# allenai/satlas-super-resolution

Measured on AMD Instinct MI355X. Metric: G+D train-step images/sec, higher is better.
Workload: dtype fp32h

## Files before the change

include/ssr_hip.h:

```cpp
#ifndef SSR_HIP_H
#define SSR_HIP_H

#include <stdint.h>

#ifdef __cplusplus
extern "C" {
#endif

#define SSR_F32 0
#define SSR_BF16 1
#define SSR_F32X3 2
#define SSR_F32H 3
#define SSR_F32H_WSHIFT 10

#define SSR_OK 0
#define SSR_EINVAL (-1)
#define SSR_EUNSUP (-2)

#define SSR_ACT_NONE 0
#define SSR_ACT_LRELU 1
#define SSR_ACT_RELU 2

typedef struct ssr_view {
    void* p;
    int32_t cs;
    int32_t coff;
} ssr_view;

typedef struct ssr_conv_desc {
    int32_t dtype;
    ssr_view x;
    int32_t N, Hi, Wi;
    int32_t up;
    int32_t Cin;
    ssr_view x2;
    int32_t Cin2;
    const void* w;
    int32_t CoutPad;
    const float* bias;
    int32_t KH, KW, stride, pad_y, pad_x;
    int32_t Gh, Gw;
    int32_t Ho, Wo, oys, oyo, oxs, oxo;
    int32_t Cout;
    ssr_view y, y0, y1;
    float alpha;
    int32_t act;
    ssr_view r1; int32_t r1_nc; float beta1;
    ssr_view r2; int32_t r2_nc; float beta2;
    int32_t accumulate;
    ssr_view m; int32_t m_c0, m_c1;
    int32_t s2d;
    int32_t m_relu;
    int32_t* fix_list;
    int32_t fix_cap;
    float fix_thr;
    const float* w_ref;
    const float* w_ref_sigma;
    int32_t w_ref_cin;
} ssr_conv_desc;

int ssr_conv2d(const ssr_conv_desc* d, void* stream);
int ssr_conv2d_fixup(const ssr_conv_desc* d, void* stream);
int ssr_conv2d_batch(const ssr_conv_desc* ds, int32_t n, void* stream);
int ssr_conv2d_impl(const ssr_conv_desc* d, void* stream, int32_t impl);
int ssr_conv2d_variant(const ssr_conv_desc* d);
int ssr_conv2d_chain(const ssr_conv_desc* ds, int32_t n, void* state, void* stream);
int ssr_conv2d_chain_ok(const ssr_conv_desc* ds, int32_t n);
int64_t ssr_conv2d_chain_state_bytes(int32_t N, int32_t Gh, int32_t Gw);
int ssr_conv2d_symbol(const ssr_conv_desc* d, char* buf, int32_t buflen);
int ssr_conv2d_ck(int32_t dtype, int32_t KH);
int ssr_conv2d_s2d_ok(int32_t dtype, int32_t Cin, int32_t Cout, int32_t CoutPad);

typedef struct ssr_rdb_desc {
    int32_t dtype, N, H, W;
    ssr_view in, slices, out, mask;
    const void* w[5];
    const float* bias[5];
    float alpha5, beta1;
    ssr_view r2;
    float beta2;
    const void* w_next[5];
    int32_t w_next_bytes[5];
    int32_t tile;
} ssr_rdb_desc;
int ssr_rdb_forward(const ssr_rdb_desc* d, void* stream);
int ssr_rdb_backward(const ssr_rdb_desc* d, void* stream);
int ssr_rdb_tile_of(const ssr_rdb_desc* d);

typedef struct ssr_wgrad_layer {
    ssr_view x;
    ssr_view dy;
    int32_t N, Hi, Wi, up, Cin, Cout;
    int32_t pad_y, pad_x, Gh, Gw;
    float alpha;
    float* dw;
    int32_t Cin_w;
    float* db;
} ssr_wgrad_layer;

typedef struct ssr_wgrad_item {
    int32_t layer, co0, ci0, tile_begin, tile_end, atomic;
    int32_t nco, layer_b, co0_b;
} ssr_wgrad_item;

int ssr_conv2d_wgrad(const ssr_wgrad_layer* layers_dev, const ssr_wgrad_item* items_dev, int32_t n_items,
                     int32_t dtype, int32_t KH, int32_t KW, int32_t stride, void* stream);
int32_t ssr_wgrad_tiles(int32_t N, int32_t Gh, int32_t Gw, int32_t dtype, int32_t KH);
int32_t ssr_wgrad_ci_tile(int32_t dtype, int32_t KH);
int32_t ssr_wgrad_co_tile(int32_t dtype, int32_t KH);

typedef struct ssr_pack_item {
    const float* src;
    const float* inv_scale;
    void* dst_fwd;
    void* dst_dgrad;
    int32_t Cout, Cin, KH, KW, stride;
    int32_t CoutPad, CinPad;
    int32_t CinPadO, CoutPadI;
    int32_t ck_fwd, ck_dgrad;
    int32_t fwd_s2d;
} ssr_pack_item;

int ssr_pack_weights(const ssr_pack_item* items_dev, int32_t n_items, int32_t dtype, void* stream);

typedef struct ssr_pack_seg {
    const float* src;
    void* dst;
    float scale;
    int32_t Cout, Cin;
    int32_t ci0, nci;
    int32_t kbase;
    int32_t rows_pad, ck;
} ssr_pack_seg;
int ssr_pack_dgrad_gather(const ssr_pack_seg* items_dev, int32_t n_items, int32_t dtype, void* stream);

int ssr_add_views(ssr_view dst, ssr_view src, int32_t dtype, int64_t npix, int32_t C, void* stream);

int ssr_nchw_to_nhwc(const float* src, int32_t N, int32_t C, int32_t H, int32_t W, ssr_view dst, int32_t dtype,
                     int32_t unshuffle, int32_t up, float scale, void* stream);
int ssr_nhwc_to_nchw(ssr_view src, int32_t dtype, float* dst, int32_t N, int32_t C, int32_t H, int32_t W,
                     void* stream);
int ssr_fill(void* p, int64_t n_elems, int32_t dtype, float value, void* stream);

int ssr_bilinear2x_fwd(ssr_view a, ssr_view b, ssr_view y, int32_t dtype, int32_t N, int32_t H, int32_t W, int32_t C,
                       void* stream);
int ssr_bilinear2x_bwd(ssr_view dy, ssr_view r, ssr_view y1, ssr_view y, ssr_view m, int32_t dtype, int32_t N,
                       int32_t H, int32_t W, int32_t C, void* stream);
#define SSR_BILINEAR_FLAT 0x100
int ssr_nearest2x_bwd(ssr_view dy, ssr_view r, ssr_view y1, ssr_view y, ssr_view m, int32_t dtype, int32_t N,
                      int32_t H, int32_t W, int32_t C, void* stream);

typedef struct ssr_sn_item {
    const float* w;
    float* u;
    float* v;
    float* sigma;
    float* tmp;
    int32_t rows, cols;
} ssr_sn_item;
int ssr_spectral_norm(const ssr_sn_item* items_dev, int32_t n_items, int32_t max_rows, int32_t max_cols,
                      int32_t power_iter, void* stream);
#define SSR_SN_BWD_SLOTS 64
typedef struct ssr_sn_bwd_item {
    const float* dw_sn; const float* w; const float* u; const float* v; const float* sigma;
    float* dw; float* tmp; int32_t rows, cols;
} ssr_sn_bwd_item;
int ssr_spectral_norm_bwd(const ssr_sn_bwd_item* items_dev, int32_t n_items, int32_t max_elems, void* stream);

int ssr_usm_sharp(const float* src, float* dst, int32_t planes, int32_t H, int32_t W, float in_scale, float weight,
                  float threshold, void* stream);

#define SSR_DETERMINISTIC 0x200
#define SSR_LOSS_SLOTS 256
int ssr_l1_loss(ssr_view a, ssr_view b, ssr_view grad, int32_t dtype, int64_t npix, int32_t C, float weight,
                float* loss_out, void* stream);
int ssr_bce_logits_loss(ssr_view x, ssr_view grad, int32_t dtype, int64_t npix, float target, float weight,
                        float* loss_out, float* mean_out, void* stream);

typedef struct ssr_reduce_item { float* dst; const float* src; int64_t n, stride; int32_t parts, pad_; } ssr_reduce_item;
int ssr_wgrad_reduce(const ssr_reduce_item* items_dev, int32_t n_items, int64_t max_elems, void* stream);

typedef struct ssr_adam_args {
    float* param; const float* grad; float* exp_avg; float* exp_avg_sq;
    float* ema;
    int64_t n;
    const float* lr;
    int32_t* step;
    float beta1, beta2, eps, ema_decay, grad_scale;
} ssr_adam_args;
int ssr_adam_step(const ssr_adam_args* a, void* stream);

int ssr_axpby_f32(float a, const float* x, float b, float* y, int64_t n, void* stream);

#define SSR_SCAN_MAX_RANGES 8
int ssr_nonfinite_scan(const float* const* srcs, const int64_t* ns, int32_t n_ranges, int32_t* flag, void* stream);
int ssr_adam_step_guarded(const ssr_adam_args* a, int32_t* flag, int32_t* skipped, void* stream);

int ssr_quantize_u8(const float* src_nchw, uint8_t* dst_nhwc, int32_t N, int32_t C, int32_t H, int32_t W, int32_t mode, void* stream);
int ssr_quantize_u8_checked(const float* src_nchw, uint8_t* dst_nhwc, int32_t N, int32_t C, int32_t H, int32_t W, int32_t mode,
                            int32_t* nonfinite, void* stream);
int ssr_metric_shift_sums(const uint8_t* a, const uint8_t* b, int32_t H, int32_t W, int32_t C, int32_t crop, int32_t max_offset,
                          int64_t* out, void* stream);
int ssr_metric_ssim_sums(const uint8_t* a, const uint8_t* b, int32_t H, int32_t W, int32_t C, int32_t crop, double* out, void* stream);

int ssr_scene_zero_scan(const uint8_t* scene, int32_t T, int32_t H, int32_t W, uint8_t* has_zero, void* stream);
int ssr_scene_gather(const uint8_t* scene, int32_t T, int32_t H, int32_t W, const int32_t* chunk_ids, const int32_t* frame_ids,
                     int32_t B, int32_t n, ssr_view dst, int32_t dtype, void* stream);
int ssr_scene_scatter_u8(ssr_view src, int32_t dtype, const int32_t* chunk_ids, int32_t B, int32_t C, uint8_t* mosaic, int32_t Ho,
                         int32_t Wo, int32_t* nonfinite, void* stream);

int ssr_scene_zero_scan_at(const uint8_t* scene, int32_t T, int32_t H, int32_t W, const int32_t* origins, int32_t n_chunks,
                           uint8_t* has_zero, void* stream);
int ssr_scene_gather_at(const uint8_t* scene, int32_t T, int32_t H, int32_t W, const int32_t* origins, const int32_t* frame_ids,
                        int32_t B, int32_t n, ssr_view dst, int32_t dtype, void* stream);
// ... 39 lines not shown
```

satlas_super_resolution_amd/csrc/common.h:

```cpp
#pragma once
#include <hip/hip_runtime.h>
#include <stdint.h>
#include "ssr_hip.h"
#include <type_traits>

template <int I, int N, typename F> __device__ __forceinline__ void static_for(F&& f) {
    if constexpr (I < N) {
        f(std::integral_constant<int, I>{});
        static_for<I + 1, N>(f);
    }
}

typedef float f32x4 __attribute__((ext_vector_type(4)));
typedef float f32x16 __attribute__((ext_vector_type(16)));
typedef __bf16 bf16x8 __attribute__((ext_vector_type(8)));
typedef __bf16 bf16x4 __attribute__((ext_vector_type(4)));
typedef uint32_t u32x4 __attribute__((ext_vector_type(4)));
typedef _Float16 f16x8 __attribute__((ext_vector_type(8)));
typedef _Float16 f16x4 __attribute__((ext_vector_type(4)));

template <bool H> __device__ __forceinline__ f32x16 split_mfma(const bf16x8& a, const bf16x8& b, const f32x16& c) {
    if constexpr (H) return __builtin_amdgcn_mfma_f32_32x32x16_f16(__builtin_bit_cast(f16x8, a), __builtin_bit_cast(f16x8, b), c, 0, 0, 0);
    else return __builtin_amdgcn_mfma_f32_32x32x16_bf16(a, b, c, 0, 0, 0);
}
template <bool H> __device__ __forceinline__ void split_f32x4(const u32x4& v, uint2& hi, uint2& lo) {
    const f32x4 f = __builtin_bit_cast(f32x4, v);
    if constexpr (H) {
        f16x4 h, l;
#pragma unroll
        for (int k = 0; k < 4; ++k) {
            h[k] = (_Float16)f[k];
            l[k] = (_Float16)(f[k] - (float)h[k]);
        }
        hi = __builtin_bit_cast(uint2, h);
        lo = __builtin_bit_cast(uint2, l);
    } else {
        bf16x4 h, l;
#pragma unroll
        for (int k = 0; k < 4; ++k) {
            h[k] = (__bf16)f[k];
            l[k] = (__bf16)(f[k] - (float)h[k]);
        }
        hi = __builtin_bit_cast(uint2, h);
        lo = __builtin_bit_cast(uint2, l);
    }
}
constexpr float SSR_F32H_WSCALE = (float)(1 << SSR_F32H_WSHIFT), SSR_F32H_UNSCALE = 1.0f / (float)(1 << SSR_F32H_WSHIFT);

#define LRELU_SLOPE 0.2f

template <typename T> struct DT;
template <> struct DT<float> { static constexpr int VEC = 4; };
template <> struct DT<__bf16> { static constexpr int VEC = 8; };

__device__ __forceinline__ float to_f32(float v) { return v; }
__device__ __forceinline__ float to_f32(__bf16 v) { return (float)v; }
template <typename T> __device__ __forceinline__ T from_f32(float v);
template <> __device__ __forceinline__ float from_f32<float>(float v) { return v; }
template <> __device__ __forceinline__ __bf16 from_f32<__bf16>(float v) { return (__bf16)v; }

__device__ __forceinline__ float lrelu(float v) { return v > 0.f ? v : LRELU_SLOPE * v; }
__device__ __forceinline__ float lrelu_grad_from_out(float out) { return out > 0.f ? 1.f : LRELU_SLOPE; }
__device__ __forceinline__ float lrelu_max(float v) {
    float r;
    const float s = LRELU_SLOPE * v;
    asm("v_max_f32 %0, %1, %2" : "=v"(r) : "v"(v), "v"(s));
    return r;
}
__device__ __forceinline__ float lrelu_mask_lo(float v, unsigned m2) { return (int)(m2 << 16) > 0 ? v : LRELU_SLOPE * v; }
__device__ __forceinline__ float lrelu_mask_hi(float v, unsigned m2) { return (int)m2 > 0xFFFF ? v : LRELU_SLOPE * v; }

template <typename T> __device__ __forceinline__ void mma16(f32x16& acc, const u32x4& a, const u32x4& b);
template <> __device__ __forceinline__ void mma16<float>(f32x16& acc, const u32x4& a, const u32x4& b) {
    const f32x4 af = __builtin_bit_cast(f32x4, a), bf = __builtin_bit_cast(f32x4, b);
#pragma unroll
    for (int s = 0; s < 4; ++s) acc = __builtin_amdgcn_mfma_f32_32x32x2f32(af[s], bf[s], acc, 0, 0, 0);
}
template <> __device__ __forceinline__ void mma16<__bf16>(f32x16& acc, const u32x4& a, const u32x4& b) {
    acc = __builtin_amdgcn_mfma_f32_32x32x16_bf16(__builtin_bit_cast(bf16x8, a), __builtin_bit_cast(bf16x8, b), acc,
                                                  0, 0, 0);
}

__device__ __forceinline__ int mfma32_row(int r, int g) { return (r & 3) + 8 * (r >> 2) + 4 * g; }

constexpr int SSR_MAX_DEVICES = 32;
inline int ssr_device_ordinal() {
    int dev = 0;
    if (hipGetDevice(&dev) != hipSuccess || dev < 0 || dev >= SSR_MAX_DEVICES) dev = 0;
    return dev;
}

#define SSR_LAUNCH_CHECK()                       \
    do {                                         \
        hipError_t e__ = hipGetLastError();      \
        if (e__ != hipSuccess) return (int)e__;  \
    } while (0)
```

satlas_super_resolution_amd/csrc/conv.hip:

```cpp
#include "conv_epilogue.h"
#include <cstdlib>
#include <cstdio>

namespace {

template <typename T, int KH, int KW, int S, int NT, int MW, int KS>
__device__ __forceinline__ void conv_body(const ssr_conv_desc& d) {
    constexpr int VEC = DT<T>::VEC;
    constexpr int KSTEPS = (KH == 4) ? 1 : 2;
    constexpr int CK = KSTEPS * 2 * VEC, VPR = 2 * KSTEPS, CKP = CK + VEC, BN = 32 * NT;
    constexpr int TH = 2 * MW, TW = 16;
    constexpr int PH = (TH - 1) * S + KH, PW = (TW - 1) * S + KW;
    constexpr int NTHR = 64 * MW * KS;
    constexpr int PVEC = PH * PW * VPR, WVEC = KH * KW * BN * VPR;
    constexpr int NPV = (PVEC + NTHR - 1) / NTHR, NWV = (WVEC + NTHR - 1) / NTHR;
    constexpr int STAGE = (PH * PW + KH * KW * BN) * CKP;
    extern __shared__ __attribute__((aligned(16))) char smem[];
    T* lds = reinterpret_cast<T*>(smem);

    const int tid = threadIdx.x, lane = tid & 63, wave = tid >> 6;
    const int wm = wave % MW, kh = wave / MW;
    const int tiles_x = (d.Gw + TW - 1) / TW, tiles_y = (d.Gh + TH - 1) / TH;
    int b = blockIdx.x;
    const int tx_i = b % tiles_x; b /= tiles_x;
// ... 635 lines not shown
            if (KS == 2 && kh_s == 1) contract_h(buf, std::integral_constant<int, 1>{}, units);
            else contract_h(buf, std::integral_constant<int, 0>{}, units);
        } else {
            if (KS == 2 && kh_s == 1) contract_h(buf, std::integral_constant<int, 1>{}, none);
            else contract_h(buf, std::integral_constant<int, 0>{}, none);
        }
    };

    XPROBE(1);
    static_for<0, PD>([&](auto jc) { load_stage(decltype(jc)::value, jc); });
    store_stage(0, std::integral_constant<int, 0>{});
    __syncthreads();
    XPROBE(2);
    for (int c = 0; c < nst; c += PD) {
        static_for<0, PD>([&](auto jc) {
            constexpr int j = decltype(jc)::value;
            const int cur = c + j;
            if (cur < nst) {
                load_stage(cur + PD, jc);
                contract(cur & 1, std::integral_constant<int, (j + 1) % PD>{}, cur + 1 < nst);
#ifdef SSR_PROBE
                const unsigned long long tm_ = __builtin_amdgcn_s_memtime();
#endif
#ifdef SSR_PROBE
                if (threadIdx.x == 0 && cur == 0) { g_probe[(blockIdx.y * gridDim.x + blockIdx.x) * 24 + 20] = tm_; g_probe[(blockIdx.y * gridDim.x + blockIdx.x) * 24 + 21] = __builtin_amdgcn_s_memtime(); }
#endif
                __syncthreads();
#ifdef SSR_PROBE
                if (cur < 12) XPROBE(3 + cur);
#endif
            }
        });
    }
    XPROBE(15);

    char* slab = smem + (size_t)MW * 16 * 64 * sizeof(float) + (size_t)wave * EPI_STAGE_BYTES;
    auto epilogue = [&](const f32x16& a, int t) {
        conv_epilogue<float>(d, a, co0 + t * 32, n, gy0 + 2 * wm, gx0, lane, slab);
    };
    if (KS == 1) {
#pragma unroll
        for (int t = 0; t < NT; ++t) epilogue(acc[t], t);
    } else {
        float* red = reinterpret_cast<float*>(smem);
        float* mine = red + (wm * 16) * 64 + lane;
        if (NT == 2) {
            if (kh == 0) {
#pragma unroll
                for (int r = 0; r < 16; ++r) mine[r * 64] = acc[1][r];
            }
            __syncthreads();
            if (kh == 1) {
#pragma unroll
                for (int r = 0; r < 16; ++r) acc[1][r] += mine[r * 64];
            }
            __syncthreads();
            if (kh == 1) {
#pragma unroll
                for (int r = 0; r < 16; ++r) mine[r * 64] = acc[0][r];
            }
            __syncthreads();
            if (kh == 0) {
#pragma unroll
                for (int r = 0; r < 16; ++r) acc[0][r] += mine[r * 64];
                epilogue(acc[0], 0);
            } else {
                epilogue(acc[1], 1);
            }
        } else {
            if (kh == 1) {
#pragma unroll
                for (int r = 0; r < 16; ++r) mine[r * 64] = acc[0][r];
            }
            __syncthreads();
            if (kh == 0) {
#pragma unroll
                for (int r = 0; r < 16; ++r) acc[0][r] += mine[r * 64];
                epilogue(acc[0], 0);
            }
        }
    }
    XPROBE(17);
}

template <int KH, int KW, int NT, int MW, int KS, int CPS, int PD>
__global__ __launch_bounds__(64 * MW * KS) void conv_x3p_kernel(const ssr_conv_desc d) {
    conv_body_x3p<KH, KW, NT, MW, KS, CPS, PD>(d);
}

template <int KH, int KW, int NT, int MW, int KS, int CPS, int PD>
int launch_conv_x3p(const ssr_conv_desc& d, hipStream_t st) {
    constexpr int BN = 32 * NT, TH = 2 * MW, TW = 16, PH = TH - 1 + KH, PW = TW - 1 + KW;
    constexpr size_t stage = (size_t)CPS * (PH * PW + KH * KW * BN) * 80;
    constexpr size_t red = (size_t)MW * 16 * 64 * sizeof(float) + (size_t)MW * KS * EPI_STAGE_BYTES;
    constexpr size_t lds = 2 * stage > red ? 2 * stage : red;
    static_assert(lds <= 160 * 1024, "LDS budget");
    auto kern = conv_x3p_kernel<KH, KW, NT, MW, KS, CPS, PD>;
    static bool attr_done[SSR_MAX_DEVICES] = {};
    const int attr_dev = ssr_device_ordinal();
    if (!attr_done[attr_dev]) {
        hipError_t e = hipFuncSetAttribute(reinterpret_cast<const void*>(kern), hipFuncAttributeMaxDynamicSharedMemorySize, (int)lds);
        if (e != hipSuccess) return (int)e;
        attr_done[attr_dev] = true;
    }
    const int tiles = ((d.Gw + TW - 1) / TW) * ((d.Gh + TH - 1) / TH) * d.N;
    hipLaunchKernelGGL(kern, dim3(tiles, d.CoutPad / BN, 1), dim3(64 * MW * KS), lds, st, d);
    SSR_LAUNCH_CHECK();
    return SSR_OK;
}

bool x3p_ok(const ssr_conv_desc& d, int cps) {
    static const bool on = [] { const char* e = getenv("SSR_X3_PIPE"); return e && e[0] == '1'; }();
    if (!on) return false;
    const long lim = 0x7fffff00L, npx = (long)d.N * d.Hi * d.Wi * 4;
    if (npx * d.x.cs > lim || (d.x2.p && npx * d.x2.cs > lim)) return false;
    if (d.x2.p && (d.Cin % (16 * cps)) != 0) return false;
    return true;
}

template <int KH, int KW, bool H = false>
int dispatch_tile_x3(const ssr_conv_desc& d, hipStream_t st) {
    bool nt2, small;
    pick_tile(d, nt2, small);
    static const long thr = [] { const char* e = getenv("SSR_X3_SMALL"); return e ? atol(e) : 0L; }();
    small = (long)((d.Gw + 15) / 16) * ((d.Gh + 7) / 8) * d.N * (d.CoutPad / (nt2 ? 64 : 32)) < thr;
    if (!small && !H) {
        static const bool p2 = [] { const char* e = getenv("SSR_X3_PIPE2"); return e && e[0] == '1'; }();
        if (nt2 && p2 && x3p_ok(d, 1)) return launch_conv_x3p<KH, KW, 2, 4, 2, 1, 3>(d, st);
        if (!nt2 && x3p_ok(d, 2)) return launch_conv_x3p<KH, KW, 1, 4, 2, 2, 2>(d, st);
    }
    if (nt2) return small ? launch_conv_x3<KH, KW, 2, 2, 2, H>(d, st) : launch_conv_x3<KH, KW, 2, 4, 2, H>(d, st);
    return small ? launch_conv_x3<KH, KW, 1, 2, 2, H>(d, st) : launch_conv_x3<KH, KW, 1, 4, 2, H>(d, st);
}

bool view_ok(const ssr_view& v, bool required) {
    if (!v.p) return !required;
    return (v.cs % 8) == 0 && (v.coff % 8) == 0 && ((uintptr_t)v.p % 16) == 0;
}

}

bool ssr_conv_res_try(const ssr_conv_desc& d, hipStream_t st, int* rc);
bool ssr_conv_res_qualifies(const ssr_conv_desc& d);
bool ssr_conv_ws_try(const ssr_conv_desc& d, hipStream_t st, int* rc, bool force);
bool ssr_conv_ws_qualifies(const ssr_conv_desc& d);
bool ssr_conv_thin_try(const ssr_conv_desc& d, hipStream_t st, int* rc, bool force);
bool ssr_conv_thin_qualifies(const ssr_conv_desc& d);
bool ssr_conv_big_try(const ssr_conv_desc& d, hipStream_t st, int* rc, bool force);
bool ssr_conv_big_qualifies(const ssr_conv_desc& d);
bool ssr_conv_big_batch_try(const ssr_conv_desc* ds, int n, hipStream_t st, int* rc);
bool ssr_conv_bigx3_try(const ssr_conv_desc& d, hipStream_t st, int* rc, bool force);
bool ssr_conv_bigx3_qualifies(const ssr_conv_desc& d);
bool ssr_conv_bigx3_batch_try(const ssr_conv_desc* ds, int n, hipStream_t st, int* rc);
bool ssr_conv_x3q_try(const ssr_conv_desc& d, hipStream_t st, int* rc, bool force);
bool ssr_conv_x3q_qualifies(const ssr_conv_desc& d);
bool ssr_conv_x3r_try(const ssr_conv_desc& d, hipStream_t st, int* rc, bool force);
bool ssr_conv_x3r_qualifies(const ssr_conv_desc& d);

extern "C" int ssr_conv2d_s2d_ok(int32_t dtype, int32_t Cin, int32_t Cout, int32_t CoutPad) {
    static const bool off = [] { const char* e = getenv("SSR_CONV_S2D"); return e && e[0] == '0'; }();
    if (dtype == SSR_F32X3 || dtype == SSR_F32H) {
        static const bool offx = [] { const char* e = getenv("SSR_X3_BIGTILE"); return e && e[0] == '0'; }();
        const int cpx = Cin / 16;
        return !off && !offx && Cin >= 16 && (Cin % 16) == 0 && (cpx & (cpx - 1)) == 0 && (CoutPad % 64) == 0 && (Cout % 8) == 0;
    }
    const int cpc = Cin / 32;
    return !off && dtype == SSR_BF16 && Cin >= 32 && (Cin % 32) == 0 && (cpc & (cpc - 1)) == 0 && (CoutPad % 64) == 0 && (Cout % 8) == 0;
}

extern "C" int ssr_conv2d_variant(const ssr_conv_desc* dp) {
    if (!dp) return SSR_EINVAL;
    if (dp->s2d) return dp->KH * 1000 + dp->stride * 100 + 2 * 10 + 9;
    const bool split = dp->dtype == SSR_F32X3 || dp->dtype == SSR_F32H;
    const bool pipelined_only = !split && (dp->act == SSR_ACT_RELU || dp->m_relu);
    if (!pipelined_only) {
        if (dp->dtype != SSR_BF16 && ssr_conv_thin_qualifies(*dp)) return dp->KH * 1000 + dp->stride * 100 + 1 * 10 + 7;
        if (split && ssr_conv_bigx3_qualifies(*dp)) return dp->KH * 1000 + dp->stride * 100 + 2 * 10 + 9;
        if (split && ssr_conv_x3r_qualifies(*dp))
            return dp->KH * 1000 + dp->stride * 100 + ((dp->CoutPad % 64) == 0 ? 2 : 1) * 10 + 5;
        if (dp->dtype == SSR_F32X3 && ssr_conv_x3q_qualifies(*dp))
            return dp->KH * 1000 + dp->stride * 100 + ((dp->CoutPad % 64) == 0 ? 2 : 1) * 10 + 6;
        if (!split) {
            if (ssr_conv_thin_qualifies(*dp)) return dp->KH * 1000 + dp->stride * 100 + 1 * 10 + 7;
            if (ssr_conv_ws_qualifies(*dp)) return dp->KH * 1000 + dp->stride * 100 + 1 * 10 + 8;
            if (ssr_conv_big_qualifies(*dp)) return dp->KH * 1000 + dp->stride * 100 + 2 * 10 + 9;
            if (dp->dtype == SSR_F32 && ssr_conv_x3r_qualifies(*dp))
                return dp->KH * 1000 + dp->stride * 100 + ((dp->CoutPad % 64) == 0 ? 2 : 1) * 10 + 5;
            if (ssr_conv_res_qualifies(*dp)) return dp->KH * 1000 + dp->stride * 100 + 1 * 10 + 1;
        }
    }
    bool nt2, small;
    pick_tile(*dp, nt2, small);
    return dp->KH * 1000 + dp->stride * 100 + (nt2 ? 2 : 1) * 10 + (small ? 2 : 4);
}

void ssr_conv_x3r_instance(const ssr_conv_desc& d, int* ntw, int* nu, int* ep);
int ssr_conv_x3r_tile_height(const ssr_conv_desc& d);

extern "C" int ssr_conv2d_symbol(const ssr_conv_desc* dp, char* buf, int32_t buflen) {
    if (!dp || !buf || buflen < 48) return SSR_EINVAL;
    const ssr_conv_desc& d = *dp;
    const int v = ssr_conv2d_variant(dp);
    if (v < 0) return v;
    const int w = v % 10, nt = (v / 10) % 10;
    const bool f32m = d.dtype != SSR_BF16;
    if (d.dtype != SSR_BF16 && w == 5) {
        int ntw = 1, nu = 1, ep = 3;
        ssr_conv_x3r_instance(d, &ntw, &nu, &ep);
        snprintf(buf, buflen, "conv_x3r_kernel<%d, %d, %d, %d, %d>", ntw, nu, ep, ssr_conv_x3r_tile_height(d), d.dtype == SSR_F32 ? 1 : d.dtype == SSR_F32H ? 2 : 0);
    } else if (d.dtype == SSR_F32X3 && w == 6) snprintf(buf, buflen, "conv_x3q_kernel<%d>", nt);
    else if (d.dtype == SSR_F32X3 && w == 9) snprintf(buf, buflen, "conv_bigx3_kernel4<%d>", (d.s2d || d.KH == 2) ? 2 : 3);
    else if (d.dtype == SSR_F32H && w == 9) snprintf(buf, buflen, "conv_bigh3_kernel4<%d>", (d.s2d || d.KH == 2) ? 2 : 3);
    else if (f32m && w == 7) snprintf(buf, buflen, "conv_thin_f32_kernel<%d, %d>", d.Cout == 1 ? 1 : d.Cout <= 3 ? 3 : d.Cout == 4 ? 4 : 8, d.dtype == SSR_F32X3 ? 1 : d.dtype == SSR_F32H ? 2 : 0);
    else snprintf(buf, buflen, "%s<%s,K%d,S%d,NT%d,W%d>", w == 7 ? "conv_thin_kernel" : w == 8 ? "conv_ws_kernel" : w == 9 ? "conv_big_kernel" : w == 1 ? "conv_res_kernel" : d.dtype == SSR_F32X3 ? "conv_x3_kernel" : d.dtype == SSR_F32H ? "conv_h3_kernel" : "conv_kernel",
                  d.dtype == SSR_BF16 ? "bf16" : d.dtype == SSR_F32 ? "fp32" : d.dtype == SSR_F32H ? "fp32h" : "fp32x3", v / 1000, (v / 100) % 10, nt, w);
    return SSR_OK;
}

extern "C" int ssr_conv2d_ck(int32_t dtype, int32_t KH) {
    const int vec = dtype == SSR_BF16 ? 8 : 4;
    return (KH == 4 ? 1 : 2) * 2 * vec;
}

static int conv2d_impl(const ssr_conv_desc* dp, void* stream, int impl) {
    if (!dp) return SSR_EINVAL;
    const ssr_conv_desc& d = *dp;
    if (d.act < SSR_ACT_NONE || d.act > SSR_ACT_RELU) return SSR_EINVAL;
    if (!view_ok(d.x, true) || !d.w || ((uintptr_t)d.w % 16) != 0) return SSR_EINVAL;
    if (!d.y.p || d.y.cs <= 0) return SSR_EINVAL;
    if (d.Cin <= 0 || (d.Cin % 8) != 0 || d.CoutPad <= 0 || (d.CoutPad % 32) != 0 || d.Cout > d.CoutPad)
        return SSR_EINVAL;
    if (!(d.up == 1 || d.up == 2) || d.N <= 0 || d.Gh <= 0 || d.Gw <= 0) return SSR_EINVAL;
    if (d.x2.p && (d.Cin2 <= 0 || (d.Cin2 % 8) != 0 || !view_ok(d.x2, true))) return SSR_EINVAL;
    if (!d.x2.p && d.Cin2 != 0) return SSR_EINVAL;
    hipStream_t st = reinterpret_cast<hipStream_t>(stream);
    int rc = 0;
    if (d.s2d) {
        if (!(d.KH == 4 && d.KW == 4 && d.stride == 2 && d.pad_y == 1 && d.pad_x == 1 && d.up == 1 && !d.x2.p)) return SSR_EINVAL;
        if (!ssr_conv2d_s2d_ok(d.dtype, d.Cin, d.Cout, d.CoutPad) || (d.Hi % 2) || (d.Wi % 2) || d.Gh != d.Hi / 2 || d.Gw != d.Wi / 2)
            return SSR_EINVAL;
        ssr_conv_desc e = d;
        e.KH = e.KW = 2; e.stride = 1; e.pad_y = e.pad_x = 0; e.Cin = 4 * d.Cin;
        if (d.dtype == SSR_F32X3 || d.dtype == SSR_F32H) return ssr_conv_bigx3_try(e, st, &rc, true) ? rc : SSR_EUNSUP;
        return ssr_conv_big_try(e, st, &rc, true) ? rc : SSR_EUNSUP;
    }
    if (d.dtype == SSR_F32H) {
        if (d.fix_list) return SSR_EUNSUP;
        if (impl == 4) return ssr_conv_bigx3_try(d, st, &rc, true) ? rc : SSR_EUNSUP;
        if (impl == 5) return ssr_conv_thin_try(d, st, &rc, true) ? rc : SSR_EUNSUP;
        if (impl == 7) return ssr_conv_x3r_try(d, st, &rc, true) ? rc : SSR_EUNSUP;
        if (impl == 0 && ssr_conv_thin_try(d, st, &rc, false)) return rc;
        if (impl == 0 && ssr_conv_bigx3_try(d, st, &rc, false)) return rc;
        if (impl == 0 && ssr_conv_x3r_try(d, st, &rc, false)) return rc;
        if (d.KH == 3 && d.KW == 3 && d.stride == 1) return dispatch_tile_x3<3, 3, true>(d, st);
        if (d.KH == 2 && d.KW == 2 && d.stride == 1) return dispatch_tile_x3<2, 2, true>(d, st);
        ssr_conv_desc e = d;
        e.dtype = SSR_F32;
        return dispatch_geom<float>(e, st);
    }
    if (d.dtype == SSR_F32X3) {
        if (impl == 4) return ssr_conv_bigx3_try(d, st, &rc, true) ? rc : SSR_EUNSUP;
        if (impl == 5) return ssr_conv_thin_try(d, st, &rc, true) ? rc : SSR_EUNSUP;
        if (impl == 6) return ssr_conv_x3q_try(d, st, &rc, true) ? rc : SSR_EUNSUP;
        if (impl == 7) return ssr_conv_x3r_try(d, st, &rc, true) ? rc : SSR_EUNSUP;
        if (impl == 0 && ssr_conv_thin_try(d, st, &rc, false)) return rc;
        if (impl == 0 && ssr_conv_bigx3_try(d, st, &rc, false)) return rc;
        if (impl == 0 && ssr_conv_x3r_try(d, st, &rc, false)) return rc;
        if (impl == 0 && ssr_conv_x3q_try(d, st, &rc, false)) return rc;
        if (d.KH == 3 && d.KW == 3 && d.stride == 1) return dispatch_tile_x3<3, 3>(d, st);
        if (d.KH == 2 && d.KW == 2 && d.stride == 1) return dispatch_tile_x3<2, 2>(d, st);
        ssr_conv_desc e = d;
        e.dtype = SSR_F32;
        return dispatch_geom<float>(e, st);
    }
    if (d.act == SSR_ACT_RELU || d.m_relu) impl = 3;
    if (impl == 1) return ssr_conv_ws_try(d, st, &rc, true) ? rc : SSR_EUNSUP;
    if (impl == 4) return ssr_conv_big_try(d, st, &rc, true) ? rc : SSR_EUNSUP;
    if (impl == 5) return ssr_conv_thin_try(d, st, &rc, true) ? rc : SSR_EUNSUP;
    if (impl == 0 && ssr_conv_thin_try(d, st, &rc, false)) return rc;
    if (impl == 0 && ssr_conv_ws_try(d, st, &rc, false)) return rc;
    if (impl == 0 && ssr_conv_big_try(d, st, &rc, false)) return rc;
    if (d.dtype == SSR_F32 && impl == 7) return ssr_conv_x3r_try(d, st, &rc, true) ? rc : SSR_EUNSUP;
    if (d.dtype == SSR_F32 && impl == 0 && ssr_conv_x3r_try(d, st, &rc, false)) return rc;
    if (impl != 3 && ssr_conv_res_try(d, st, &rc)) return rc;
    if (d.dtype == SSR_F32) return dispatch_geom<float>(d, st);
    if (d.dtype == SSR_BF16) return dispatch_geom<__bf16>(d, st);
    return SSR_EUNSUP;
}

extern "C" int ssr_conv2d(const ssr_conv_desc* dp, void* stream) { return conv2d_impl(dp, stream, 0); }

namespace {
__global__ __launch_bounds__(256) void conv_fixup_kernel(const ssr_conv_desc d) {
    int* hdr = d.fix_list;
    const int count = min(hdr[0], d.fix_cap);
    const int lane = threadIdx.x & 63, wave = threadIdx.x >> 6;
    const int nw = gridDim.x * 4;
    const int KK = d.KH * d.KW, K = d.w_ref_cin * KK;
    const float* __restrict__ xp = reinterpret_cast<const float*>(d.x.p);
    float* __restrict__ yp = reinterpret_cast<float*>(d.y.p);
    const double inv_sigma = d.w_ref_sigma ? 1.0 / (double)d.w_ref_sigma[0] : 1.0;
    const int sh = d.up == 2 ? 1 : 0, LH = d.Hi << sh, LW = d.Wi << sh;
    for (int e = blockIdx.x * 4 + wave; e < count; e += nw) {
        const int p = hdr[4 + 2 * e], co = hdr[5 + 2 * e];
        const int ox = p % d.Wo, t = p / d.Wo, oy = t % d.Ho, n = t / d.Ho;
        const float* __restrict__ wrow = d.w_ref + (size_t)co * K;
        double s = 0.0;
        for (int k = lane; k < K; k += 64) {
            const int ci = k / KK, tap = k - ci * KK, ky = tap / d.KW, kx = tap - ky * d.KW;
            const int iy = oy * d.stride + ky - d.pad_y, ix = ox * d.stride + kx - d.pad_x;
            if (iy >= 0 && iy < LH && ix >= 0 && ix < LW) {
                const size_t px = (size_t)(n * d.Hi + (iy >> sh)) * d.Wi + (ix >> sh);
                s += (double)wrow[k] * (double)xp[px * d.x.cs + d.x.coff + ci];
            }
        }
#pragma unroll
        for (int m = 32; m >= 1; m >>= 1) s += __shfl_xor(s, m);
        if (lane == 0) {
            const float v = (float)(s * inv_sigma + (d.bias ? (double)d.bias[co] : 0.0));
            yp[(size_t)p * d.y.cs + d.y.coff + co] = lrelu(v);
        }
    }
    __syncthreads();
    if (threadIdx.x == 0) {
        __threadfence();
        if (atomicAdd(hdr + 1, 1) == (int)gridDim.x - 1) {
            atomicMax(hdr + 2, hdr[0]);
            hdr[0] = 0;
            hdr[1] = 0;
        }
    }
}
}

extern "C" int ssr_conv2d_fixup(const ssr_conv_desc* dp, void* stream) {
    if (!dp) return SSR_EINVAL;
    const ssr_conv_desc& d = *dp;
    if (!d.fix_list || d.fix_cap <= 0 || !d.w_ref || d.w_ref_cin <= 0 || !d.x.p || !d.y.p) return SSR_EINVAL;
    if ((d.dtype != SSR_F32X3 && d.dtype != SSR_F32) || d.act != SSR_ACT_LRELU || d.x2.p || d.y0.p || d.y1.p || d.r1.p || d.r2.p || d.m.p ||
        d.accumulate || d.alpha != 1.f || d.stride != 1 || d.s2d || d.oys != 1 || d.oxs != 1 || d.oyo != 0 || d.oxo != 0 ||
        d.w_ref_cin > d.Cin)
        return SSR_EUNSUP;
    hipLaunchKernelGGL(conv_fixup_kernel, dim3(32), dim3(256), 0, reinterpret_cast<hipStream_t>(stream), d);
    SSR_LAUNCH_CHECK();
    return SSR_OK;
}

extern "C" int ssr_conv2d_batch(const ssr_conv_desc* ds, int32_t n, void* stream) {
    if (!ds || n <= 0 || n > 4) return SSR_EINVAL;
    bool same = ds[0].dtype == SSR_BF16 && ds[0].KH == 2 && ds[0].KW == 2 && ds[0].stride == 1;
    for (int k = 1; k < n && same; ++k)
        same = ds[k].dtype == ds[0].dtype && ds[k].KH == 2 && ds[k].KW == 2 && ds[k].stride == 1 && ds[k].N == ds[0].N &&
               ds[k].Gh == ds[0].Gh && ds[k].Gw == ds[0].Gw && ds[k].CoutPad == ds[0].CoutPad && ds[k].Cin == ds[0].Cin &&
               ds[k].Cin2 == ds[0].Cin2 && ds[k].Hi == ds[0].Hi && ds[k].Wi == ds[0].Wi && ds[k].up == ds[0].up;
    static const bool off = [] { const char* e = getenv("SSR_CONV_BATCH"); return e && e[0] == '0'; }();
    if (!off && ds[0].dtype == SSR_F32X3 && ds[0].KH == 2 && ds[0].KW == 2 && ds[0].stride == 1) {
        int rcx = 0;
        if (ssr_conv_bigx3_batch_try(ds, n, reinterpret_cast<hipStream_t>(stream), &rcx)) return rcx;
    }
    if (same && !off) {
        for (int k = 0; k < n; ++k) {
            const ssr_conv_desc& d = ds[k];
            if (!view_ok(d.x, true) || !d.w || ((uintptr_t)d.w % 16) != 0 || !d.y.p || d.y.cs <= 0 || d.Cin <= 0 || (d.Cin % 8) != 0 ||
                d.CoutPad <= 0 || (d.CoutPad % 32) != 0 || d.Cout > d.CoutPad || !(d.up == 1 || d.up == 2) || d.N <= 0 || d.Gh <= 0 ||
                d.Gw <= 0 || (d.x2.p && (d.Cin2 <= 0 || (d.Cin2 % 8) != 0 || !view_ok(d.x2, true))) || (!d.x2.p && d.Cin2 != 0))
                return SSR_EINVAL;
        }
        hipStream_t st = reinterpret_cast<hipStream_t>(stream);
        int rcb = 0;
        if (ssr_conv_big_batch_try(ds, n, st, &rcb)) return rcb;
        bool nt2, small;
        pick_tile(ds[0], nt2, small);
        const long tiles4 = (long)((ds[0].Gw + 15) / 16) * ((ds[0].Gh + 7) / 8) * ds[0].N * (ds[0].CoutPad / (nt2 ? 64 : 32)) * n;
        small = tiles4 < 384;
        if (nt2) return small ? launch_conv4<__bf16, 2, 2, 1, 2, 2, 2>(ds, n, st) : launch_conv4<__bf16, 2, 2, 1, 2, 4, 2>(ds, n, st);
        return small ? launch_conv4<__bf16, 2, 2, 1, 1, 2, 2>(ds, n, st) : launch_conv4<__bf16, 2, 2, 1, 1, 4, 2>(ds, n, st);
    }
    for (int k = 0; k < n; ++k) {
        const int rc = conv2d_impl(ds + k, stream, 0);
// ... 8 lines not shown
```

satlas_super_resolution_amd/csrc/conv_big_x3.hip:

```cpp
#include "common.h"
#include <cstdlib>

namespace {

constexpr int XB_TH = 32, XB_TW = 16;
template <int KT> struct XbT {
    static constexpr int AROW = 80;
    static constexpr int VPP = 4;
    static constexpr int PH = XB_TH + KT - 1, PW = XB_TW + KT - 1, NPIX = PH * PW;
    static constexpr int PATCH = NPIX * AROW;
    static constexpr int WROWS = KT * KT * 64;
    static constexpr int WBYTES = WROWS * AROW;
    static constexpr int BUF = PATCH + WBYTES;
    static constexpr int BIAS = BUF;
    static constexpr int SLABS = BIAS + 256;
    static constexpr int LDS = SLABS + 4 * 32 * 272;
    static constexpr int NPV = (NPIX * VPP + 255) / 256;
    static constexpr int NWV = (WROWS * VPP + 255) / 256;
    static constexpr int NSTEP = KT * KT;
    static constexpr int TAIL = KT == 3 ? 2 : 1;
    static constexpr int LPS = (NPV + NWV + NSTEP - TAIL - 1) / (NSTEP - TAIL);
    static_assert(LDS <= 160 * 1024 && LPS <= 6, "LDS budget / load slots of a step");
};

#define XB_BAR() asm volatile("s_waitcnt lgkmcnt(0)\n\ts_barrier" ::: "memory")
#ifdef SSR_PROBE
#define XB_T() (__builtin_amdgcn_s_memtime())
#define XB_ACC(k, t0) do { const unsigned long long t1_ = XB_T(); xb_t[k] += t1_ - (t0); (t0) = t1_; } while (0)
#else
#define XB_T() 0ull
#define XB_ACC(k, t0) do { } while (0)
#endif
constexpr int XB_OOB = 0x7ffffff0;
constexpr int XB_SLAB_PITCH = 272, XB_SLAB = 32 * XB_SLAB_PITCH;
__device__ __forceinline__ __amdgpu_buffer_rsrc_t xb_rsrc(const void* p, long bytes) {
    return __builtin_amdgcn_make_buffer_rsrc(const_cast<void*>(p), 0, (int)(bytes > 0x7fffff00L ? 0x7fffff00L : (bytes < 0 ? 0 : bytes)), 0x00020000);
}
template <int KT>
__device__ __forceinline__ void xb_pixel(int w, int m, int s, int& row, int& col) {
    row = 8 * w + 2 * m + (s >> 4);
    col = s < 16 ? s : ((s + 32 - (XB_TW + KT - 1)) & 15);
}
__device__ __forceinline__ void xb_split4(const u32x4& v, uint2& hi, uint2& lo) {
    const f32x4 f = __builtin_bit_cast(f32x4, v);
    bf16x4 h, l;
#pragma unroll
    for (int k = 0; k < 4; ++k) {
        h[k] = (__bf16)f[k];
        l[k] = (__bf16)(f[k] - (float)h[k]);
    }
    hi = __builtin_bit_cast(uint2, h);
    lo = __builtin_bit_cast(uint2, l);
}

template <int KT, bool H = false>
__device__ __forceinline__ void conv_bigx3_body(const ssr_conv_desc& d) {
    using T = XbT<KT>;
    constexpr int AROW = T::AROW, VPP = T::VPP, PW = T::PW, NPIX = T::NPIX, PATCH = T::PATCH, NPV = T::NPV, NWV = T::NWV, NSTEP = T::NSTEP;
    extern __shared__ __attribute__((aligned(16))) char smem[];
    const int tid = threadIdx.x, lane = tid & 63, wave = tid >> 6;
    const int i = lane & 31, g = lane >> 5;
    const int tiles_x = (d.Gw + XB_TW - 1) / XB_TW, tiles_y = (d.Gh + XB_TH - 1) / XB_TH;
    const int tpi = tiles_x * tiles_y, G = gridDim.x / tpi;
    const int tp = blockIdx.x % tpi, n0 = blockIdx.x / tpi;
    const int tx_i = tp % tiles_x, ty_i = tp / tiles_x;
    const int nimg = (d.N - n0 + G - 1) / G;
    const int gy0 = ty_i * XB_TH, gx0 = tx_i * XB_TW;
    const int co0 = blockIdx.y * 64;
    const int upshift = d.up == 2 ? 1 : 0;
    const int LH = d.Hi << upshift, LW = d.Wi << upshift;
    const int nchunks = (d.Cin + 15) / 16;
    const int wchunk = KT * KT * d.CoutPad * 64;
    const int T_ = nimg * nchunks;
    const int ximg = d.Hi * d.Wi * d.x.cs * 4, oimg = d.Ho * d.Wo;

    unsigned long long xb_t[8] = {0, 0, 0, 0, 0, 0, 0, 0}, xb_t0 = XB_T();
    const unsigned long long xb_start = xb_t0;
    (void)xb_t; (void)xb_start;
    float* bias_lds = reinterpret_cast<float*>(smem + T::BIAS);
    if (tid < 64) bias_lds[tid] = (d.bias && co0 + tid < d.Cout) ? d.bias[co0 + tid] * (H ? SSR_F32H_WSCALE : 1.f) : 0.f;

    const bool s2d = KT == 2 && d.s2d != 0;
    const int cpc_shift = s2d ? 31 - __builtin_clz((unsigned)(d.Cin >> 6)) : 0;
    const int x_cs = d.x.cs, x_Wi = d.Wi, x_Cin = d.Cin;
    static_assert((T::WROWS * VPP) % 256 == 0, "no partial weight vector");
    const int p4 = tid >> 2, part4 = tid & 3;
    const int plo0 = p4 * AROW + part4 * 8;
    const int wlo0 = PATCH + p4 * AROW + part4 * 16;
    const int wgo0 = (co0 + p4) * 64 + part4 * 16, wstep = d.CoutPad * 64;
    constexpr int PTAIL = NPIX * VPP - (NPV - 1) * 256;
    int pgo[NPV];
    unsigned pmk[KT == 2 ? NPV : 1];
    const int climit = s2d ? 0x7fffffff : x_Cin - (tid % VPP) * 4;
#pragma unroll
    for (int q = 0; q < NPV; ++q) {
        const int v = tid + q * 256;
        const int pix = v / VPP, part = v % VPP;
        const int py = pix / PW, px = pix - py * PW;
        const int ly = gy0 + py - d.pad_y, lx = gx0 + px - d.pad_x;
        if constexpr (KT == 2) {
            if (s2d) {
                const int sy = 2 * ly - 1, sx = 2 * lx - 1;
                const bool y0 = sy >= 0 && sy < d.Hi, y1 = sy + 1 >= 0 && sy + 1 < d.Hi;
                const bool x0 = sx >= 0 && sx < d.Wi, x1 = sx + 1 >= 0 && sx + 1 < d.Wi;
                pmk[q] = v < NPIX * VPP ? (unsigned)(y0 && x0) | (unsigned)(y0 && x1) << 1 | (unsigned)(y1 && x0) << 2 | (unsigned)(y1 && x1) << 3 : 0u;
                pgo[q] = ((sy * d.Wi + sx) * d.x.cs + d.x.coff + part * 4) * 4 + (d.Wi + 1) * d.x.cs * 4;
            } else {
                const bool ok = v < NPIX * VPP && ly >= 0 && ly < LH && lx >= 0 && lx < LW;
                pmk[q] = ok ? 1u : 0u;
                pgo[q] = ok ? (((ly >> upshift) * d.Wi + (lx >> upshift)) * d.x.cs + d.x.coff + part * 4) * 4 : XB_OOB;
            }
        } else {
            const bool ok = v < NPIX * VPP && ly >= 0 && ly < LH && lx >= 0 && lx < LW;
            pgo[q] = ok ? (((ly >> upshift) * d.Wi + (lx >> upshift)) * d.x.cs + d.x.coff + part * 4) * 4 : XB_OOB;
        }
    }
    const long xbias = s2d ? (long)(d.Wi + 1) * d.x.cs * 4 : 0;
    const __amdgpu_buffer_rsrc_t rsx = xb_rsrc(reinterpret_cast<const char*>(d.x.p) - xbias, (long)d.N * ximg + xbias),
                                 rsw = xb_rsrc(d.w, (long)nchunks * wchunk);
    u32x4 rp[NPV], rw[NWV];
    struct LoadPos { int q, c0, xs, ws; };
    auto load_pos = [&](int nn, int c) {
        LoadPos p;
        p.c0 = c * 16;
        if constexpr (KT == 2) {
            p.q = s2d ? c >> cpc_shift : 0;
            p.xs = nn * ximg + (s2d ? (((p.q >> 1) * x_Wi + (p.q & 1)) * x_cs + ((c - (p.q << cpc_shift)) << 4)) * 4 : p.c0 * 4);
        } else {
            p.q = 0;
            p.xs = nn * ximg + p.c0 * 4;
        }
        p.ws = c * wchunk;
        return p;
    };
    auto load_one = [&](const LoadPos& lp, auto jc) {
        constexpr int j = decltype(jc)::value;
        if constexpr (j < NPV) {
            bool ok = lp.c0 < climit;
            if constexpr (KT == 2) ok = ok && ((pmk[j] >> lp.q) & 1u);
            rp[j] = __builtin_amdgcn_raw_buffer_load_b128(rsx, ok ? pgo[j] : XB_OOB, lp.xs, 0);
        } else {
            rw[j - NPV] = __builtin_amdgcn_raw_buffer_load_b128(rsw, wgo0, lp.ws + (j - NPV) * wstep, 0);
        }
    };
    auto load_chunk = [&](int nn, int c) { const LoadPos lp = load_pos(nn, c); static_for<0, NPV + NWV>([&](auto jc) { load_one(lp, jc); }); };
    auto store_chunk = [&]() {
        static_for<0, NPV>([&](auto jc) {
            constexpr int j = decltype(jc)::value;
            uint2 hi, lo;
            split_f32x4<H>(rp[j], hi, lo);
            if (j + 1 < NPV || tid < PTAIL) {
                *reinterpret_cast<uint2*>(smem + plo0 + j * 64 * AROW) = hi;
                *reinterpret_cast<uint2*>(smem + plo0 + j * 64 * AROW + 32) = lo;
            }
        });
        static_for<0, NWV>([&](auto jc) {
            constexpr int j = decltype(jc)::value;
            *reinterpret_cast<u32x4*>(smem + wlo0 + j * 64 * AROW) = rw[j];
        });
    };

    int a_off[4];
#pragma unroll
    for (int m = 0; m < 4; ++m) {
        int row, col;
        xb_pixel<KT>(wave, m, i, row, col);
        a_off[m] = (row * PW + col) * AROW + g * 16;
    }
    const int b_off = PATCH + i * AROW + g * 16;
    const int co_l = 4 * g;

    load_chunk(n0, 0);
    __syncthreads();
    XB_ACC(1, xb_t0);
    f32x16 acc[4][2];
    auto acc_init = [&]() {
#pragma unroll
        for (int t = 0; t < 2; ++t)
#pragma unroll
            for (int q4 = 0; q4 < 4; ++q4) {
                const f32x4 bq = *reinterpret_cast<const f32x4*>(bias_lds + t * 32 + 8 * q4 + co_l);
#pragma unroll
                for (int e = 0; e < 4; ++e)
#pragma unroll
                    for (int m = 0; m < 4; ++m) acc[m][t][4 * q4 + e] = bq[e];
            }
    };

    char* slab = smem + T::SLABS + wave * XB_SLAB;
    auto epilogue_impl = [&](int nn, auto opsc, auto y01c) __attribute__((always_inline)) {
        constexpr bool OPS = decltype(opsc)::value, Y01 = decltype(y01c)::value;
        const long obytes = (long)d.N * oimg * 4;
        const __amdgpu_buffer_rsrc_t rs_r1 = xb_rsrc(d.r1.p, d.r1.p ? obytes * d.r1.cs : 0), rs_r2 = xb_rsrc(d.r2.p, d.r2.p ? obytes * d.r2.cs : 0),
                                     rs_m = xb_rsrc(d.m.p, d.m.p ? obytes * d.m.cs : 0), rs_y = xb_rsrc(d.y.p, obytes * d.y.cs),
                                     rs_y0 = xb_rsrc(d.y0.p, d.y0.p ? obytes * d.y0.cs : 0), rs_y1 = xb_rsrc(d.y1.p, d.y1.p ? obytes * d.y1.cs : 0);
        const bool has_r1 = d.r1.p != nullptr, has_r2 = d.r2.p != nullptr, has_m = d.m.p != nullptr, has_acc = d.accumulate != 0,
                   has_y0 = d.y0.p != nullptr, has_y1 = d.y1.p != nullptr, m_relu = d.m_relu != 0;
        const float slope = d.act == SSR_ACT_LRELU ? 0.2f : d.act == SSR_ACT_RELU ? 0.f : 1.f;
        const float alpha = d.alpha, beta1 = has_r1 ? d.beta1 : 0.f, beta2 = has_r2 ? d.beta2 : 0.f, gacc = has_acc ? 1.f : 0.f;
        const int y_cs = d.y.cs, y_co = d.y.coff, y0_cs = d.y0.cs, y0_co = d.y0.coff, y1_cs = d.y1.cs, y1_co = d.y1.coff;
        const int r1_cs = d.r1.cs, r1_co = d.r1.coff, r2_cs = d.r2.cs, r2_co = d.r2.coff, m_cs = d.m.cs, m_co = d.m.coff;
        const int Gh = d.Gh, Gw = d.Gw, oys = d.oys, oyo = d.oyo, oxs = d.oxs, oxo = d.oxo, Wo = d.Wo;
        const int pimg = nn * oimg;
        const int hp = lane >> 4, c = co0 + (lane & 15) * 4;
        const bool cok = c < d.Cout;
#pragma unroll
        for (int m = 0; m < 4; ++m) {
            int po[8];
#pragma unroll
            for (int h = 0; h < 8; ++h) {
                int row, col;
                xb_pixel<KT>(wave, m, 4 * h + hp, row, col);
                const int gy = gy0 + row, gx = gx0 + col;
                const bool ok = gy < Gh && gx < Gw;
                const int cy = gy < Gh ? gy : Gh - 1, cx = gx < Gw ? gx : Gw - 1;
                po[h] = (pimg + (cy * oys + oyo) * Wo + cx * oxs + oxo) | (ok && cok ? 0 : (int)0x80000000);
            }
#pragma unroll
            for (int t = 0; t < 2; ++t)
#pragma unroll
                for (int q4 = 0; q4 < 4; ++q4) {
                    const f32x4 v = {acc[m][t][4 * q4], acc[m][t][4 * q4 + 1], acc[m][t][4 * q4 + 2], acc[m][t][4 * q4 + 3]};
                    *reinterpret_cast<f32x4*>(slab + i * XB_SLAB_PITCH + (t * 32 + 8 * q4 + co_l) * 4) = v;
                }
#pragma unroll
            for (int hh = 0; hh < 2; ++hh) {
                u32x4 q1[OPS ? 4 : 1], q2[OPS ? 4 : 1], qa[OPS ? 4 : 1], qm[OPS ? 4 : 1];
                if constexpr (OPS) {
#pragma unroll
                    for (int h4 = 0; h4 < 4; ++h4) {
                        const int pp = po[4 * hh + h4] & 0x7fffffff;
                        q1[h4] = __builtin_amdgcn_raw_buffer_load_b128(rs_r1, cok && has_r1 ? (pp * r1_cs + r1_co + c) * 4 : XB_OOB, 0, 0);
                        q2[h4] = __builtin_amdgcn_raw_buffer_load_b128(rs_r2, cok && has_r2 ? (pp * r2_cs + r2_co + c) * 4 : XB_OOB, 0, 0);
                        qa[h4] = __builtin_amdgcn_raw_buffer_load_b128(rs_y, cok && has_acc ? (pp * y_cs + y_co + c) * 4 : XB_OOB, 0, 0);
                        qm[h4] = __builtin_amdgcn_raw_buffer_load_b128(rs_m, cok && has_m ? (pp * m_cs + m_co + c) * 4 : XB_OOB, 0, 0);
                    }
                }
#pragma unroll
                for (int h4 = 0; h4 < 4; ++h4) {
                    const int h = 4 * hh + h4;
                    f32x4 a = *reinterpret_cast<const f32x4*>(slab + (4 * h + hp) * XB_SLAB_PITCH + (lane & 15) * 16);
                    if constexpr (H) a *= SSR_F32H_UNSCALE;
                    const bool ok = po[h] >= 0;
                    const int pp = po[h] & 0x7fffffff;
                    f32x4 v, s0, s1;
#pragma unroll
                    for (int e = 0; e < 4; ++e) {
                        float x = fmaxf(a[e], slope * a[e]) * alpha;
                        s0[e] = x;
                        if constexpr (OPS) {
                            x += beta1 * __builtin_bit_cast(f32x4, q1[h4])[e] + beta2 * __builtin_bit_cast(f32x4, q2[h4])[e] + gacc * __builtin_bit_cast(f32x4, qa[h4])[e];
                            s1[e] = x;
                            const float mv = __builtin_bit_cast(f32x4, qm[h4])[e];
                            const float f = m_relu ? (mv > 0.f ? 1.f : 0.f) : lrelu_grad_from_out(mv);
                            x *= has_m ? f : 1.f;
                        } else {
                            s1[e] = x;
                        }
                        v[e] = x;
                    }
                    if constexpr (Y01) {
                        __builtin_amdgcn_raw_buffer_store_b128(__builtin_bit_cast(u32x4, s0), rs_y0, ok && has_y0 ? (pp * y0_cs + y0_co + c) * 4 : XB_OOB, 0, 0);
                        __builtin_amdgcn_raw_buffer_store_b128(__builtin_bit_cast(u32x4, s1), rs_y1, ok && has_y1 ? (pp * y1_cs + y1_co + c) * 4 : XB_OOB, 0, 0);
                    }
                    __builtin_amdgcn_raw_buffer_store_b128(__builtin_bit_cast(u32x4, v), rs_y, ok ? (pp * y_cs + y_co + c) * 4 : XB_OOB, 0, 0);
                }
            }
        }
    };
    auto epilogue = [&](int nn) __attribute__((always_inline)) {
        const bool ops = d.r1.p != nullptr || d.r2.p != nullptr || d.m.p != nullptr || d.accumulate != 0;
        const bool y01 = d.y0.p != nullptr || d.y1.p != nullptr;
        if (ops) {
            if (y01) epilogue_impl(nn, std::true_type{}, std::true_type{});
            else epilogue_impl(nn, std::true_type{}, std::false_type{});
        } else {
            if (y01) epilogue_impl(nn, std::false_type{}, std::true_type{});
            else epilogue_impl(nn, std::false_type{}, std::false_type{});
        }
    };

    auto chunk = [&](int c, bool stored, int nn1, int c1, auto hnc) __attribute__((always_inline)) {
        constexpr bool has_next = decltype(hnc)::value;
        xb_t0 = XB_T();
        if (!stored) {
            if (c > 0) XB_BAR();
            XB_ACC(2, xb_t0);
            store_chunk();
            XB_ACC(3, xb_t0);
        }
        XB_BAR();
        XB_ACC(4, xb_t0);
        const LoadPos lp1 = load_pos(nn1, c1);
        bf16x8 wq[2][2][2], pq[2][4][2];
        auto issue1 = [&](auto sc, auto kc) {
            constexpr int s_ = decltype(sc)::value, k = decltype(kc)::value;
            if constexpr (k < 4)
                wq[s_ & 1][k >> 1][k & 1] = *reinterpret_cast<const bf16x8*>(smem + b_off + (s_ * 64 + (k >> 1) * 32) * AROW + (k & 1) * 32);
            else
                pq[s_ & 1][(k - 4) >> 1][k & 1] =
                    *reinterpret_cast<const bf16x8*>(smem + a_off[(k - 4) >> 1] + ((s_ / KT) * PW + s_ % KT) * AROW + (k & 1) * 32);
        };
        static_for<0, 12>([&](auto kc) { issue1(std::integral_constant<int, 0>{}, kc); });
        static_for<0, NSTEP>([&](auto sc) {
            constexpr int s_ = decltype(sc)::value;
            static_for<0, 24>([&](auto kc) {
                constexpr int k = decltype(kc)::value, m = k / 6, t = (k % 6) / 3, p = k % 3;
                acc[m][t] = split_mfma<H>(wq[s_ & 1][t][p == 0 ? 1 : 0], pq[s_ & 1][m][p == 1 ? 1 : 0], acc[m][t]);
                __builtin_amdgcn_sched_barrier(0);
                if constexpr (k < 12) {
                    if constexpr (s_ + 1 < NSTEP) issue1(std::integral_constant<int, s_ + 1>{}, kc);
                } else if constexpr (has_next && (k & 1) == 0 && (k - 12) / 2 < T::LPS) {
                    constexpr int j = s_ * T::LPS + (k - 12) / 2;
                    if constexpr (j < NPV + NWV) load_one(lp1, std::integral_constant<int, j>{});
                }
                __builtin_amdgcn_sched_barrier(0);
            });
        });
        __builtin_amdgcn_sched_barrier(0);
        XB_ACC(5, xb_t0);
        xb_t[7] += 1;
    };
    int gc = 0;
    for (int k = 0; k < nimg; ++k) {
        const int nn = n0 + k * G;
        const bool last_img = k + 1 == nimg;
        acc_init();
        for (int c = 0; c < (last_img ? nchunks - 1 : nchunks); ++c, ++gc) {
            const bool last_c = c + 1 == nchunks;
            chunk(gc, k > 0 && c == 0, last_c ? nn + G : nn, last_c ? 0 : c + 1, std::true_type{});
        }
        if (!last_img) {
            xb_t0 = XB_T();
            XB_BAR();
            XB_ACC(2, xb_t0);
            store_chunk();
            XB_ACC(3, xb_t0);
            epilogue(nn);
            XB_ACC(6, xb_t0);
        }
    }
    const int nl = n0 + (nimg - 1) * G;
    chunk(gc, nimg > 1 && nchunks == 1, nl, 0, std::false_type{});
    xb_t0 = XB_T();
    epilogue(nl);
    XB_ACC(6, xb_t0);
#ifdef SSR_PROBE
    if (tid == 0) {
        xb_t[0] = XB_T() - xb_start;
        const int b = (blockIdx.z * gridDim.y + blockIdx.y) * gridDim.x + blockIdx.x;
        for (int k = 0; k < 8; ++k) g_probe[b * 8 + k] = xb_t[k];
    }
#endif
    (void)T_;
}

struct ssr_conv_desc4x { ssr_conv_desc d[4]; };
template <int KT>
__global__ __launch_bounds__(256, 1) void conv_bigx3_kernel4(const ssr_conv_desc4x p) {
    conv_bigx3_body<KT>(p.d[blockIdx.z]);
}
template <int KT>
__global__ __launch_bounds__(256, 1) void conv_bigh3_kernel4(const ssr_conv_desc4x p) {
    conv_bigx3_body<KT, true>(p.d[blockIdx.z]);
}

template <int KT, bool H = false>
int launch_bigx3(const ssr_conv_desc* ds, int n, hipStream_t st) {
    constexpr int lds = XbT<KT>::LDS;
    const ssr_conv_desc& d = ds[0];
    const int tpi = ((d.Gh + XB_TH - 1) / XB_TH) * ((d.Gw + XB_TW - 1) / XB_TW);
    static const int ncu = [] { int dev = 0, v = 256; if (hipGetDevice(&dev) == hipSuccess && hipDeviceGetAttribute(&v, hipDeviceAttributeMultiprocessorCount, dev) != hipSuccess) v = 256; return v > 0 ? v : 256; }();
    int G = d.N;
    {
        const long per_img = (long)tpi * (d.CoutPad / 64) * n;
        long best = -1;
        for (int g = 1; g <= d.N; ++g) {
            const long rounds = (per_img * g + ncu - 1) / ncu, cost = rounds * ((d.N + g - 1) / g);
            const long key = (cost << 24) | (rounds << 12) | (4095 - (g > 4095 ? 4095 : g));
            if (best < 0 || key < best) { best = key; G = g; }
        }
    }
    if (const char* e = getenv("SSR_CONV_BIG_G")) {
        const int g = atoi(e);
        if (g >= 1) G = g < d.N ? g : d.N;
    }
    const int tiles = tpi * G;
    auto kern = H ? conv_bigh3_kernel4<KT> : conv_bigx3_kernel4<KT>;
    static bool attr_done[SSR_MAX_DEVICES] = {};
    const int attr_dev = ssr_device_ordinal();
    if (!attr_done[attr_dev]) {
        hipError_t e = hipFuncSetAttribute(reinterpret_cast<const void*>(kern), hipFuncAttributeMaxDynamicSharedMemorySize, lds);
        if (e != hipSuccess) return (int)e;
        attr_done[attr_dev] = true;
    }
    ssr_conv_desc4x p;
    for (int k = 0; k < 4; ++k) p.d[k] = ds[k < n ? k : 0];
    hipLaunchKernelGGL(kern, dim3(tiles, d.CoutPad / 64, n), dim3(256), lds, st, p);
    SSR_LAUNCH_CHECK();
    return SSR_OK;
}

}

bool ssr_conv_bigx3_shape_ok(const ssr_conv_desc& d) {
    if ((d.dtype != SSR_F32X3 && d.dtype != SSR_F32H) || d.fix_list) return false;
    const bool k3 = d.KH == 3 && d.KW == 3 && d.pad_y == 1 && d.pad_x == 1;
    const bool k2 = d.KH == 2 && d.KW == 2 && (d.pad_y == 0 || d.pad_y == 1) && (d.pad_x == 0 || d.pad_x == 1);
    if (!(k3 || k2) || d.stride != 1 || d.x2.p) return false;
    if (d.Cin < 8 || (d.CoutPad % 64) != 0 || (d.Cout % 4) != 0) return false;
    if (d.s2d) {
        const int cpc = d.Cin / 64;
        if (!k2 || d.pad_y != 0 || d.pad_x != 0 || d.up != 1 || (d.Cin % 64) != 0 || cpc < 1 || (cpc & (cpc - 1)) != 0) return false;
        if ((d.Hi % 2) != 0 || (d.Wi % 2) != 0 || d.Gh != d.Hi / 2 || d.Gw != d.Wi / 2) return false;
    } else if (d.Gh != (d.Hi << (d.up == 2)) || d.Gw != (d.Wi << (d.up == 2))) return false;
    if (d.r1.p && d.r1_nc < d.Cout) return false;
    if (d.r2.p && d.r2_nc < d.Cout) return false;
    if (d.m.p && !(d.m_c0 == 0 && d.m_c1 >= d.Cout)) return false;
    const long lim = 0x7fffff00L;
    const long xin = ((long)d.N * d.Hi * d.Wi + d.Wi + 1) * d.x.cs * 4, npo = (long)d.N * d.Ho * d.Wo * 4;
    if (xin > lim || npo * d.y.cs > lim || (d.y0.p && npo * d.y0.cs > lim) || (d.y1.p && npo * d.y1.cs > lim) || (d.r1.p && npo * d.r1.cs > lim) ||
        (d.r2.p && npo * d.r2.cs > lim) || (d.m.p && npo * d.m.cs > lim))
        return false;
    if ((long)((d.Cin + 15) / 16) * d.KH * d.KW * d.CoutPad * 64 > lim) return false;
    auto al16 = [](const ssr_view& v) { return !v.p || ((v.cs % 4) == 0 && (v.coff % 4) == 0 && ((uintptr_t)v.p % 16) == 0); };
    return d.x.p && d.y.p && al16(d.x) && al16(d.y) && al16(d.y0) && al16(d.y1) && al16(d.r1) && al16(d.r2) && al16(d.m);
}

bool ssr_conv_bigx3_qualifies(const ssr_conv_desc& d) {
    static const bool off = [] { const char* e = getenv("SSR_X3_BIGTILE"); return e && e[0] == '0'; }();
    if (off || !ssr_conv_bigx3_shape_ok(d) || d.KH != 3) return false;
    const long per_img = (long)((d.Gh + XB_TH - 1) / XB_TH) * ((d.Gw + XB_TW - 1) / XB_TW) * (d.CoutPad / 64);
    return per_img >= 4 && d.Gh >= 24;
}

bool ssr_conv_bigx3_try(const ssr_conv_desc& d, hipStream_t st, int* rc, bool force) {
    if (force ? !ssr_conv_bigx3_shape_ok(d) : !ssr_conv_bigx3_qualifies(d)) return false;
    if (d.dtype == SSR_F32H) *rc = d.KH == 3 ? launch_bigx3<3, true>(&d, 1, st) : launch_bigx3<2, true>(&d, 1, st);
    else *rc = d.KH == 3 ? launch_bigx3<3>(&d, 1, st) : launch_bigx3<2>(&d, 1, st);
    return true;
}

bool ssr_conv_bigx3_batch_try(const ssr_conv_desc* ds, int n, hipStream_t st, int* rc) {
    const char* e = getenv("SSR_X3_BIGTILE2");
    const bool off = e && e[0] == '0', always = e && e[0] == '2';
    if (off || n < 1 || n > 4) return false;
    for (int k = 0; k < n; ++k)
        if (!ssr_conv_bigx3_shape_ok(ds[k]) || ds[k].dtype != SSR_F32X3 || ds[k].KH != 2 || ds[k].s2d) return false;
    const ssr_conv_desc& d = ds[0];
    for (int k = 1; k < n; ++k)
        if (ds[k].N != d.N || ds[k].Gh != d.Gh || ds[k].Gw != d.Gw || ds[k].CoutPad != d.CoutPad || ds[k].Cin != d.Cin || ds[k].Hi != d.Hi || ds[k].Wi != d.Wi ||
            ds[k].up != d.up)
            return false;
    const long per_img = (long)((d.Gh + XB_TH - 1) / XB_TH) * ((d.Gw + XB_TW - 1) / XB_TW) * (d.CoutPad / 64) * n;
    if (!always && (per_img < 8 || d.Gh < 24)) return false;
    *rc = launch_bigx3<2>(ds, n, st);
    return true;
}
```

satlas_super_resolution_amd/csrc/conv_x3c.hip:

```cpp
#include "conv_x3r_core.h"
#include <cstdio>

#ifdef SSR_PROBE
#define CPROBE(cond, k) do { if (cond) g_probe[blockIdx.x * 32 + (k)] = __builtin_amdgcn_s_memtime(); } while (0)
#else
#define CPROBE(cond, k)
#endif

namespace {

constexpr int XC_MAXN = 4;
constexpr int XC_MAXCH = 16;
constexpr int XC_NS = 6;
constexpr int XC_RING = XC_NS * XR_SUB;
constexpr int XC_RED = 16 * XR_SLOT;
constexpr int XC_CTL = XC_RING + XC_RED;
constexpr int XC_LDS = XC_CTL + 256;
static_assert(XC_LDS <= 160 * 1024, "LDS budget");
constexpr int XC_STATE_HDR = 64;
constexpr int XC_POLL_MAX = 1 << 20;

struct ssr_chain_args {
    ssr_conv_desc d[XC_MAXN];
    int32_t n;
// ... 217 lines not shown
                });
                int gn = g + 4 < glast ? g + 4 : glast;
                int c_next = gn / 3, base_next = base_of(gn);
                int gnn = gn, c_nn = c_next, base_nn = base_next;
                auto body = [&](int j, auto jpc) {
                    constexpr int JP = decltype(jpc)::value;
                    static_for<0, NSUB>([&](auto qc) {
                        constexpr int q = decltype(qc)::value, kx = q / SPT, part = q % SPT, qn = q + PD;
                        constexpr int ws = (JP * 3 + kx) % WR, as = (JP * NSUB + q) % NSETS, asn = (JP * NSUB + qn) % NSETS;
                        auto group = [&](auto pc) {
                            constexpr int P = decltype(pc)::value;
#pragma unroll
                            for (int t2 = 0; t2 < TPS; ++t2)
                                acc[part * TPS + t2] = __builtin_amdgcn_mfma_f32_32x32x16_bf16(af[as][t2][P == 0 ? 1 : 0], wf[ws][P == 1 ? 1 : 0], acc[part * TPS + t2], 0, 0, 0);
                        };
                        auto reads = [&](auto hc) {
                            if constexpr (qn < NSUB) issue_a(base_cur, std::integral_constant<int, qn>{}, std::integral_constant<int, asn>{}, hc);
                            else issue_a(base_next, std::integral_constant<int, qn - NSUB>{}, std::integral_constant<int, asn>{}, hc);
                        };
                        __builtin_amdgcn_sched_barrier(0);
                        if constexpr (qn == NSUB) {
                            if (c_next > c_cur) {
                                asm volatile("" ::: "memory");
                                if (lane == 0) *(xr_lds_int)(uintptr_t)(ctl_addr + 16 + 4 * w) = Gbase + c_next;
                                asm volatile("" ::: "memory");
                            }
                            ensure(Gbase + c_next);
                            __builtin_amdgcn_sched_barrier(0);
                        }
                        group(std::integral_constant<int, 0>{});
                        __builtin_amdgcn_sched_barrier(0);
                        reads(I1{});
                        if constexpr (part == 0) {
                            constexpr int wsp = (JP * 3 + kx + WR - 1) % WR, ioff = (kx + WR - 1) / 3, tap = (kx + WR - 1) % 3;
                            load_w(g + 4 * ioff, std::integral_constant<int, tap>{}, std::integral_constant<int, wsp>{});
                        }
                        __builtin_amdgcn_sched_barrier(0);
                        group(std::integral_constant<int, 1>{});
                        __builtin_amdgcn_sched_barrier(0);
                        reads(I0{});
                        if constexpr (q == 0) {
                            gnn = g + 8 < glast ? g + 8 : glast;
                            c_nn = gnn / 3;
                            base_nn = base_of(gnn);
                        }
                        __builtin_amdgcn_sched_barrier(0);
                        group(std::integral_constant<int, 2>{});
                        __builtin_amdgcn_sched_barrier(0);
                    });
                    g += 4;
                    c_cur = c_next; base_cur = base_next;
                    gn = gnn; c_next = c_nn; base_next = base_nn;
                };
                for (int j = 0; j < nj; j += 2) {
                    body(j, std::integral_constant<int, 0>{});
                    if (j + 1 < nj) body(j + 1, std::integral_constant<int, 1>{});
                }
            }
            asm volatile("" ::: "memory");
            if (lane == 0) *(xr_lds_int)(uintptr_t)(ctl_addr + 16 + 4 * w) = Gbase + nch;
            asm volatile("" ::: "memory");
            Gbase += nch;
            CPROBE(tid == 0, 2 + 4 * ci);
            if (ci > 0) lds_wait(8 * ci);
            char* red = smem + XC_RING;
#pragma unroll
            for (int t = 0; t < 4; ++t)
                if (t != w) {
                    char* sp = red + (w * 4 + t) * XR_SLOT + lane * 16;
#pragma unroll
                    for (int q = 0; q < 4; ++q) {
                        f32x4 v = {acc[t][4 * q], acc[t][4 * q + 1], acc[t][4 * q + 2], acc[t][4 * q + 3]};
                        *reinterpret_cast<f32x4*>(sp + q * 1024) = v;
                    }
                }
            lds_arrive();
            lds_wait(8 * ci + 4);
            CPROBE(tid == 0, 3 + 4 * ci);
            f32x16 own;
#pragma unroll
            for (int t = 0; t < 4; ++t)
                if (t == w) own = acc[t];
            f32x16 sum;
#pragma unroll
            for (int s = 0; s < 4; ++s) {
                f32x16 part;
                const char* sp = red + (s * 4 + w) * XR_SLOT + lane * 16;
#pragma unroll
                for (int q = 0; q < 4; ++q) {
                    const f32x4 v = *reinterpret_cast<const f32x4*>(sp + q * 1024);
                    part[4 * q] = v[0]; part[4 * q + 1] = v[1]; part[4 * q + 2] = v[2]; part[4 * q + 3] = v[3];
                }
                const bool mine = s == w;
#pragma unroll
                for (int r = 0; r < 16; ++r) {
                    const float p = mine ? own[r] : part[r];
                    sum[r] = s == 0 ? p : sum[r] + p;
                }
            }
            lds_arrive();
            xr_epilogue<EP, 16>(d, sum, 0, n, gy0 + 2 * w, gx0, lane, red + (w * 4 + w) * XR_SLOT);
            asm volatile("s_waitcnt vmcnt(0)" ::: "memory");
            if (lane == 0) __hip_atomic_store((gu8*)((char*)a.state + flag_off + ci * 4 + w), (unsigned char)eb, __ATOMIC_RELAXED, __HIP_MEMORY_SCOPE_AGENT);
            CPROBE(tid == 0, 4 + 4 * ci);
        }
    }
    __syncthreads();
    if (tid == 0) {
        const unsigned done = atomicAdd(a.state + 1, 1u);
        if (done == gridDim.x - 1) {
            __hip_atomic_store(a.state + 0, 0u, __ATOMIC_RELAXED, __HIP_MEMORY_SCOPE_AGENT);
            __hip_atomic_store(a.state + 1, 0u, __ATOMIC_RELAXED, __HIP_MEMORY_SCOPE_AGENT);
            __hip_atomic_fetch_add(a.state + 2, 1u, __ATOMIC_RELAXED, __HIP_MEMORY_SCOPE_AGENT);
        }
    }
    CPROBE(tid == 0, 31);
}

template <int EP>
int launch_x3c(const ssr_chain_args& a, int blocks, hipStream_t st) {
    auto kern = conv_x3c_kernel<EP>;
    static bool attr_done[SSR_MAX_DEVICES] = {};
    const int dev = ssr_device_ordinal();
    if (!attr_done[dev]) {
        hipError_t e = hipFuncSetAttribute(reinterpret_cast<const void*>(kern), hipFuncAttributeMaxDynamicSharedMemorySize, XC_LDS);
        if (e != hipSuccess) return (int)e;
        attr_done[dev] = true;
    }
    hipLaunchKernelGGL(kern, dim3(blocks), dim3(XR_NTHR), XC_LDS, st, a);
    SSR_LAUNCH_CHECK();
    return SSR_OK;
}

bool overlap(const ssr_view& a, int na, const ssr_view& b, int nb) {
    return a.p && b.p && a.p == b.p && a.coff < b.coff + nb && b.coff < a.coff + na;
}

}

bool ssr_conv_x3r_shape_ok(const ssr_conv_desc& d);
void ssr_conv_x3r_instance(const ssr_conv_desc& d, int* ntw, int* nu, int* ep);

extern "C" int64_t ssr_conv2d_chain_state_bytes(int32_t N, int32_t Gh, int32_t Gw) {
    return XC_STATE_HDR + (int64_t)N * ((Gw + 15) / 16) * ((Gh + 7) / 8) * 16;
}

extern "C" int ssr_conv2d_chain_ok(const ssr_conv_desc* ds, int32_t n) {
    static const bool off = [] { const char* e = getenv("SSR_X3_CHAIN"); return e && e[0] == '0'; }();
    if (off || !ds || n < 2 || n > XC_MAXN) return 0;
    int ep0 = -1;
    for (int k = 0; k < n; ++k) {
        const ssr_conv_desc& d = ds[k];
        if (d.dtype != SSR_F32X3 || !ssr_conv_x3r_shape_ok(d) || d.CoutPad != 32 || d.Cout > 32) return 0;
        if (d.N != ds[0].N || d.Hi != ds[0].Hi || d.Wi != ds[0].Wi || d.Gh != ds[0].Gh || d.Gw != ds[0].Gw) return 0;
        if ((d.Cin % 16) != 0 || (d.x2.p && (d.Cin2 % 16) != 0) || (d.Cin + d.Cin2) / 16 > XC_MAXCH || d.Cin + d.Cin2 < 16) return 0;
        int nt = 0, nu = 0, ep = 3;
        ssr_conv_x3r_instance(d, &nt, &nu, &ep);
        if (ep == XR_EP_GENERIC || (ep0 >= 0 && ep != ep0)) return 0;
        ep0 = ep;
        for (int j = 0; j < k; ++j) {
            if (overlap(d.y, d.Cout, ds[j].y, ds[j].Cout)) return 0;
            if (overlap(d.y, d.Cout, ds[j].x, ds[j].Cin) || (ds[j].x2.p && overlap(d.y, d.Cout, ds[j].x2, ds[j].Cin2))) return 0;
        }
        if (overlap(d.y, d.Cout, d.x, d.Cin) || (d.x2.p && overlap(d.y, d.Cout, d.x2, d.Cin2))) return 0;
        if (d.r1.p || d.r2.p) return 0;
        if (d.m.p) for (int j = 0; j < n; ++j) if (overlap(ds[j].y, ds[j].Cout, d.m, d.Cout)) return 0;
    }
    const int tiles = ((ds[0].Gw + 15) / 16) * ((ds[0].Gh + 7) / 8);
    if (tiles > 64) return 0;
    for (int k = 0; k < n; ++k) {
        const ssr_conv_desc& d = ds[k];
        const int nch = (d.Cin + d.Cin2) / 16;
        int first_dep = -1, last_free = -1, prev = -2;
        bool asc = true, desc = true;
        for (int c = 0; c < nch; ++c) {
            const bool in_x = c * 16 < d.Cin;
            ssr_view v = in_x ? d.x : d.x2;
            v.coff += in_x ? c * 16 : c * 16 - d.Cin;
            int dep = -1;
            for (int j = 0; j < k; ++j)
                if (overlap(v, 16, ds[j].y, ds[j].Cout)) {
                    if (dep >= 0) return 0;
                    if (v.coff < ds[j].y.coff || v.coff + 16 > ds[j].y.coff + ds[j].Cout) return 0;
                    dep = j;
                }
            if (c > 0) {
                if (dep < prev) asc = false;
                if (dep > prev) desc = false;
            }
            prev = dep;
            (void)first_dep; (void)last_free;
        }
        if (!asc && !desc) return 0;
    }
    return 1;
}

extern "C" int ssr_conv2d_chain(const ssr_conv_desc* ds, int32_t n, void* state, void* stream) {
    if (!ds || n <= 0) return SSR_EINVAL;
    hipStream_t st = reinterpret_cast<hipStream_t>(stream);
    if (!state || !ssr_conv2d_chain_ok(ds, n)) {
        for (int k = 0; k < n; ++k) {
            const int rc = ssr_conv2d(ds + k, stream);
            if (rc != SSR_OK) return rc;
        }
        return SSR_OK;
    }
    ssr_chain_args a{};
    a.n = n;
    a.tiles_x = (ds[0].Gw + 15) / 16;
    a.tiles_y = (ds[0].Gh + 7) / 8;
    a.state = reinterpret_cast<uint32_t*>(state);
    int ep = 3, nt = 0, nu = 0;
    for (int k = 0; k < n; ++k) {
        a.d[k] = ds[k];
        const ssr_conv_desc& d = ds[k];
        const int nch = (d.Cin + d.Cin2) / 16;
        a.nch[k] = nch;
        int firstd = -1;
        for (int c = 0; c < nch; ++c) {
            const bool in_x = c * 16 < d.Cin;
            ssr_view v = in_x ? d.x : d.x2;
            v.coff += in_x ? c * 16 : c * 16 - d.Cin;
            int dep = -1;
            for (int j = 0; j < k; ++j)
                if (overlap(v, 16, ds[j].y, ds[j].Cout)) dep = j;
            a.dep[k][c] = (int8_t)dep;
            if (c == 0) firstd = dep;
        }
        a.rev[k] = (int8_t)((nch > 1 && firstd > a.dep[k][nch - 1]) ? 1 : 0);
        ssr_conv_x3r_instance(d, &nt, &nu, &ep);
    }
    const int blocks = a.tiles_x * a.tiles_y * ds[0].N;
    switch (ep) {
        case XR_EP_LRELU: return launch_x3c<XR_EP_LRELU>(a, blocks, st);
        case XR_EP_LIN: return launch_x3c<XR_EP_LIN>(a, blocks, st);
        case XR_EP_MASK: return launch_x3c<XR_EP_MASK>(a, blocks, st);
        default: return SSR_EUNSUP;
    }
}
```

satlas_super_resolution_amd/engine.py:

```python
from __future__ import annotations

import ctypes as C
import math
import os
from collections import OrderedDict
from dataclasses import dataclass
from typing import Dict, List, Optional, Tuple

import torch

from . import hip
from .hip import ConvDesc, View, WgradItem, WgradLayer, PackItem, SNItem, SNBwdItem, ReduceItem, view


def rup(a: int, b: int) -> int:
    return (a + b - 1) // b * b


def ck_of(dt: int) -> int:
    return 32 if dt == hip.BF16 else 16


@dataclass
class ConvSpec:
# ... 128 lines not shown
        with torch.no_grad():
            for key in self.offsets:
                if key in sd:
                    self.tensor(key).copy_(sd[key].to(self.device, torch.float32))
                elif strict:
                    raise KeyError(key)
            for n in self.sn_names:
                if n + ".weight_u" in sd:
                    self.u[n].copy_(sd[n + ".weight_u"].to(self.device, torch.float32))
                    self.v[n].copy_(sd[n + ".weight_v"].to(self.device, torch.float32))
                elif strict:
                    raise KeyError(n + ".weight_u")

    def state_dict(self) -> "OrderedDict[str, torch.Tensor]":
        out = OrderedDict()
        for s in self.specs.values():
            if s.sn:
                out[s.name + ".weight_orig"] = self.tensor(s.name + ".weight_orig").clone()
                out[s.name + ".weight_u"] = self.u[s.name].clone()
                out[s.name + ".weight_v"] = self.v[s.name].clone()
            else:
                out[s.name + ".weight"] = self.tensor(s.name + ".weight").clone()
            if s.bias:
                out[s.name + ".bias"] = self.tensor(s.name + ".bias").clone()
        return out

    def pack(self):
        hip.check(hip.lib().ssr_pack_weights(self.pack_table.data_ptr(), len(self._pack_items), self.fwd_dtype,
                                             hip.stream_ptr()), "ssr_pack_weights")
        if self._pack_items_bwd is not None:
            hip.check(hip.lib().ssr_pack_weights(self.pack_table_bwd.data_ptr(), len(self._pack_items_bwd), self.dtype,
                                                 hip.stream_ptr()), "ssr_pack_weights (backward layouts)")
        if self._seg_items:
            if self.seg_table is None:
                self.seg_table = hip.device_table(self._seg_items)
            hip.check(hip.lib().ssr_pack_dgrad_gather(self.seg_table.data_ptr(), len(self._seg_items), self.dtype,
                                                      hip.stream_ptr()), "ssr_pack_dgrad_gather")

    def add_repack(self, name: str, ck: int) -> torch.Tensor:
        key = (name, ck)
        if key in self.repacked:
            return self.repacked[key]
        s = self.specs[name]
        cout_pad, cin_pad = rup(s.cout, 32), rup(rup(s.cin, 8), ck)
        buf = torch.zeros(s.k * s.k * cout_pad * cin_pad, dtype=hip.torch_dtype(self.dtype), device=self.device)
        woff, _ = self.offsets[name + (".weight_orig" if s.sn else ".weight")]
        inv = (self.sigma.data_ptr() + 4 * self.sn_names.index(name)) if s.sn else None
        self._pack_items.append(PackItem(self.data.data_ptr() + 4 * woff, inv, buf.data_ptr(), None, s.cout, s.cin, s.k, s.k,
                                         s.stride, cout_pad, cin_pad, rup(s.cin, 32), rup(rup(s.cout, 8), ck), ck, ck))
        self.pack_table = hip.device_table(self._pack_items)
        self.repacked[key] = buf
        return buf

    def add_rdb_gather(self, prefix: str, nf: int, gc: int, a5: float, ck0: int = 0):
        tdt = hip.torch_dtype(self.dtype)
        if ck0 and (prefix, "k0", ck0) not in self.gather:
            K = 4 * gc + nf
            rows_pad, kpad = rup(nf, 32), rup(K, ck0)
            buf = torch.zeros(kpad * 9 * rows_pad, dtype=tdt, device=self.device)
            self.gather[(prefix, "k0", ck0)] = buf
            for jj in range(1, 6):
                cout_j = nf if jj == 5 else gc
                self._seg_items.append(hip.PackSeg(self.ptr(f"{prefix}.conv{jj}.weight"), buf.data_ptr(),
                                                   a5 if jj == 5 else 1.0, cout_j, nf + (jj - 1) * gc, 0, nf,
                                                   (jj - 1) * gc, rows_pad, ck0))
            self.seg_table = None
        if (prefix, 0) in self.gather:
            return
        ck = hip.lib().ssr_conv2d_ck(self.dtype, 3)
        for k in range(5):
            nout = nf if k == 0 else gc
            ci0 = 0 if k == 0 else nf + (k - 1) * gc
            K = (4 - k) * gc + nf
            rows_pad, kpad = rup(nout, 32), rup(K, ck)
            buf = torch.zeros(kpad * 9 * rows_pad, dtype=tdt, device=self.device)
            self.gather[(prefix, k)], self.gather_rows[(prefix, k)] = buf, rows_pad
            for jj in range(k + 1, 6):
                cout_j = nf if jj == 5 else gc
                cin_j = nf + (jj - 1) * gc
                self._seg_items.append(hip.PackSeg(self.ptr(f"{prefix}.conv{jj}.weight"), buf.data_ptr(),
                                                   a5 if jj == 5 else 1.0, cout_j, cin_j, ci0, nout,
                                                   (jj - k - 1) * gc, rows_pad, ck))
        self.seg_table = None

    def spectral_norm(self, power_iter: bool):
        if self.sn_names:
            hip.check(hip.lib().ssr_spectral_norm(self.sn_table.data_ptr(), len(self.sn_names), self.sn_max_rows,
                                                  self.sn_max_cols, 1 if power_iter else 0, hip.stream_ptr()),
                      "ssr_spectral_norm")

    def spectral_norm_backward(self):
        if self.sn_names:
            hip.check(hip.lib().ssr_spectral_norm_bwd(self.sn_bwd_table.data_ptr(), len(self.sn_names),
                                                      self.sn_max_elems, hip.stream_ptr()), "ssr_spectral_norm_bwd")
            hip.check(hip.lib().ssr_fill(self.grad_sn.data_ptr(), self.grad_sn.numel(), hip.F32, 0.0, hip.stream_ptr()), "ssr_fill")


class Launcher:

    FORK, JOIN = object(), object()

    def __init__(self):
        self.calls = []
        self._sides = {}

    def add(self, fn, *args, what=""):
        self.calls.append((fn, args, what))

    def fork(self, sub: "Launcher", what=""):
        self.calls.append((Launcher.FORK, (sub,), what))

    def join(self):
        self.calls.append((Launcher.JOIN, (), "join"))

    def flat_calls(self):
        for fn, args, what in self.calls:
            if fn is Launcher.FORK:
                yield from args[0].flat_calls()
            elif fn is not Launcher.JOIN:
                yield fn, args, what

    def run(self):
        st = hip.stream_ptr()
        for fn, args, what in self.calls:
            if fn is Launcher.FORK:
                side = self._sides.get(id(args[0]))
                if side is None:
                    side = self._sides[id(args[0])] = torch.cuda.Stream()
                side.wait_stream(torch.cuda.current_stream())
                with torch.cuda.stream(side):
                    args[0].run()
                continue
            if fn is Launcher.JOIN:
                for side in self._sides.values():
                    torch.cuda.current_stream().wait_stream(side)
                continue
            rc = fn(*args, st)
            if rc != 0:
                hip.check(rc, what or getattr(fn, "__name__", "call"))

    def __len__(self):
        return len(self.calls)


class _ConvBuilder:

    def __init__(self, store: ParamStore, N: int):
        self.store, self.N, self.dt = store, N, store.dtype
        self.keep = []
        self.packed_fwd, self.packed_dgrad = store.packed_fwd, store.packed_dgrad

    def conv(self, L: Launcher, name: str, x: View, hi: int, wi: int, y: View, *, up=1, act=hip.ACT_NONE, alpha=1.0,
             y0: View = hip.NULL_VIEW, r1: View = hip.NULL_VIEW, r1_nc=0, beta1=0.0, r2: View = hip.NULL_VIEW,
             r2_nc=0, beta2=0.0, cin: Optional[int] = None):
        s = self.store.specs[name]
        cout_pad, _, _, _ = self.store.pad[name]
        d = ConvDesc()
        d.dtype = self.store.fwd_dtype
        d.x, d.N, d.Hi, d.Wi, d.up = x, self.N, hi, wi, up
        d.Cin = rup(s.cin, 8) if cin is None else cin
        d.w = self.packed_fwd[name].data_ptr()
        d.CoutPad = cout_pad
        d.bias = self.store.ptr(name + ".bias") if s.bias else None
        d.KH = d.KW = s.k
        d.stride = s.stride
        d.pad_y = d.pad_x = 1
        lh, lw = hi * up, wi * up
        d.Gh, d.Gw = (lh // s.stride, lw // s.stride)
        d.Ho, d.Wo, d.oys, d.oyo, d.oxs, d.oxo = d.Gh, d.Gw, 1, 0, 1, 0
        d.Cout = s.cout
        d.y, d.y0, d.y1 = y, y0, hip.NULL_VIEW
        d.alpha, d.act = alpha, act
        d.r1, d.r1_nc, d.beta1 = r1, r1_nc, beta1
        d.r2, d.r2_nc, d.beta2 = r2, r2_nc, beta2
        d.accumulate = 0
        d.m, d.m_c0, d.m_c1 = hip.NULL_VIEW, 0, 0
        d.s2d = 1 if self.store.s2d.get(name) else 0
        self.keep.append(d)
        fix = (self.store.fwd_dtype == hip.F32X3 and act == hip.ACT_LRELU and s.stride == 1 and s.k == 3 and alpha == 1.0 and not y0.p
               and not r1.p and not r2.p and X3_FIXUP[0])
        if fix:
            d.fix_list = self._fix_list()
            d.fix_cap, d.fix_thr = X3_FIX_CAP, X3_FIX_THR[0]
            d.w_ref, d.w_ref_cin = self.store.ptr(name + (".weight_orig" if s.sn else ".weight")), s.cin
            d.w_ref_sigma = (self.store.sigma.data_ptr() + 4 * self.store.sn_names.index(name)) if s.sn else None
        L.add(hip.lib().ssr_conv2d, C.byref(d), what=f"conv fwd {name}")
        if fix:
            L.add(hip.lib().ssr_conv2d_fixup, C.byref(d), what=f"lrelu decision fix-up {name}")
        return d

    def _fix_list(self) -> int:
        words = 4 + 2 * X3_FIX_CAP
        if not getattr(self, "_fix_pool", None) or self._fix_used == self._fix_pool[-1].shape[0]:
            self._fix_pool = getattr(self, "_fix_pool", []) + [torch.zeros(64, words, dtype=torch.int32, device=self.store.device)]
            self._fix_used = 0
        self._fix_used += 1
        return self._fix_pool[-1][self._fix_used - 1].data_ptr()

    def fix_high_water(self) -> int:
        return max([int(p[:, 2].max()) for p in getattr(self, "_fix_pool", [])] or [0])

    def dgrad(self, L: Launcher, name: str, dy: View, gh: int, gw: int, y: View, *, cout: Optional[int] = None,
              alpha=1.0, y1: View = hip.NULL_VIEW, r1: View = hip.NULL_VIEW, r1_nc=0, beta1=0.0,
              r2: View = hip.NULL_VIEW, r2_nc=0, beta2=0.0, accumulate=0, m: View = hip.NULL_VIEW, m_c0=0, m_c1=0,
              cin_dy: Optional[int] = None, m_relu=0):
        s = self.store.specs[name]
        _, _, cin_pad_o, cout_pad_i = self.store.pad[name]
        wbase = self.packed_dgrad[name].data_ptr()
        esz = 2 if self.dt == hip.BF16 else 4
        classes = [(0, 0)] if s.stride == 1 else [(0, 0), (0, 1), (1, 0), (1, 1)]
        arr = (ConvDesc * len(classes))()
        for ic, (py, px) in enumerate(classes):
            d = arr[ic]
            d.dtype = self.dt
            d.x, d.N, d.Hi, d.Wi, d.up = dy, self.N, gh, gw, 1
            d.Cin = rup(s.cout, 8) if cin_dy is None else cin_dy
            d.CoutPad = cin_pad_o
            d.bias = None
            d.Cout = s.cin if cout is None else cout
            if s.stride == 1:
                d.w = wbase
                d.KH = d.KW = s.k
                d.stride, d.pad_y, d.pad_x = 1, 1, 1
                d.Gh, d.Gw = gh, gw
                d.Ho, d.Wo, d.oys, d.oyo, d.oxs, d.oxo = gh, gw, 1, 0, 1, 0
            else:
                cls = py * 2 + px
                d.w = wbase + cls * 4 * cin_pad_o * cout_pad_i * esz
                d.KH = d.KW = 2
                d.stride, d.pad_y, d.pad_x = 1, 1 - py, 1 - px
                d.Gh, d.Gw = gh, gw
                d.Ho, d.Wo, d.oys, d.oyo, d.oxs, d.oxo = 2 * gh, 2 * gw, 2, py, 2, px
            d.y, d.y0, d.y1 = y, hip.NULL_VIEW, y1
            d.alpha, d.act = alpha, hip.ACT_NONE
            d.r1, d.r1_nc, d.beta1 = r1, r1_nc, beta1
            d.r2, d.r2_nc, d.beta2 = r2, r2_nc, beta2
            d.accumulate = accumulate
            d.m, d.m_c0, d.m_c1 = m, m_c0, m_c1
            d.m_relu = m_relu
        self.keep.append(arr)
        if len(classes) == 1:
            L.add(hip.lib().ssr_conv2d, C.byref(arr[0]), what=f"conv dgrad {name}")
        else:
            L.add(hip.lib().ssr_conv2d_batch, arr, len(classes), what=f"conv dgrad {name}")


def gather_dgrad(cb: "_ConvBuilder", L: Launcher, prefix: str, k: int, x1: View, c1: int, x2: View, c2: int, gh: int,
                 gw: int, y: View, cout: int, **epi):
    st = cb.store
    d = ConvDesc()
    d.dtype = cb.dt
    d.N, d.Hi, d.Wi, d.up = cb.N, gh, gw, 1
    if c1 > 0:
        d.x, d.Cin, d.x2, d.Cin2 = x1, c1, x2, c2
    else:
        d.x, d.Cin, d.x2, d.Cin2 = x2, c2, hip.NULL_VIEW, 0
    d.w = st.gather[(prefix, k)].data_ptr()
    d.CoutPad = st.gather_rows[(prefix, k)]
    d.bias = None
    d.KH = d.KW = 3
    d.stride, d.pad_y, d.pad_x = 1, 1, 1
    d.Gh, d.Gw = gh, gw
    d.Ho, d.Wo, d.oys, d.oyo, d.oxs, d.oxo = gh, gw, 1, 0, 1, 0
    d.Cout = cout
    d.y, d.y0, d.y1 = y, hip.NULL_VIEW, hip.NULL_VIEW
    d.alpha, d.act = 1.0, hip.ACT_NONE
    d.r1, d.r1_nc, d.beta1 = epi.get("r1", hip.NULL_VIEW), epi.get("r1_nc", 0), epi.get("beta1", 0.0)
    d.r2, d.r2_nc, d.beta2 = epi.get("r2", hip.NULL_VIEW), epi.get("r2_nc", 0), epi.get("beta2", 0.0)
    d.accumulate = 0
    d.m, d.m_c0, d.m_c1 = epi.get("m", hip.NULL_VIEW), epi.get("m_c0", 0), epi.get("m_c1", 0)
    cb.keep.append(d)
    L.add(hip.lib().ssr_conv2d, C.byref(d), what=f"conv dgrad-gather {prefix}.slice{k}")
    return d


X3_FIXUP = [os.environ.get("SSR_X3_FIXUP", "0") == "1"]
X3_FIX_THR = [float(os.environ.get("SSR_X3_FIX_THR", "1e-4"))]
X3_FIX_CAP = 8192

_DET = [os.environ.get("SSR_DETERMINISTIC", "0") == "1"]


def deterministic() -> bool:
    return _DET[0]


class deterministic_mode:
    def __init__(self, on: bool):
        self.on = bool(on)

    def __enter__(self):
        self.prev, _DET[0] = _DET[0], (self.on or _DET[0])

    def __exit__(self, *a):
        _DET[0] = self.prev


_CUS = None


def _device_cus():
    global _CUS
    if _CUS is None:
        n = torch.cuda.get_device_properties(torch.cuda.current_device()).multi_processor_count if torch.cuda.is_available() else 256
        _CUS = (int(n), 8 if n % 32 == 0 and n >= 64 else 1)
    return _CUS


class WgradBatch:

    MAX_TILES_PER_ITEM = {3: int(os.environ.get("SSR_WGRAD_T3", "128")), 4: int(os.environ.get("SSR_WGRAD_T4", "64"))}

    def __init__(self, dtype: int, k: int, stride: int, force_atomic: bool = False, det: Optional[bool] = None):
        self.dtype, self.k, self.stride = dtype, k, stride
        self.force_atomic = force_atomic
        fused = dtype == hip.F32X3 and ((k == 3 and stride == 1 and os.environ.get("SSR_X3_WGRAD_FUSED", "1") == "1")
                                        or (k == 4 and stride == 2 and os.environ.get("SSR_X3_WGRAD_FUSED4", "1") == "1"))
        self.kdt = hip.F32X3 if fused else hip.BF16 if dtype == hip.F32X3 else dtype
        self.layers: List[WgradLayer] = []
        self.items: List[WgradItem] = []
        self.layer_tab = self.item_tab = None
        self.split_tabs: List[torch.Tensor] = []
        self.split_tab = None
        self.splits: List[Tuple[torch.Tensor, torch.Tensor, torch.Tensor]] = []
        self.det = deterministic() if det is None else bool(det)
        assert not (self.det and force_atomic), "deterministic mode: no second launch may accumulate into the same gradients concurrently"
        self.virtual = set()
        self._partials = []
        self.partial = self.reduce_tab = None
        self.n_reduce = self.max_reduce = 0

    def add(self, x: View, dy: View, N, hi, wi, up, cin, cout, gh, gw, alpha, dw_ptr, cin_w, db_ptr):
        li = len(self.layers)
        self.layers.append(WgradLayer(x, dy, N, hi, wi, up, cin, cout, 1, 1, gh, gw, alpha, dw_ptr, cin_w, db_ptr))
        tiles = hip.lib().ssr_wgrad_tiles(N, gh, gw, self.kdt, self.k)
        splits = max(1, -(-tiles // (self.MAX_TILES_PER_ITEM.get(self.k, 128) * (2 if self.kdt == hip.F32X3 else 1))))
        per = -(-tiles // splits)
        lsp = [li] * splits
        if self.det and splits > 1:
            lsp = []
            for sp in range(splits):
                lsp.append(len(self.layers))
                self.virtual.add(len(self.layers))
                self.layers.append(WgradLayer(x, dy, N, hi, wi, up, cin, cout, 1, 1, gh, gw, alpha, None, cin_w, None))
            self._partials.append((dw_ptr, db_ptr, cout * cin_w * self.k * self.k, cout if db_ptr else 0, lsp))
        for co0 in range(0, cout, 32):
            for ci0 in range(0, cin_w, hip.lib().ssr_wgrad_ci_tile(self.kdt, self.k)):
                for sp in range(splits):
                    b, e = sp * per, min(tiles, (sp + 1) * per)
                    if b < e:
                        atomic = 1 if ((splits > 1 and not self.det) or self.force_atomic) else 0
                        self.items.append(WgradItem(lsp[sp], co0, ci0, b, e, atomic, 1, lsp[sp], co0))

    def _weight(self, it):
        L = self.layers[it.layer]
        return (it.tile_end - it.tile_begin) * (2 if L.Cin_w - it.ci0 > 32 else 1) * max(1, it.nco)

    COST_TILE = {2: 5900, 1: 4300}
    COST_WRITEOUT = 25000

    @property
    def N_CU(self):
        return _device_cus()[0]

    @property
    def N_XCD(self):
        return _device_cus()[1]

    def _cost(self, it):
        nco = max(1, it.nco)
        return (it.tile_end - it.tile_begin) * self.COST_TILE[nco] + nco * self.COST_WRITEOUT

    def _makespan(self, items):
        import heapq
        free = [0] * self.N_CU
        for c in sorted((self._cost(it) for it in items), reverse=True):
            heapq.heapreplace(free, free[0] + c)
        return max(free)

    def _balance(self, items):
        def cut(its, t_pair, t_single):
            out = []
            for it in its:
                n, t = it.tile_end - it.tile_begin, (t_pair if it.nco == 2 else t_single)
                parts = max(1, -(-n // t))
                per = -(-n // parts)
                for b in range(it.tile_begin, it.tile_end, per):
                    out.append(WgradItem(it.layer, it.co0, it.ci0, b, min(it.tile_end, b + per), 1 if parts > 1 else it.atomic,
                                         it.nco, it.layer_b, it.co0_b))
            return out
        best = None
        for t_pair in (128, 64, 32):
            for t_single in (128, 64, 32, 16):
                cand = cut(items, t_pair, t_single)
                m = self._makespan(cand)
                if best is None or m < best[0] * 0.98:
                    best = (m, cand, t_pair, t_single)
# ... 106 lines not shown
            self.layer_tab = hip.device_table(self.layers)
            return
        for xi, dyi, with_bias in ((0, 0, True), (0, 1, True), (1, 0, False)):
            tab = []
            for L in self.layers:
                tab.append(WgradLayer(self._twin(L.x, xi), self._twin(L.dy, dyi), L.N, L.Hi, L.Wi, L.up, L.Cin, L.Cout, L.pad_y,
                                      L.pad_x, L.Gh, L.Gw, L.alpha, L.dw, L.Cin_w, L.db if with_bias else None))
            self.split_tabs.append(hip.device_table(tab))
        self.layer_tab = self.split_tabs[0]

    def launch(self, L: Launcher):
        if not self.layers:
            return
        lib = hip.lib()
        if self.partial is not None:
            L.add(lib.ssr_fill, self.partial.data_ptr(), self.partial.numel(), hip.F32, 0.0, what="zero wgrad partials")
        self._launch_wgrad(L, lib)
        if self.partial is not None:
            L.add(lib.ssr_wgrad_reduce, self.reduce_tab.data_ptr(), self.n_reduce, self.max_reduce, what="wgrad partials -> grad (fixed order)")

    def _launch_wgrad(self, L: Launcher, lib):
        if self.dtype == hip.F32X3 and self.kdt == hip.BF16:
            if all(p.numel() % 8 == 0 for p, _, _ in self.splits):
                if self.split_tab is None:
                    self.split_tab = hip.device_table([hip.SplitItem(p.data_ptr(), h.data_ptr(), l.data_ptr(), p.numel()) for p, h, l in self.splits])
                L.add(lib.ssr_split_bf16_multi, self.split_tab.data_ptr(), len(self.splits), max(p.numel() for p, _, _ in self.splits),
                      what="split bf16")
            else:
                for parent, hi_t, lo_t in self.splits:
                    L.add(lib.ssr_split_bf16, parent.data_ptr(), hi_t.data_ptr(), lo_t.data_ptr(), parent.numel(), what="split bf16")
            for tab in self.split_tabs:
                L.add(lib.ssr_conv2d_wgrad, tab.data_ptr(), self.item_tab.data_ptr(), len(self.items), hip.BF16, self.k, self.k,
                      self.stride, what="wgrad batch (split pass)")
            return
        L.add(lib.ssr_conv2d_wgrad, self.layer_tab.data_ptr(), self.item_tab.data_ptr(), len(self.items),
              self.kdt, self.k, self.k, self.stride, what="wgrad batch")


def generator_specs(num_in_ch, num_out_ch=3, scale=4, num_feat=64, num_block=23, num_grow_ch=32) -> List[ConvSpec]:
    if scale == 2:
        num_in_ch *= 4
    elif scale == 1:
        num_in_ch *= 16
    nf, gc = num_feat, num_grow_ch
    specs = [ConvSpec("conv_first", nf, num_in_ch)]
    for i in range(num_block):
        for j in (1, 2, 3):
            for k in range(1, 5):
                specs.append(ConvSpec(f"body.{i}.rdb{j}.conv{k}", gc, nf + (k - 1) * gc, dgrad_packed=False))
            specs.append(ConvSpec(f"body.{i}.rdb{j}.conv5", nf, nf + 4 * gc, dgrad_packed=False))
    specs.append(ConvSpec("conv_body", nf, nf))
    specs.append(ConvSpec("conv_up1", nf, nf))
    specs.append(ConvSpec("conv_up2", nf, nf))
    if scale in (8, 16):
        specs.append(ConvSpec("conv_up3", nf, nf))
        if scale == 16:
            specs.append(ConvSpec("conv_up4", nf, nf))
    specs.append(ConvSpec("conv_hr", nf, nf))
    specs.append(ConvSpec("conv_last", num_out_ch, nf))
    return specs


class GeneratorPlan:

    def _link_rdb_prefetch(self, descs):
        esz = 2
        if os.environ.get("SSR_RDB_PREFETCH", "0") != "1":
            return
        for cur, nxt in zip(descs[:-1], descs[1:]):
            for k in range(5):
                cur.w_next[k] = nxt.w[k]
                cin = self.nf + k * self.gc
                cur.w_next_bytes[k] = 9 * cin * (self.nf if k == 4 else self.gc) * esz

    def __init__(self, store: ParamStore, B: int, H: int, W: int, *, num_in_ch, num_out_ch=3, scale=4, num_feat=64,
                 num_block=23, num_grow_ch=32, training=True, out_buf: Optional[torch.Tensor] = None,
                 d_out_buf: Optional[torch.Tensor] = None, need_input_grad=False, wgrad_atomic: bool = False,
                 bwd_segments: int = 1):
        self.store, self.B, self.dt = store, B, store.dtype
        self.det = deterministic()
        self.scale, self.nf, self.nb, self.gc = scale, num_feat, num_block, num_grow_ch
        self.num_in_ch, self.num_out_ch = num_in_ch, num_out_ch
        self.unshuffle = 2 if scale == 2 else 4 if scale == 1 else 1
        assert H % self.unshuffle == 0 and W % self.unshuffle == 0
        self.Hin, self.Win = H, W
        H, W = H // self.unshuffle, W // self.unshuffle
        self.H, self.W = H, W
        self.cin_eff = num_in_ch * self.unshuffle ** 2
        assert num_feat % 8 == 0 and num_grow_ch % 8 == 0, "num_feat/num_grow_ch must be multiples of 8"
        self.training = training
        tdt, dev = hip.torch_dtype(self.dt), store.device
        nf, gc, nb = self.nf, self.gc, self.nb
        cd = nf + 4 * gc
        z = lambda *s: torch.zeros(*s, dtype=tdt, device=dev)
        self.n_up = {1: 2, 2: 2, 4: 2, 8: 3, 16: 4}[scale] if scale in (1, 2, 4, 8, 16) else 2
        self.up_names = [f"conv_up{i + 1}" for i in range(self.n_up)]
        self.Ho, self.Wo = H * (1 << self.n_up), W * (1 << self.n_up)
        self.xin = z(B, H, W, rup(self.cin_eff, 8))
        n_rdb = 3 * nb
        n_bufs = n_rdb if training else min(n_rdb, 4)
        self.bufs = [z(B, H, W, cd) for _ in range(n_bufs)]
        self.body_out = z(B, H, W, nf)
        self.trunk = z(B, H, W, nf)
        self.ups = [z(B, H << (i + 1), W << (i + 1), nf) for i in range(self.n_up)]
        self.hr = z(B, self.Ho, self.Wo, nf)
        self.out = out_buf if out_buf is not None else z(B, self.Ho, self.Wo, rup(num_out_ch, 8))
        assert self.out.shape[:3] == (B, self.Ho, self.Wo)
        cb = self._cb = _ConvBuilder(store, B)
        self._cb = cb
        self._chain_state = None
        if (self.dt == hip.F32X3 and nf == 64 and gc == 32 and not X3_FIXUP[0] and os.environ.get("SSR_X3_CHAIN", "0") == "1"):
            nbytes = int(hip.lib().ssr_conv2d_chain_state_bytes(B, H, W))
            self._chain_state = torch.zeros((nbytes + 3) // 4, dtype=torch.int32, device=dev)
        F = Launcher()
        buf = lambda r: self.bufs[r % n_bufs]
        self.feat = self.bufs[0] if n_bufs == n_rdb else z(B, H, W, nf)
        cb.conv(F, "conv_first", view(self.xin), H, W, view(buf(0), 0),
                y0=hip.NULL_VIEW if n_bufs == n_rdb else view(self.feat))
        self.fused_rdb = (self.dt == hip.BF16 and nf == 64 and gc == 32 and os.environ.get("SSR_FUSED_RDB", "1") != "0")
        self._rdb_descs = []
        for r in range(n_rdb):
            i, j = divmod(r, 3)
            p = f"body.{i}.rdb{j + 1}"
            cur = buf(r)
            dst = view(self.body_out) if r == n_rdb - 1 else view(buf(r + 1), 0)
            if self.fused_rdb:
                rd = hip.RdbDesc()
                rd.dtype, rd.N, rd.H, rd.W = self.dt, B, H, W
                rd.inp, rd.slices, rd.out, rd.mask = view(cur, 0), view(cur, 0), dst, hip.NULL_VIEW
                for k in range(5):
                    rd.w[k] = store.packed_fwd[f"{p}.conv{k + 1}"].data_ptr()
                    rd.bias[k] = store.ptr(f"{p}.conv{k + 1}.bias")
                rd.w[4] = store.add_repack(f"{p}.conv5", 16).data_ptr()
                if j < 2:
                    rd.alpha5, rd.beta1, rd.r2, rd.beta2 = 0.2, 1.0, hip.NULL_VIEW, 0.0
                else:
                    rd.alpha5, rd.beta1, rd.r2, rd.beta2 = 0.04, 0.2, view(buf(r - 2), 0), 1.0
                self._rdb_descs.append(rd)
                F.add(hip.lib().ssr_rdb_forward, C.byref(rd), what=f"rdb fwd {p}")
                continue
            tmp = Launcher() if self._chain_state is not None else F
            ds = [cb.conv(tmp, f"{p}.conv{k}", view(cur, 0), H, W, view(cur, nf + (k - 1) * gc), act=hip.ACT_LRELU,
                          cin=nf + (k - 1) * gc) for k in range(1, 5)]
            if tmp is not F:
                self._add_chain(F, ds, f"conv chain fwd {p}.conv1-4")
            if j < 2:
                cb.conv(F, f"{p}.conv5", view(cur, 0), H, W, dst, alpha=0.2, r1=view(cur, 0), r1_nc=nf, beta1=1.0,
                        cin=cd)
            else:
                cb.conv(F, f"{p}.conv5", view(cur, 0), H, W, dst, alpha=0.04, r1=view(cur, 0), r1_nc=nf, beta1=0.2,
                        r2=view(buf(r - 2), 0), r2_nc=nf, beta2=1.0, cin=cd)
        self._link_rdb_prefetch(self._rdb_descs)
        cb.conv(F, "conv_body", view(self.body_out), H, W, view(self.trunk), r1=view(self.feat, 0), r1_nc=nf, beta1=1.0)
        src, sh, sw = self.trunk, H, W
        for i, nm in enumerate(self.up_names):
            cb.conv(F, nm, view(src), sh, sw, view(self.ups[i]), up=2, act=hip.ACT_LRELU)
            src, sh, sw = self.ups[i], sh * 2, sw * 2
        cb.conv(F, "conv_hr", view(src), sh, sw, view(self.hr), act=hip.ACT_LRELU)
        cb.conv(F, "conv_last", view(self.hr), sh, sw, view(self.out))
        self.fwd = F
        if not training:
            return
        assert n_bufs == n_rdb
        self.d_out = d_out_buf if d_out_buf is not None else z(B, self.Ho, self.Wo, self.out.shape[-1])
        assert self.d_out.shape == self.out.shape
        self.g_hr = z(B, self.Ho, self.Wo, nf)
        self.g_ups = [z(B, H << (i + 1), W << (i + 1), nf) for i in range(self.n_up)]
        self.g_tmp = [z(B, H << (i + 1), W << (i + 1), nf) for i in range(self.n_up)]
        self.g_trunk = z(B, H, W, nf)
        self.g_body_out = z(B, H, W, nf)
        self.dbufs = [z(B, H, W, cd) for _ in range(n_rdb)]
        self.g_xin = z(B, H, W, self.xin.shape[-1]) if need_input_grad else None
        Bk = Launcher()
        st = store
        n_chunks = max(1, int(os.environ.get("SSR_WGRAD_CHUNKS", "1")))
        n_seg = max(1, int(bwd_segments))
        if n_seg > 1:
            n_chunks = n_seg
        cuts = {round(n_rdb * q / n_chunks) for q in range(1, n_chunks)}
        batches = [WgradBatch(self.dt, 3, 1, wgrad_atomic, det=self.det)]
        self.bwd_segments = []
        seg_state = {"launcher": Bk, "hi": st.numel}

        def add_wg(name, x: View, dy: View, hi, wi, up, gh, gw, alpha=1.0, cin=None):
            s = st.specs[name]
            batches[-1].add(x, dy, B, hi, wi, up, rup(s.cin, 8) if cin is None else cin, s.cout, gh, gw, alpha,
                            st.ptr(name + ".weight", st.grad), s.cin, st.ptr(name + ".bias", st.grad) if s.bias else None)

        def close_batch(next_first_key=None):
            nonlocal Bk
            wgb = batches[-1]
            wgb.finalize()
            if n_seg > 1:
                wgb.launch(Bk)
                lo = st.offsets[next_first_key][0] if next_first_key else 0
                hi = seg_state["hi"]
                assert 0 <= lo < hi <= st.numel, (next_first_key, lo, hi)
                g0, esz = st.grad.data_ptr(), st.grad.element_size()
                for iw, Lw in enumerate(wgb.layers):
                    if iw in wgb.virtual:
                        continue
                    for ptr in (Lw.dw, Lw.db):
                        if ptr:
                            off = (int(ptr) - g0) // esz
                            assert lo <= off < hi, f"weight gradient at arena offset {off} outside its segment [{lo}, {hi})"
                self.bwd_segments.append((Bk, lo, hi - lo))
                seg_state["hi"] = lo
                Bk = Launcher()
            else:
                sub = Launcher()
                wgb.launch(sub)
                Bk.fork(sub, what="wgrad chunk")
            batches.append(WgradBatch(self.dt, 3, 1, wgrad_atomic, det=self.det))

        Ho, Wo = self.Ho, self.Wo
        last_up = self.ups[-1]
        add_wg("conv_last", view(self.hr), view(self.d_out), Ho, Wo, 1, Ho, Wo)
        cb.dgrad(Bk, "conv_last", view(self.d_out), Ho, Wo, view(self.g_hr), m=view(self.hr), m_c0=0, m_c1=nf)
        add_wg("conv_hr", view(last_up), view(self.g_hr), Ho, Wo, 1, Ho, Wo)
        cb.dgrad(Bk, "conv_hr", view(self.g_hr), Ho, Wo, view(self.g_ups[-1]), m=view(last_up), m_c0=0, m_c1=nf)
        for i in reversed(range(self.n_up)):
            nm = self.up_names[i]
            hh, ww = H << (i + 1), W << (i + 1)
            src = self.ups[i - 1] if i > 0 else self.trunk
            add_wg(nm, view(src), view(self.g_ups[i]), hh // 2, ww // 2, 2, hh, ww)
            cb.dgrad(Bk, nm, view(self.g_ups[i]), hh, ww, view(self.g_tmp[i]))
            if i > 0:
                Bk.add(hip.lib().ssr_nearest2x_bwd, view(self.g_tmp[i]), hip.NULL_VIEW, hip.NULL_VIEW,
                       view(self.g_ups[i - 1]), view(self.ups[i - 1]), self.dt, B, hh // 2, ww // 2, nf,
                       what="nearest2x_bwd")
            else:
                Bk.add(hip.lib().ssr_nearest2x_bwd, view(self.g_tmp[i]), hip.NULL_VIEW, hip.NULL_VIEW,
                       view(self.g_trunk), hip.NULL_VIEW, self.dt, B, H, W, nf, what="nearest2x_bwd")
        add_wg("conv_body", view(self.body_out), view(self.g_trunk), H, W, 1, H, W)
        cb.dgrad(Bk, "conv_body", view(self.g_trunk), H, W, view(self.g_body_out))
        bwd_descs = []
        for r in reversed(range(n_rdb)):
            i, j = divmod(r, 3)
            p = f"body.{i}.rdb{j + 1}"
            cur, dcur = self.bufs[r], self.dbufs[r]
            d_out_r = view(self.g_body_out) if r == n_rdb - 1 else view(self.dbufs[r + 1], 0)
            if j == 2:
                d_rrdb = d_out_r
                a5, b5 = 0.04, 0.2
            else:
                rr = 3 * i + 2
                d_rrdb = view(self.g_body_out) if rr == n_rdb - 1 else view(self.dbufs[rr + 1], 0)
                a5, b5 = 0.2, 1.0
            fused_bwd = self.fused_rdb and os.environ.get("SSR_FUSED_RDB_BWD", "1") != "0"
            if n_chunks > 1 and (r + 1) in cuts:
                ir, jr = divmod(r + 1, 3)
                close_batch(f"body.{ir}.rdb{jr + 1}.conv1.weight")
            store.add_rdb_gather(p, nf, gc, a5, ck0=16 if fused_bwd else 0)
            add_wg(f"{p}.conv5", view(cur, 0), d_out_r, H, W, 1, H, W, alpha=a5, cin=cd)
            for k in (4, 3, 2, 1):
                add_wg(f"{p}.conv{k}", view(cur, 0), view(dcur, nf + (k - 1) * gc), H, W, 1, H, W,
                       cin=nf + (k - 1) * gc)
            if fused_bwd:
                rd = hip.RdbDesc()
                rd.dtype, rd.N, rd.H, rd.W = self.dt, B, H, W
                rd.inp, rd.slices, rd.out, rd.mask = d_out_r, view(dcur, 0), view(dcur, 0), view(cur, 0)
                for jj in range(5):
                    rd.w[jj] = store.gather[(p, 4 - jj)].data_ptr()
                    rd.bias[jj] = None
                rd.w[4] = store.gather[(p, "k0", 16)].data_ptr()
                rd.alpha5, rd.beta1 = 1.0, b5
                rd.r2, rd.beta2 = (d_rrdb, 1.0) if j == 0 else (hip.NULL_VIEW, 0.0)
                self._rdb_descs.append(rd)
                bwd_descs.append(rd)
                Bk.add(hip.lib().ssr_rdb_backward, C.byref(rd), what=f"rdb bwd {p}")
                continue
            tmp = Launcher() if self._chain_state is not None else Bk
            ds = [gather_dgrad(cb, tmp, p, k, view(dcur, nf + k * gc), (4 - k) * gc, d_out_r, nf, H, W,
                               view(dcur, nf + (k - 1) * gc), gc, m=view(cur, nf + (k - 1) * gc), m_c0=0, m_c1=gc) for k in (4, 3, 2, 1)]
            if tmp is not Bk:
                self._add_chain(Bk, ds, f"conv chain dgrad-gather {p}.slice4-1")
            kw = dict(r1=d_out_r, r1_nc=nf, beta1=b5)
            if j == 0:
                kw.update(r2=d_rrdb, r2_nc=nf, beta2=1.0)
            gather_dgrad(cb, Bk, p, 0, view(dcur, nf), 4 * gc, d_out_r, nf, H, W, view(dcur, 0), nf, **kw)
        self._link_rdb_prefetch(bwd_descs)
        Bk.add(hip.lib().ssr_add_views, view(self.dbufs[0], 0), view(self.g_trunk), self.dt, B * H * W, nf,
               what="add d_trunk")
        add_wg("conv_first", view(self.xin), view(self.dbufs[0], 0), H, W, 1, H, W, cin=self.xin.shape[-1])
        if need_input_grad:
            cb.dgrad(Bk, "conv_first", view(self.dbufs[0], 0), H, W, view(self.g_xin), cout=self.xin.shape[-1],
                     cin_dy=nf)
        if n_chunks > 1:
            close_batch()
            if n_seg == 1:
                Bk.join()
            batches.pop()
        else:
            batches[0].finalize()
            batches[0].launch(Bk)
        self._wg_batches = batches
        if n_seg > 1:
            whole = Launcher()
            for L, _, _ in self.bwd_segments:
                whole.calls.extend(L.calls)
            self.bwd = whole
            assert sum(n for _, _, n in self.bwd_segments) == st.numel and self.bwd_segments[-1][1] == 0
        else:
            self.bwd = Bk

    def _add_chain(self, L: Launcher, descs, what: str):
        arr = (ConvDesc * len(descs))()
        for i, d in enumerate(descs):
            C.memmove(C.byref(arr[i]), C.byref(d), C.sizeof(ConvDesc))
        self._cb.keep.append(arr)
        L.add(hip.lib().ssr_conv2d_chain, arr, len(descs), self._chain_state.data_ptr(), what=what)

    def load_input(self, x_nchw: torch.Tensor, scale: float = 1.0):
        assert x_nchw.dtype == torch.float32 and x_nchw.is_contiguous() and x_nchw.is_cuda
        assert tuple(x_nchw.shape) == (self.B, self.num_in_ch, self.Hin, self.Win), x_nchw.shape
        hip.check(hip.lib().ssr_nchw_to_nhwc(x_nchw.data_ptr(), self.B, self.num_in_ch, self.Hin, self.Win,
                                             view(self.xin), self.dt, self.unshuffle, 1, scale, hip.stream_ptr()),
                  "ssr_nchw_to_nhwc")

    def read_output(self, out_nchw: Optional[torch.Tensor] = None) -> torch.Tensor:
        if out_nchw is None:
            out_nchw = torch.empty(self.B, self.num_out_ch, self.Ho, self.Wo, device=self.store.device)
        hip.check(hip.lib().ssr_nhwc_to_nchw(view(self.out), self.dt, out_nchw.data_ptr(), self.B, self.num_out_ch,
                                             self.Ho, self.Wo, hip.stream_ptr()), "ssr_nhwc_to_nchw")
        return out_nchw

    def load_output_grad(self, g_nchw: torch.Tensor):
        hip.check(hip.lib().ssr_nchw_to_nhwc(g_nchw.data_ptr(), self.B, self.num_out_ch, self.Ho, self.Wo,
                                             view(self.d_out), self.dt, 1, 1, 1.0, hip.stream_ptr()),
                  "ssr_nchw_to_nhwc")

    def read_input_grad(self) -> torch.Tensor:
        g = torch.empty(self.B, self.cin_eff, self.H, self.W, device=self.store.device)
        hip.check(hip.lib().ssr_nhwc_to_nchw(view(self.g_xin), self.dt, g.data_ptr(), self.B, self.cin_eff, self.H,
                                             self.W, hip.stream_ptr()), "ssr_nhwc_to_nchw")
        return g


class SplitGeneratorPlan:

    def __init__(self, store: ParamStore, B: int, H: int, W: int, *, out_buf: torch.Tensor, d_out_buf: torch.Tensor, parts: int = 2,
                 **kw):
        assert B % parts == 0 and kw.get("training", True)
        h = B // parts
        self.B, self.half, self.store = B, h, store
        self.parts = [GeneratorPlan(store, h, H, W, out_buf=out_buf[i * h:(i + 1) * h], d_out_buf=d_out_buf[i * h:(i + 1) * h],
                                    wgrad_atomic=True, **kw) for i in range(parts)]
        a = self.parts[0]
        self.fused_rdb, self.unshuffle = a.fused_rdb, a.unshuffle
        self.num_in_ch, self.num_out_ch, self.Hin, self.Win, self.Ho, self.Wo = a.num_in_ch, a.num_out_ch, a.Hin, a.Win, a.Ho, a.Wo
        self.out, self.dt = out_buf, a.dt
        self.fwd, self.bwd = Launcher(), Launcher()
        for L, which in ((self.fwd, "fwd"), (self.bwd, "bwd")):
            for p in self.parts[1:]:
                L.fork(getattr(p, which), what="another part of the batch")
            L.calls.extend(getattr(a, which).calls)
            L.join()

    def load_input(self, x_nchw: torch.Tensor, scale: float = 1.0):
        for i, p in enumerate(self.parts):
            p.load_input(x_nchw[i * self.half:(i + 1) * self.half], scale)

    def read_output(self, out_nchw: Optional[torch.Tensor] = None) -> torch.Tensor:
        if out_nchw is None:
            out_nchw = torch.empty(self.B, self.num_out_ch, self.Ho, self.Wo, device=self.store.device)
        for i, p in enumerate(self.parts):
            p.read_output(out_nchw[i * self.half:(i + 1) * self.half])
        return out_nchw


def discriminator_specs(num_in_ch, num_feat=64, in_hw: Optional[Tuple[int, int]] = None, dtype: Optional[int] = None) -> List[ConvSpec]:
    nf = num_feat
    min_rows = 16 if dtype in (hip.F32X3, hip.F32H3, hip.F32H) else 24
    grid = lambda k: None if in_hw is None or min(in_hw[0] >> k, in_hw[1] >> k) >= min_rows else False
    return _disc_specs(num_in_ch, nf, grid)


def _disc_specs(num_in_ch, nf, grid) -> List[ConvSpec]:
    return [
        ConvSpec("conv0", nf, num_in_ch, 3, 1, True, False),
        ConvSpec("conv1", nf * 2, nf, 4, 2, False, True, s2d=grid(1)),
        ConvSpec("conv2", nf * 4, nf * 2, 4, 2, False, True, s2d=grid(2)),
        ConvSpec("conv3", nf * 8, nf * 4, 4, 2, False, True, s2d=grid(3)),
        ConvSpec("conv4", nf * 4, nf * 8, 3, 1, False, True),
        ConvSpec("conv5", nf * 2, nf * 4, 3, 1, False, True),
        ConvSpec("conv6", nf, nf * 2, 3, 1, False, True),
        ConvSpec("conv7", nf, nf, 3, 1, False, True),
        ConvSpec("conv8", nf, nf, 3, 1, False, True),
        ConvSpec("conv9", 1, nf, 3, 1, True, False),
    ]


class DiscriminatorPlan:

    def __init__(self, store: ParamStore, B: int, H: int, W: int, *, num_in_ch, num_feat=64, skip_connection=True,
                 training=True):
        assert H % 8 == 0 and W % 8 == 0, "U-Net discriminator needs H, W divisible by 8"
        assert num_feat % 8 == 0
        self.store, self.B, self.H, self.W, self.dt = store, B, H, W, store.dtype
        self.det = deterministic()
        self.nf, self.skip, self.cd = num_feat, skip_connection, num_in_ch
        self.cdp = rup(num_in_ch, 8)
        tdt, dev = hip.torch_dtype(self.dt), store.device
        nf = num_feat
        z = lambda *s: torch.zeros(*s, dtype=tdt, device=dev)
        H2, W2, H4, W4, H8, W8 = H // 2, W // 2, H // 4, W // 4, H // 8, W // 8
        self.x0, self.x1, self.x2, self.x3 = z(B, H, W, nf), z(B, H2, W2, 2 * nf), z(B, H4, W4, 4 * nf), z(B, H8, W8, 8 * nf)
        self.u3, self.a4 = z(B, H4, W4, 8 * nf), z(B, H4, W4, 4 * nf)
        self.u4, self.a5 = z(B, H2, W2, 4 * nf), z(B, H2, W2, 2 * nf)
        self.u5, self.a6 = z(B, H, W, 2 * nf), z(B, H, W, nf)
        self.x6 = z(B, H, W, nf) if skip_connection else self.a6
        self.o7, self.o8 = z(B, H, W, nf), z(B, H, W, nf)
        self.logits = z(B, H, W, 8)
        self._cb = _ConvBuilder(store, B)
        self._fwd_cache: Dict[Tuple[int, int], Launcher] = {}
        self._bwd_cache: Dict[Tuple, Launcher] = {}
        self.training = training
        if training:
            self.d_logits = z(B, H, W, 8)
            self.g_o8, self.g_o7 = z(B, H, W, nf), z(B, H, W, nf)
            self.g_a6, self.g_x6 = z(B, H, W, nf), (z(B, H, W, nf) if skip_connection else None)
            self.g_u5 = z(B, H, W, 2 * nf)
            self.g_a5, self.g_x5 = z(B, H2, W2, 2 * nf), (z(B, H2, W2, 2 * nf) if skip_connection else None)
            self.g_u4 = z(B, H2, W2, 4 * nf)
            self.g_a4, self.g_x4 = z(B, H4, W4, 4 * nf), (z(B, H4, W4, 4 * nf) if skip_connection else None)
            self.g_u3 = z(B, H4, W4, 8 * nf)
            self.g3, self.g2, self.g1, self.g0 = z(B, H8, W8, 8 * nf), z(B, H4, W4, 4 * nf), z(B, H2, W2, 2 * nf), z(B, H, W, nf)
            self.g_in = z(B, H, W, self.cdp)

    def forward_plan(self, x_buf: torch.Tensor) -> Launcher:
        key = x_buf.data_ptr()
        if key in self._fwd_cache:
            return self._fwd_cache[key]
        assert tuple(x_buf.shape) == (self.B, self.H, self.W, self.cdp), (x_buf.shape, self.cdp)
        cb, nf, B, H, W, dt = self._cb, self.nf, self.B, self.H, self.W, self.dt
        H2, W2, H4, W4, H8, W8 = H // 2, W // 2, H // 4, W // 4, H // 8, W // 8
        L = Launcher()
        lib = hip.lib()
        LR = hip.ACT_LRELU
        cb.conv(L, "conv0", view(x_buf), H, W, view(self.x0), act=LR, cin=self.cdp)
        cb.conv(L, "conv1", view(self.x0), H, W, view(self.x1), act=LR)
        cb.conv(L, "conv2", view(self.x1), H2, W2, view(self.x2), act=LR)
        cb.conv(L, "conv3", view(self.x2), H4, W4, view(self.x3), act=LR)
        L.add(lib.ssr_bilinear2x_fwd, view(self.x3), hip.NULL_VIEW, view(self.u3), dt, B, H8, W8, 8 * nf,
              what="bilinear u3")
        cb.conv(L, "conv4", view(self.u3), H4, W4, view(self.a4), act=LR)
        L.add(lib.ssr_bilinear2x_fwd, view(self.a4), view(self.x2) if self.skip else hip.NULL_VIEW, view(self.u4), dt,
              B, H4, W4, 4 * nf, what="bilinear u4")
        cb.conv(L, "conv5", view(self.u4), H2, W2, view(self.a5), act=LR)
        L.add(lib.ssr_bilinear2x_fwd, view(self.a5), view(self.x1) if self.skip else hip.NULL_VIEW, view(self.u5), dt,
              B, H2, W2, 2 * nf, what="bilinear u5")
        if self.skip:
            cb.conv(L, "conv6", view(self.u5), H, W, view(self.x6), act=LR, y0=view(self.a6), r1=view(self.x0),
                    r1_nc=nf, beta1=1.0)
        else:
            cb.conv(L, "conv6", view(self.u5), H, W, view(self.a6), act=LR)
        cb.conv(L, "conv7", view(self.x6), H, W, view(self.o7), act=LR)
        cb.conv(L, "conv8", view(self.o7), H, W, view(self.o8), act=LR)
        cb.conv(L, "conv9", view(self.o8), H, W, view(self.logits))
        self._fwd_cache[key] = L
        return L

    def backward_plan(self, x_buf: torch.Tensor, param_grads: bool, input_grad: bool,
                      in_residual: Optional[torch.Tensor] = None) -> Launcher:
        key = (x_buf.data_ptr(), param_grads, 1 if input_grad else 0, 0 if in_residual is None else in_residual.data_ptr())
        if key in self._bwd_cache:
            return self._bwd_cache[key]
        cb, st, nf, B, H, W, dt = self._cb, self.store, self.nf, self.B, self.H, self.W, self.dt
        H2, W2, H4, W4, H8, W8 = H // 2, W // 2, H // 4, W // 4, H // 8, W // 8
        lib = hip.lib()
        L = Launcher()
        wg3, wg4 = WgradBatch(dt, 3, 1, det=self.det), WgradBatch(dt, 4, 2, det=self.det)

        def add_wg(name, x, dy, hi, wi, gh, gw, cin=None):
            if not param_grads:
                return
            s = st.specs[name]
            arena = st.grad_sn if s.sn else st.grad
            (wg3 if s.k == 3 else wg4).add(x, dy, B, hi, wi, 1, rup(s.cin, 8) if cin is None else cin, s.cout, gh, gw,
                                           1.0, st.ptr(st.wkey(name), arena), s.cin,
                                           st.ptr(name + ".bias", st.grad) if s.bias else None)

        NV = hip.NULL_VIEW
        add_wg("conv9", view(self.o8), view(self.d_logits), H, W, H, W)
        cb.dgrad(L, "conv9", view(self.d_logits), H, W, view(self.g_o8), m=view(self.o8), m_c0=0, m_c1=nf)
        add_wg("conv8", view(self.o7), view(self.g_o8), H, W, H, W)
        cb.dgrad(L, "conv8", view(self.g_o8), H, W, view(self.g_o7), m=view(self.o7), m_c0=0, m_c1=nf)
        add_wg("conv7", view(self.x6), view(self.g_o7), H, W, H, W)
        cb.dgrad(L, "conv7", view(self.g_o7), H, W, view(self.g_a6), y1=view(self.g_x6) if self.skip else NV,
                 m=view(self.a6), m_c0=0, m_c1=nf)
        add_wg("conv6", view(self.u5), view(self.g_a6), H, W, H, W)
        cb.dgrad(L, "conv6", view(self.g_a6), H, W, view(self.g_u5))
        L.add(lib.ssr_bilinear2x_bwd, view(self.g_u5), NV, view(self.g_x5) if self.skip else NV, view(self.g_a5),
              view(self.a5), dt, B, H2, W2, 2 * nf, what="bilinear bwd 5")
        add_wg("conv5", view(self.u4), view(self.g_a5), H2, W2, H2, W2)
        cb.dgrad(L, "conv5", view(self.g_a5), H2, W2, view(self.g_u4))
        L.add(lib.ssr_bilinear2x_bwd, view(self.g_u4), NV, view(self.g_x4) if self.skip else NV, view(self.g_a4),
              view(self.a4), dt, B, H4, W4, 4 * nf, what="bilinear bwd 4")
        add_wg("conv4", view(self.u3), view(self.g_a4), H4, W4, H4, W4)
        cb.dgrad(L, "conv4", view(self.g_a4), H4, W4, view(self.g_u3))
        L.add(lib.ssr_bilinear2x_bwd, view(self.g_u3), NV, NV, view(self.g3), view(self.x3), dt, B, H8, W8, 8 * nf,
              what="bilinear bwd 3")
        sk = lambda t: (view(t) if self.skip else NV)
        add_wg("conv3", view(self.x2), view(self.g3), H4, W4, H8, W8)
        cb.dgrad(L, "conv3", view(self.g3), H8, W8, view(self.g2), r1=sk(self.g_x4), r1_nc=4 * nf, beta1=1.0,
                 m=view(self.x2), m_c0=0, m_c1=4 * nf)
        add_wg("conv2", view(self.x1), view(self.g2), H2, W2, H4, W4)
        cb.dgrad(L, "conv2", view(self.g2), H4, W4, view(self.g1), r1=sk(self.g_x5), r1_nc=2 * nf, beta1=1.0,
                 m=view(self.x1), m_c0=0, m_c1=2 * nf)
        add_wg("conv1", view(self.x0), view(self.g1), H, W, H2, W2)
        cb.dgrad(L, "conv1", view(self.g1), H2, W2, view(self.g0), r1=sk(self.g_x6), r1_nc=nf, beta1=1.0,
                 m=view(self.x0), m_c0=0, m_c1=nf)
        add_wg("conv0", view(x_buf), view(self.g0), H, W, H, W, cin=self.cdp)
        if input_grad:
            kw = {}
            if in_residual is not None:
                kw.update(r1=view(in_residual), r1_nc=self.cdp, beta1=1.0)
            cb.dgrad(L, "conv0", view(self.g0), H, W, view(self.g_in), cout=self.cdp, cin_dy=nf, **kw)
        wg3.finalize(); wg4.finalize()
        wg3.launch(L); wg4.launch(L)
        self._keep = getattr(self, "_keep", []) + [wg3, wg4]
        self._bwd_cache[key] = L
        return L
```

satlas_super_resolution_amd/hip.py:

```python
from __future__ import annotations

import ctypes as C
import os
from typing import Optional

import torch

_HERE = os.path.dirname(os.path.abspath(__file__))
LIB_PATH = os.path.join(_HERE, "libssr_hip.so")

F32, BF16, F32X3 = 0, 1, 2
F32H3 = 3
ACT_NONE, ACT_LRELU, ACT_RELU = 0, 1, 2
DETERMINISTIC = 0x200
LOSS_SLOTS = 256
SN_BWD_SLOTS = 64
BILINEAR_FLAT = 0x100


class HipLibraryError(RuntimeError):
    pass


class View(C.Structure):
    _fields_ = [("p", C.c_void_p), ("cs", C.c_int32), ("coff", C.c_int32)]


NULL_VIEW = View(None, 0, 0)


class ConvDesc(C.Structure):
    _fields_ = [
        ("dtype", C.c_int32),
        ("x", View), ("N", C.c_int32), ("Hi", C.c_int32), ("Wi", C.c_int32), ("up", C.c_int32), ("Cin", C.c_int32),
        ("x2", View), ("Cin2", C.c_int32),
        ("w", C.c_void_p), ("CoutPad", C.c_int32), ("bias", C.c_void_p),
        ("KH", C.c_int32), ("KW", C.c_int32), ("stride", C.c_int32), ("pad_y", C.c_int32), ("pad_x", C.c_int32),
        ("Gh", C.c_int32), ("Gw", C.c_int32),
        ("Ho", C.c_int32), ("Wo", C.c_int32), ("oys", C.c_int32), ("oyo", C.c_int32), ("oxs", C.c_int32),
        ("oxo", C.c_int32), ("Cout", C.c_int32),
        ("y", View), ("y0", View), ("y1", View),
        ("alpha", C.c_float), ("act", C.c_int32),
        ("r1", View), ("r1_nc", C.c_int32), ("beta1", C.c_float),
        ("r2", View), ("r2_nc", C.c_int32), ("beta2", C.c_float),
        ("accumulate", C.c_int32),
        ("m", View), ("m_c0", C.c_int32), ("m_c1", C.c_int32),
        ("s2d", C.c_int32), ("m_relu", C.c_int32),
        ("fix_list", C.c_void_p), ("fix_cap", C.c_int32), ("fix_thr", C.c_float), ("w_ref", C.c_void_p), ("w_ref_sigma", C.c_void_p),
        ("w_ref_cin", C.c_int32),
    ]


class RdbDesc(C.Structure):
    _fields_ = [("dtype", C.c_int32), ("N", C.c_int32), ("H", C.c_int32), ("W", C.c_int32),
                ("inp", View), ("slices", View), ("out", View), ("mask", View), ("w", C.c_void_p * 5), ("bias", C.c_void_p * 5),
                ("alpha5", C.c_float), ("beta1", C.c_float), ("r2", View), ("beta2", C.c_float),
                ("w_next", C.c_void_p * 5), ("w_next_bytes", C.c_int32 * 5), ("tile", C.c_int32)]


class WgradLayer(C.Structure):
    _fields_ = [
        ("x", View), ("dy", View),
        ("N", C.c_int32), ("Hi", C.c_int32), ("Wi", C.c_int32), ("up", C.c_int32), ("Cin", C.c_int32),
        ("Cout", C.c_int32), ("pad_y", C.c_int32), ("pad_x", C.c_int32), ("Gh", C.c_int32), ("Gw", C.c_int32),
        ("alpha", C.c_float), ("dw", C.c_void_p), ("Cin_w", C.c_int32), ("db", C.c_void_p),
    ]


class WgradItem(C.Structure):
    _fields_ = [("layer", C.c_int32), ("co0", C.c_int32), ("ci0", C.c_int32), ("tile_begin", C.c_int32),
                ("tile_end", C.c_int32), ("atomic", C.c_int32), ("nco", C.c_int32), ("layer_b", C.c_int32), ("co0_b", C.c_int32)]


class PackItem(C.Structure):
    _fields_ = [
        ("src", C.c_void_p), ("inv_scale", C.c_void_p), ("dst_fwd", C.c_void_p), ("dst_dgrad", C.c_void_p),
        ("Cout", C.c_int32), ("Cin", C.c_int32), ("KH", C.c_int32), ("KW", C.c_int32), ("stride", C.c_int32),
        ("CoutPad", C.c_int32), ("CinPad", C.c_int32), ("CinPadO", C.c_int32), ("CoutPadI", C.c_int32),
        ("ck_fwd", C.c_int32), ("ck_dgrad", C.c_int32), ("fwd_s2d", C.c_int32),
    ]


class PackSeg(C.Structure):
    _fields_ = [("src", C.c_void_p), ("dst", C.c_void_p), ("scale", C.c_float), ("Cout", C.c_int32), ("Cin", C.c_int32),
                ("ci0", C.c_int32), ("nci", C.c_int32), ("kbase", C.c_int32), ("rows_pad", C.c_int32), ("ck", C.c_int32)]


class SNItem(C.Structure):
    _fields_ = [("w", C.c_void_p), ("u", C.c_void_p), ("v", C.c_void_p), ("sigma", C.c_void_p), ("tmp", C.c_void_p),
                ("rows", C.c_int32), ("cols", C.c_int32)]


class SNBwdItem(C.Structure):
    _fields_ = [("dw_sn", C.c_void_p), ("w", C.c_void_p), ("u", C.c_void_p), ("v", C.c_void_p), ("sigma", C.c_void_p),
                ("dw", C.c_void_p), ("tmp", C.c_void_p), ("rows", C.c_int32), ("cols", C.c_int32)]


class ReduceItem(C.Structure):
    _fields_ = [("dst", C.c_void_p), ("src", C.c_void_p), ("n", C.c_int64), ("stride", C.c_int64), ("parts", C.c_int32),
                ("pad_", C.c_int32)]


class SplitItem(C.Structure):
    _fields_ = [("x", C.c_void_p), ("hi", C.c_void_p), ("lo", C.c_void_p), ("n", C.c_int64)]


class AdamArgs(C.Structure):
    _fields_ = [("param", C.c_void_p), ("grad", C.c_void_p), ("exp_avg", C.c_void_p), ("exp_avg_sq", C.c_void_p),
                ("ema", C.c_void_p), ("n", C.c_int64), ("lr", C.c_void_p), ("step", C.c_void_p),
                ("beta1", C.c_float), ("beta2", C.c_float), ("eps", C.c_float), ("ema_decay", C.c_float),
                ("grad_scale", C.c_float)]


ABI_SYMBOLS = [
    "ssr_conv2d", "ssr_conv2d_fixup", "ssr_conv2d_batch", "ssr_conv2d_impl", "ssr_conv2d_variant", "ssr_conv2d_symbol", "ssr_conv2d_chain", "ssr_conv2d_chain_ok", "ssr_conv2d_chain_state_bytes", "ssr_conv2d_ck", "ssr_conv2d_s2d_ok", "ssr_rdb_forward", "ssr_rdb_backward", "ssr_rdb_tile_of", "ssr_conv2d_wgrad", "ssr_wgrad_reduce", "ssr_wgrad_tiles", "ssr_wgrad_ci_tile", "ssr_wgrad_co_tile", "ssr_pack_weights", "ssr_pack_dgrad_gather", "ssr_add_views", "ssr_nchw_to_nhwc", "ssr_nhwc_to_nchw",
    "ssr_fill", "ssr_bilinear2x_fwd", "ssr_bilinear2x_bwd", "ssr_nearest2x_bwd", "ssr_spectral_norm",
    "ssr_spectral_norm_bwd", "ssr_usm_sharp", "ssr_l1_loss", "ssr_bce_logits_loss", "ssr_adam_step", "ssr_axpby_f32",
    "ssr_quantize_u8", "ssr_metric_shift_sums", "ssr_metric_ssim_sums", "ssr_split_bf16", "ssr_split_bf16_multi", "ssr_channel_affine", "ssr_relu_maxpool2_fwd", "ssr_relu_maxpool2_bwd",
    "ssr_gram_splits", "ssr_gram_fwd", "ssr_gram_l1", "ssr_gram_bwd",
    "ssr_nonfinite_scan", "ssr_adam_step_guarded", "ssr_quantize_u8_checked",
    "ssr_scene_zero_scan", "ssr_scene_gather", "ssr_scene_scatter_u8",
    "ssr_scene_zero_scan_at", "ssr_scene_gather_at", "ssr_scene_blend_add", "ssr_scene_blend_finish",
    "ssr_scene_gather_bands",
    "ssr_device_info", "ssr_abi_version",
]
SCAN_MAX_RANGES = 8

_lib: Optional[C.CDLL] = None


def lib() -> C.CDLL:
    global _lib
    if _lib is not None:
        return _lib
    if not os.path.exists(LIB_PATH):
        raise HipLibraryError(
            f"{LIB_PATH} not found: build it with `python -c 'import __graft_entry__ as g; g.build()'` "
            "(hipcc --offload-arch=gfx950).  There is no CPU fallback for the product path.")
    try:
        l = C.CDLL(LIB_PATH)
    except OSError as e:
        raise HipLibraryError(f"cannot load {LIB_PATH}: {e}") from e
    vp, i32, i64, f32 = C.c_void_p, C.c_int32, C.c_int64, C.c_float
    l.ssr_conv2d.argtypes = [C.POINTER(ConvDesc), vp]
    l.ssr_conv2d_fixup.argtypes = [C.POINTER(ConvDesc), vp]
    l.ssr_conv2d_impl.argtypes = [C.POINTER(ConvDesc), vp, i32]
    l.ssr_conv2d_batch.argtypes = [C.POINTER(ConvDesc), i32, vp]
    l.ssr_conv2d_variant.argtypes = [C.POINTER(ConvDesc)]
    l.ssr_conv2d_symbol.argtypes = [C.POINTER(ConvDesc), C.c_char_p, i32]
    l.ssr_conv2d_chain.argtypes = [C.POINTER(ConvDesc), i32, vp, vp]
    l.ssr_conv2d_chain_ok.argtypes = [C.POINTER(ConvDesc), i32]
    l.ssr_conv2d_chain_state_bytes.argtypes = [i32, i32, i32]
    l.ssr_conv2d_ck.argtypes = [i32, i32]
    l.ssr_conv2d_s2d_ok.argtypes = [i32, i32, i32, i32]
    l.ssr_rdb_forward.argtypes = [C.POINTER(RdbDesc), vp]
    l.ssr_rdb_backward.argtypes = [C.POINTER(RdbDesc), vp]
    l.ssr_rdb_tile_of.argtypes = [C.POINTER(RdbDesc)]
    l.ssr_conv2d_wgrad.argtypes = [vp, vp, i32, i32, i32, i32, i32, vp]
    l.ssr_wgrad_reduce.argtypes = [vp, i32, i64, vp]
    l.ssr_wgrad_ci_tile.argtypes = [i32, i32]
    l.ssr_wgrad_co_tile.argtypes = [i32, i32]
    l.ssr_wgrad_tiles.argtypes = [i32, i32, i32, i32, i32]
    l.ssr_pack_weights.argtypes = [vp, i32, i32, vp]
    l.ssr_pack_dgrad_gather.argtypes = [vp, i32, i32, vp]
    l.ssr_add_views.argtypes = [View, View, i32, i64, i32, vp]
    l.ssr_nchw_to_nhwc.argtypes = [vp, i32, i32, i32, i32, View, i32, i32, i32, f32, vp]
    l.ssr_nhwc_to_nchw.argtypes = [View, i32, vp, i32, i32, i32, i32, vp]
    l.ssr_fill.argtypes = [vp, i64, i32, f32, vp]
    l.ssr_bilinear2x_fwd.argtypes = [View, View, View, i32, i32, i32, i32, i32, vp]
    l.ssr_bilinear2x_bwd.argtypes = [View, View, View, View, View, i32, i32, i32, i32, i32, vp]
    l.ssr_nearest2x_bwd.argtypes = [View, View, View, View, View, i32, i32, i32, i32, i32, vp]
    l.ssr_spectral_norm.argtypes = [vp, i32, i32, i32, i32, vp]
    l.ssr_spectral_norm_bwd.argtypes = [vp, i32, i32, vp]
    l.ssr_l1_loss.argtypes = [View, View, View, i32, i64, i32, f32, vp, vp]
    l.ssr_usm_sharp.argtypes = [vp, vp, i32, i32, i32, f32, f32, f32, vp]
    l.ssr_bce_logits_loss.argtypes = [View, View, i32, i64, f32, f32, vp, vp, vp]
    l.ssr_adam_step.argtypes = [C.POINTER(AdamArgs), vp]
    l.ssr_axpby_f32.argtypes = [f32, vp, f32, vp, i64, vp]
    l.ssr_quantize_u8.argtypes = [vp, vp, i32, i32, i32, i32, i32, vp]
    l.ssr_metric_shift_sums.argtypes = [vp, vp, i32, i32, i32, i32, i32, vp, vp]
    l.ssr_metric_ssim_sums.argtypes = [vp, vp, i32, i32, i32, i32, vp, vp]
    l.ssr_split_bf16.argtypes = [vp, vp, vp, i64, vp]
    l.ssr_split_bf16_multi.argtypes = [vp, i32, i64, vp]
    l.ssr_channel_affine.argtypes = [View, View, i32, i64, i32, C.POINTER(C.c_float), C.POINTER(C.c_float), i32, vp]
    l.ssr_relu_maxpool2_fwd.argtypes = [View, View, i32, i32, i32, i32, i32, vp]
    l.ssr_relu_maxpool2_bwd.argtypes = [View, View, View, i32, i32, i32, i32, i32, i32, vp]
    l.ssr_gram_splits.argtypes = [i32, i32, i32]
    l.ssr_gram_fwd.argtypes = [View, vp, vp, i32, i32, i32, i32, f32, vp]
    l.ssr_gram_l1.argtypes = [vp, vp, vp, i32, i64, f32, vp, vp]
    l.ssr_gram_bwd.argtypes = [View, vp, View, i32, i32, i32, i32, f32, i32, vp]
    l.ssr_nonfinite_scan.argtypes = [C.POINTER(vp), C.POINTER(i64), i32, vp, vp]
    l.ssr_adam_step_guarded.argtypes = [C.POINTER(AdamArgs), vp, vp, vp]
    l.ssr_quantize_u8_checked.argtypes = [vp, vp, i32, i32, i32, i32, i32, vp, vp]
    l.ssr_scene_zero_scan.argtypes = [vp, i32, i32, i32, vp, vp]
    l.ssr_scene_gather.argtypes = [vp, i32, i32, i32, vp, vp, i32, i32, View, i32, vp]
    l.ssr_scene_scatter_u8.argtypes = [View, i32, vp, i32, i32, vp, i32, i32, vp, vp]
    l.ssr_scene_zero_scan_at.argtypes = [vp, i32, i32, i32, vp, i32, vp, vp]
    l.ssr_scene_gather_at.argtypes = [vp, i32, i32, i32, vp, vp, i32, i32, View, i32, vp]
    l.ssr_scene_blend_add.argtypes = [View, i32, vp, i32, i32, vp, vp, i32, i32, vp, vp]
    l.ssr_scene_blend_finish.argtypes = [vp, vp, vp, i32, vp, i32, i32, vp]
    l.ssr_scene_gather_bands.argtypes = [vp, vp, i32, i32, i32, i32, vp, vp, i32, i32, View, i32, vp]
    l.ssr_device_info.argtypes = [C.c_char_p, i32]
    l.ssr_abi_version.argtypes = []
    for s in ABI_SYMBOLS:
        getattr(l, s).restype = i64 if s == "ssr_conv2d_chain_state_bytes" else i32
    _lib = l
    return l


def check(rc: int, what: str):
    if rc != 0:
        raise HipLibraryError(f"{what} failed with code {rc}"
                              + (" (bad descriptor)" if rc == -1 else " (unsupported)" if rc == -2 else " (hipError)"))


def stream_ptr() -> int:
    return torch.cuda.current_stream().cuda_stream


F32F = 16 + F32X3
F32H = 32 + F32X3


def storage_code(dt: int) -> int:
    return F32X3 if dt in (F32F, F32H) else dt


def forward_code(dt: int) -> int:
    return F32 if dt == F32F else F32H3 if dt == F32H else dt


def torch_dtype(dt: int):
    return torch.bfloat16 if dt == BF16 else torch.float32


def dtype_code(dt) -> int:
    if isinstance(dt, str):
        try:
            return {"fp32": F32, "float32": F32, "bf16": BF16, "bfloat16": BF16, "fp32x3": F32X3, "bf16x3": F32X3, "fp32f": F32F, "fp32h": F32H}[dt]
        except KeyError:
            raise ValueError(f"unsupported compute dtype {dt!r}") from None
    if dt is torch.float32:
        return F32
    if dt is torch.bfloat16:
        return BF16
    if dt in (F32, BF16, F32X3, F32F, F32H):
        return int(dt)
    raise ValueError(f"unsupported compute dtype {dt!r}")


import weakref

_PARENTS = weakref.WeakValueDictionary()


def parent_of(v: "View") -> torch.Tensor:
    return _PARENTS[v.p]


def view(t: Optional[torch.Tensor], coff: int = 0) -> View:
    if t is None:
        return View(None, 0, 0)
    assert t.is_contiguous()
    old = _PARENTS.get(t.data_ptr())
    if old is None or old.numel() < t.numel():
        _PARENTS[t.data_ptr()] = t
    return View(t.data_ptr(), t.shape[-1], coff)


def device_table(items) -> torch.Tensor:
    arr_t = type(items[0]) * len(items)
    arr = arr_t(*items)
    raw = bytes(memoryview(arr).cast("B"))
    host = torch.frombuffer(bytearray(raw), dtype=torch.uint8)
    return host.cuda()


def device_info() -> str:
    buf = C.create_string_buffer(256)
    lib().ssr_device_info(buf, 256)
    return buf.value.decode()


def conv_symbol(desc) -> str:
    buf = C.create_string_buffer(96)
    check(lib().ssr_conv2d_symbol(C.byref(desc), buf, 96), "ssr_conv2d_symbol")
    return buf.value.decode()
```

Before: 1183.

## Store LeakyReLU activation signs as packed bitmasks for backward masking

```diff
diff --git a/include/ssr_hip.h b/include/ssr_hip.h
--- a/include/ssr_hip.h
+++ b/include/ssr_hip.h
@@ -57,9 +57,15 @@
     const float* w_ref;
     const float* w_ref_sigma;
     int32_t w_ref_cin;
+    uint32_t* ybits;
+    int32_t ybits_words;
+    int32_t ybits_s0;
+    const uint32_t* mbits;
+    int32_t mbits_words;
 } ssr_conv_desc;
 
 int ssr_conv2d(const ssr_conv_desc* d, void* stream);
+int ssr_conv2d_bits_ok(const ssr_conv_desc* d);
 int ssr_conv2d_fixup(const ssr_conv_desc* d, void* stream);
 int ssr_conv2d_batch(const ssr_conv_desc* ds, int32_t n, void* stream);
 int ssr_conv2d_impl(const ssr_conv_desc* d, void* stream, int32_t impl);
diff --git a/satlas_super_resolution_amd/csrc/common.h b/satlas_super_resolution_amd/csrc/common.h
--- a/satlas_super_resolution_amd/csrc/common.h
+++ b/satlas_super_resolution_amd/csrc/common.h
@@ -60,7 +60,8 @@
 template <> __device__ __forceinline__ __bf16 from_f32<__bf16>(float v) { return (__bf16)v; }
 
 __device__ __forceinline__ float lrelu(float v) { return v > 0.f ? v : LRELU_SLOPE * v; }
-__device__ __forceinline__ float lrelu_grad_from_out(float out) { return out > 0.f ? 1.f : LRELU_SLOPE; }
+__device__ __forceinline__ bool act_out_positive(float out) { return out > 0.f; }
+__device__ __forceinline__ float lrelu_grad_from_out(float out) { return act_out_positive(out) ? 1.f : LRELU_SLOPE; }
 __device__ __forceinline__ float lrelu_max(float v) {
     float r;
     const float s = LRELU_SLOPE * v;
diff --git a/satlas_super_resolution_amd/csrc/conv.hip b/satlas_super_resolution_amd/csrc/conv.hip
--- a/satlas_super_resolution_amd/csrc/conv.hip
+++ b/satlas_super_resolution_amd/csrc/conv.hip
@@ -811,6 +811,8 @@
 bool ssr_conv_bigx3_try(const ssr_conv_desc& d, hipStream_t st, int* rc, bool force);
 bool ssr_conv_bigx3_qualifies(const ssr_conv_desc& d);
 bool ssr_conv_bigx3_batch_try(const ssr_conv_desc* ds, int n, hipStream_t st, int* rc);
+bool ssr_conv_bigx3_batch_qualifies(const ssr_conv_desc* ds, int n);
+bool ssr_conv_bigx3_shape_ok(const ssr_conv_desc& d);
 bool ssr_conv_x3q_try(const ssr_conv_desc& d, hipStream_t st, int* rc, bool force);
 bool ssr_conv_x3q_qualifies(const ssr_conv_desc& d);
 bool ssr_conv_x3r_try(const ssr_conv_desc& d, hipStream_t st, int* rc, bool force);
@@ -868,8 +870,8 @@
         ssr_conv_x3r_instance(d, &ntw, &nu, &ep);
         snprintf(buf, buflen, "conv_x3r_kernel<%d, %d, %d, %d, %d>", ntw, nu, ep, ssr_conv_x3r_tile_height(d), d.dtype == SSR_F32 ? 1 : d.dtype == SSR_F32H ? 2 : 0);
     } else if (d.dtype == SSR_F32X3 && w == 6) snprintf(buf, buflen, "conv_x3q_kernel<%d>", nt);
-    else if (d.dtype == SSR_F32X3 && w == 9) snprintf(buf, buflen, "conv_bigx3_kernel4<%d>", (d.s2d || d.KH == 2) ? 2 : 3);
-    else if (d.dtype == SSR_F32H && w == 9) snprintf(buf, buflen, "conv_bigh3_kernel4<%d>", (d.s2d || d.KH == 2) ? 2 : 3);
+    else if (d.dtype == SSR_F32X3 && w == 9) snprintf(buf, buflen, "conv_bigx3%s_kernel4<%d>", (d.ybits || d.mbits) ? "b" : "", (d.s2d || d.KH == 2) ? 2 : 3);
+    else if (d.dtype == SSR_F32H && w == 9) snprintf(buf, buflen, "conv_bigh3%s_kernel4<%d>", (d.ybits || d.mbits) ? "b" : "", (d.s2d || d.KH == 2) ? 2 : 3);
     else if (f32m && w == 7) snprintf(buf, buflen, "conv_thin_f32_kernel<%d, %d>", d.Cout == 1 ? 1 : d.Cout <= 3 ? 3 : d.Cout == 4 ? 4 : 8, d.dtype == SSR_F32X3 ? 1 : d.dtype == SSR_F32H ? 2 : 0);
     else snprintf(buf, buflen, "%s<%s,K%d,S%d,NT%d,W%d>", w == 7 ? "conv_thin_kernel" : w == 8 ? "conv_ws_kernel" : w == 9 ? "conv_big_kernel" : w == 1 ? "conv_res_kernel" : d.dtype == SSR_F32X3 ? "conv_x3_kernel" : d.dtype == SSR_F32H ? "conv_h3_kernel" : "conv_kernel",
                   d.dtype == SSR_BF16 ? "bf16" : d.dtype == SSR_F32 ? "fp32" : d.dtype == SSR_F32H ? "fp32h" : "fp32x3", v / 1000, (v / 100) % 10, nt, w);
@@ -881,9 +883,34 @@
     return (KH == 4 ? 1 : 2) * 2 * vec;
 }
 
+static bool conv2d_bits_kernel(const ssr_conv_desc& d, int impl) {
+    if (d.dtype != SSR_F32X3 && d.dtype != SSR_F32H) return false;
+    if (d.s2d) {
+        ssr_conv_desc e = d;
+        e.KH = e.KW = 2; e.stride = 1; e.pad_y = e.pad_x = 0; e.Cin = 4 * d.Cin;
+        return d.KH == 4 && d.KW == 4 && d.stride == 2 && d.pad_y == 1 && d.pad_x == 1 && ssr_conv2d_s2d_ok(d.dtype, d.Cin, d.Cout, d.CoutPad) &&
+               ssr_conv_bigx3_shape_ok(e);
+    }
+    if (impl == 4) return ssr_conv_bigx3_shape_ok(d);
+    return impl == 0 && !ssr_conv_thin_qualifies(d) && ssr_conv_bigx3_qualifies(d);
+}
+
+extern "C" int ssr_conv2d_bits_ok(const ssr_conv_desc* dp) {
+    if (!dp) return 0;
+    const ssr_conv_desc& d = *dp;
+    if (!d.ybits && !d.mbits) return 1;
+    if (d.dtype == SSR_F32X3 && d.KH == 2 && d.KW == 2 && d.stride == 1 && !d.s2d && d.oys == 2 && d.oxs == 2) {
+        static const bool off = [] { const char* e = getenv("SSR_CONV_BATCH"); return e && e[0] == '0'; }();
+        const ssr_conv_desc ds[4] = {d, d, d, d};
+        return !off && ssr_conv_bigx3_batch_qualifies(ds, 4) ? 1 : 0;
+    }
+    return conv2d_bits_kernel(d, 0) ? 1 : 0;
+}
+
 static int conv2d_impl(const ssr_conv_desc* dp, void* stream, int impl) {
     if (!dp) return SSR_EINVAL;
     const ssr_conv_desc& d = *dp;
+    if ((d.ybits || d.mbits) && !conv2d_bits_kernel(d, impl)) return SSR_EUNSUP;
     if (d.act < SSR_ACT_NONE || d.act > SSR_ACT_RELU) return SSR_EINVAL;
     if (!view_ok(d.x, true) || !d.w || ((uintptr_t)d.w % 16) != 0) return SSR_EINVAL;
     if (!d.y.p || d.y.cs <= 0) return SSR_EINVAL;
diff --git a/satlas_super_resolution_amd/csrc/conv_big_x3.hip b/satlas_super_resolution_amd/csrc/conv_big_x3.hip
--- a/satlas_super_resolution_amd/csrc/conv_big_x3.hip
+++ b/satlas_super_resolution_amd/csrc/conv_big_x3.hip
@@ -41,6 +41,10 @@
     row = 8 * w + 2 * m + (s >> 4);
     col = s < 16 ? s : ((s + 32 - (XB_TW + KT - 1)) & 15);
 }
+typedef unsigned u32x2 __attribute__((ext_vector_type(2)));
+template <int CTRL> __device__ __forceinline__ unsigned xb_dpp(unsigned v) {
+    return (unsigned)__builtin_amdgcn_update_dpp(0, (int)v, CTRL, 0xf, 0xf, true);
+}
 __device__ __forceinline__ void xb_split4(const u32x4& v, uint2& hi, uint2& lo) {
     const f32x4 f = __builtin_bit_cast(f32x4, v);
     bf16x4 h, l;
@@ -53,7 +57,7 @@
     lo = __builtin_bit_cast(uint2, l);
 }
 
-template <int KT, bool H = false>
+template <int KT, bool H = false, bool BK = false>
 __device__ __forceinline__ void conv_bigx3_body(const ssr_conv_desc& d) {
     using T = XbT<KT>;
     constexpr int AROW = T::AROW, VPP = T::VPP, PW = T::PW, NPIX = T::NPIX, PATCH = T::PATCH, NPV = T::NPV, NWV = T::NWV, NSTEP = T::NSTEP;
@@ -188,14 +192,18 @@
     };
 
     char* slab = smem + T::SLABS + wave * XB_SLAB;
-    auto epilogue_impl = [&](int nn, auto opsc, auto y01c) __attribute__((always_inline)) {
-        constexpr bool OPS = decltype(opsc)::value, Y01 = decltype(y01c)::value;
+    auto epilogue_impl = [&](int nn, auto opsc, auto y01c, auto bitsc) __attribute__((always_inline)) {
+        constexpr bool OPS = decltype(opsc)::value, Y01 = decltype(y01c)::value, BITS = decltype(bitsc)::value;
         const long obytes = (long)d.N * oimg * 4;
+        const bool has_yb = BITS && d.ybits != nullptr, yb_s0 = BITS && d.ybits_s0 != 0;
+        const void* const bp = has_yb ? (const void*)d.ybits : (const void*)d.mbits;
+        const int b_w = has_yb ? d.ybits_words : d.mbits_words, wd0 = co0 >> 5;
         const __amdgpu_buffer_rsrc_t rs_r1 = xb_rsrc(d.r1.p, d.r1.p ? obytes * d.r1.cs : 0), rs_r2 = xb_rsrc(d.r2.p, d.r2.p ? obytes * d.r2.cs : 0),
-                                     rs_m = xb_rsrc(d.m.p, d.m.p ? obytes * d.m.cs : 0), rs_y = xb_rsrc(d.y.p, obytes * d.y.cs),
+                                     rs_m = BITS ? xb_rsrc(bp, bp ? obytes * b_w : 0) : xb_rsrc(d.m.p, d.m.p ? obytes * d.m.cs : 0), rs_y = xb_rsrc(d.y.p, obytes * d.y.cs),
                                      rs_y0 = xb_rsrc(d.y0.p, d.y0.p ? obytes * d.y0.cs : 0), rs_y1 = xb_rsrc(d.y1.p, d.y1.p ? obytes * d.y1.cs : 0);
-        const bool has_r1 = d.r1.p != nullptr, has_r2 = d.r2.p != nullptr, has_m = d.m.p != nullptr, has_acc = d.accumulate != 0,
-                   has_y0 = d.y0.p != nullptr, has_y1 = d.y1.p != nullptr, m_relu = d.m_relu != 0;
+        const bool has_r1 = d.r1.p != nullptr, has_r2 = d.r2.p != nullptr, has_m = BITS ? !has_yb : d.m.p != nullptr, has_acc = d.accumulate != 0,
+                   has_y0 = !BITS && d.y0.p != nullptr, has_y1 = d.y1.p != nullptr, m_relu = d.m_relu != 0;
+        const float fneg = m_relu ? 0.f : LRELU_SLOPE;
         const float slope = d.act == SSR_ACT_LRELU ? 0.2f : d.act == SSR_ACT_RELU ? 0.f : 1.f;
         const float alpha = d.alpha, beta1 = has_r1 ? d.beta1 : 0.f, beta2 = has_r2 ? d.beta2 : 0.f, gacc = has_acc ? 1.f : 0.f;
         const int y_cs = d.y.cs, y_co = d.y.coff, y0_cs = d.y0.cs, y0_co = d.y0.coff, y1_cs = d.y1.cs, y1_co = d.y1.coff;
@@ -204,6 +212,9 @@
         const int pimg = nn * oimg;
         const int hp = lane >> 4, c = co0 + (lane & 15) * 4;
         const bool cok = c < d.Cout;
+        unsigned ybit[4];
+#pragma unroll
+        for (int e = 0; e < 4; ++e) ybit[e] = BITS && cok ? 1u << (4 * (lane & 7) + e) : 0u;
 #pragma unroll
         for (int m = 0; m < 4; ++m) {
             int po[8];
@@ -225,7 +236,8 @@
                 }
 #pragma unroll
             for (int hh = 0; hh < 2; ++hh) {
-                u32x4 q1[OPS ? 4 : 1], q2[OPS ? 4 : 1], qa[OPS ? 4 : 1], qm[OPS ? 4 : 1];
+                u32x4 q1[OPS ? 4 : 1], q2[OPS ? 4 : 1], qa[OPS ? 4 : 1], qm[OPS && !BITS ? 4 : 1];
+                u32x2 qb[OPS && BITS ? 4 : 1];
                 if constexpr (OPS) {
 #pragma unroll
                     for (int h4 = 0; h4 < 4; ++h4) {
@@ -233,7 +245,8 @@
                         q1[h4] = __builtin_amdgcn_raw_buffer_load_b128(rs_r1, cok && has_r1 ? (pp * r1_cs + r1_co + c) * 4 : XB_OOB, 0, 0);
                         q2[h4] = __builtin_amdgcn_raw_buffer_load_b128(rs_r2, cok && has_r2 ? (pp * r2_cs + r2_co + c) * 4 : XB_OOB, 0, 0);
                         qa[h4] = __builtin_amdgcn_raw_buffer_load_b128(rs_y, cok && has_acc ? (pp * y_cs + y_co + c) * 4 : XB_OOB, 0, 0);
-                        qm[h4] = __builtin_amdgcn_raw_buffer_load_b128(rs_m, cok && has_m ? (pp * m_cs + m_co + c) * 4 : XB_OOB, 0, 0);
+                        if constexpr (BITS) qb[h4] = __builtin_amdgcn_raw_buffer_load_b64(rs_m, cok && has_m ? (pp * b_w + wd0) * 4 : XB_OOB, 0, 0);
+                        else qm[h4] = __builtin_amdgcn_raw_buffer_load_b128(rs_m, cok && has_m ? (pp * m_cs + m_co + c) * 4 : XB_OOB, 0, 0);
                     }
                 }
 #pragma unroll
@@ -244,6 +257,8 @@
                     const bool ok = po[h] >= 0;
                     const int pp = po[h] & 0x7fffffff;
                     f32x4 v, s0, s1;
+                    unsigned mnib = 0, wv = 0;
+                    if constexpr (OPS && BITS) mnib = ((lane & 8) ? qb[h4][1] : qb[h4][0]) >> (4 * (lane & 7));
 #pragma unroll
                     for (int e = 0; e < 4; ++e) {
                         float x = fmaxf(a[e], slope * a[e]) * alpha;
@@ -251,16 +266,29 @@
                         if constexpr (OPS) {
                             x += beta1 * __builtin_bit_cast(f32x4, q1[h4])[e] + beta2 * __builtin_bit_cast(f32x4, q2[h4])[e] + gacc * __builtin_bit_cast(f32x4, qa[h4])[e];
                             s1[e] = x;
-                            const float mv = __builtin_bit_cast(f32x4, qm[h4])[e];
-                            const float f = m_relu ? (mv > 0.f ? 1.f : 0.f) : lrelu_grad_from_out(mv);
-                            x *= has_m ? f : 1.f;
+                            if constexpr (BITS) {
+                                x *= has_m ? ((mnib >> e) & 1u ? 1.f : fneg) : 1.f;
+                            } else {
+                                const float mv = __builtin_bit_cast(f32x4, qm[h4])[e];
+                                const float f = m_relu ? (act_out_positive(mv) ? 1.f : 0.f) : lrelu_grad_from_out(mv);
+                                x *= has_m ? f : 1.f;
+                            }
                         } else {
                             s1[e] = x;
                         }
                         v[e] = x;
+                        if constexpr (BITS) wv |= act_out_positive(OPS && yb_s0 ? s0[e] : x) ? ybit[e] : 0u;
+                    }
+                    if constexpr (BITS) {
+                        wv |= xb_dpp<0xB1>(wv);
+                        wv |= xb_dpp<0x4E>(wv);
+                        wv |= xb_dpp<0x141>(wv);
+                        const u32x2 w2 = {wv, xb_dpp<0x128>(wv)};
+                        __builtin_amdgcn_raw_buffer_store_b64(w2, rs_m, ok && has_yb && (lane & 15) == 0 ? (pp * b_w + wd0) * 4 : XB_OOB, 0, 0);
                     }
                     if constexpr (Y01) {
-                        __builtin_amdgcn_raw_buffer_store_b128(__builtin_bit_cast(u32x4, s0), rs_y0, ok && has_y0 ? (pp * y0_cs + y0_co + c) * 4 : XB_OOB, 0, 0);
+                        if constexpr (!BITS)
+                            __builtin_amdgcn_raw_buffer_store_b128(__builtin_bit_cast(u32x4, s0), rs_y0, ok && has_y0 ? (pp * y0_cs + y0_co + c) * 4 : XB_OOB, 0, 0);
                         __builtin_amdgcn_raw_buffer_store_b128(__builtin_bit_cast(u32x4, s1), rs_y1, ok && has_y1 ? (pp * y1_cs + y1_co + c) * 4 : XB_OOB, 0, 0);
                     }
                     __builtin_amdgcn_raw_buffer_store_b128(__builtin_bit_cast(u32x4, v), rs_y, ok ? (pp * y_cs + y_co + c) * 4 : XB_OOB, 0, 0);
@@ -269,14 +297,18 @@
         }
     };
     auto epilogue = [&](int nn) __attribute__((always_inline)) {
-        const bool ops = d.r1.p != nullptr || d.r2.p != nullptr || d.m.p != nullptr || d.accumulate != 0;
+        const bool ops = d.r1.p != nullptr || d.r2.p != nullptr || d.m.p != nullptr || d.mbits != nullptr || d.accumulate != 0;
         const bool y01 = d.y0.p != nullptr || d.y1.p != nullptr;
-        if (ops) {
-            if (y01) epilogue_impl(nn, std::true_type{}, std::true_type{});
-            else epilogue_impl(nn, std::true_type{}, std::false_type{});
+        if constexpr (BK) {
+            if (y01) epilogue_impl(nn, std::true_type{}, std::true_type{}, std::true_type{});
+            else if (ops) epilogue_impl(nn, std::true_type{}, std::false_type{}, std::true_type{});
+            else epilogue_impl(nn, std::false_type{}, std::false_type{}, std::true_type{});
+        } else if (ops) {
+            if (y01) epilogue_impl(nn, std::true_type{}, std::true_type{}, std::false_type{});
+            else epilogue_impl(nn, std::true_type{}, std::false_type{}, std::false_type{});
         } else {
-            if (y01) epilogue_impl(nn, std::false_type{}, std::true_type{});
-            else epilogue_impl(nn, std::false_type{}, std::false_type{});
+            if (y01) epilogue_impl(nn, std::false_type{}, std::true_type{}, std::false_type{});
+            else epilogue_impl(nn, std::false_type{}, std::false_type{}, std::false_type{});
         }
     };
 
@@ -365,7 +397,16 @@
     conv_bigx3_body<KT, true>(p.d[blockIdx.z]);
 }
 
-template <int KT, bool H = false>
+template <int KT>
+__global__ __launch_bounds__(256, 1) void conv_bigx3b_kernel4(const ssr_conv_desc4x p) {
+    conv_bigx3_body<KT, false, true>(p.d[blockIdx.z]);
+}
+template <int KT>
+__global__ __launch_bounds__(256, 1) void conv_bigh3b_kernel4(const ssr_conv_desc4x p) {
+    conv_bigx3_body<KT, true, true>(p.d[blockIdx.z]);
+}
+
+template <int KT, bool H = false, bool BK = false>
 int launch_bigx3(const ssr_conv_desc* ds, int n, hipStream_t st) {
     constexpr int lds = XbT<KT>::LDS;
     const ssr_conv_desc& d = ds[0];
@@ -386,7 +427,7 @@
         if (g >= 1) G = g < d.N ? g : d.N;
     }
     const int tiles = tpi * G;
-    auto kern = H ? conv_bigh3_kernel4<KT> : conv_bigx3_kernel4<KT>;
+    auto kern = BK ? (H ? conv_bigh3b_kernel4<KT> : conv_bigx3b_kernel4<KT>) : (H ? conv_bigh3_kernel4<KT> : conv_bigx3_kernel4<KT>);
     static bool attr_done[SSR_MAX_DEVICES] = {};
     const int attr_dev = ssr_device_ordinal();
     if (!attr_done[attr_dev]) {
@@ -417,6 +458,14 @@
     if (d.r1.p && d.r1_nc < d.Cout) return false;
     if (d.r2.p && d.r2_nc < d.Cout) return false;
     if (d.m.p && !(d.m_c0 == 0 && d.m_c1 >= d.Cout)) return false;
+    if (d.ybits || d.mbits) {
+        if (d.m.p || d.y0.p || (d.ybits && d.mbits) || d.CoutPad - d.Cout >= 64) return false;
+        if (d.mbits && !(d.m_c0 == 0 && d.m_c1 >= d.Cout)) return false;
+        auto plane = [&](const void* p, int words) {
+            return !p || (words > 0 && (words % 2) == 0 && 32 * words >= d.CoutPad && ((uintptr_t)p % 8) == 0 && (long)d.N * d.Ho * d.Wo * 4 * words <= 0x7fffff00L);
+        };
+        if (!plane(d.ybits, d.ybits_words) || !plane(d.mbits, d.mbits_words)) return false;
+    }
     const long lim = 0x7fffff00L;
     const long xin = ((long)d.N * d.Hi * d.Wi + d.Wi + 1) * d.x.cs * 4, npo = (long)d.N * d.Ho * d.Wo * 4;
     if (xin > lim || npo * d.y.cs > lim || (d.y0.p && npo * d.y0.cs > lim) || (d.y1.p && npo * d.y1.cs > lim) || (d.r1.p && npo * d.r1.cs > lim) ||
@@ -436,12 +485,15 @@
 
 bool ssr_conv_bigx3_try(const ssr_conv_desc& d, hipStream_t st, int* rc, bool force) {
     if (force ? !ssr_conv_bigx3_shape_ok(d) : !ssr_conv_bigx3_qualifies(d)) return false;
-    if (d.dtype == SSR_F32H) *rc = d.KH == 3 ? launch_bigx3<3, true>(&d, 1, st) : launch_bigx3<2, true>(&d, 1, st);
+    if (d.ybits || d.mbits) {
+        if (d.dtype == SSR_F32H) *rc = d.KH == 3 ? launch_bigx3<3, true, true>(&d, 1, st) : launch_bigx3<2, true, true>(&d, 1, st);
+        else *rc = d.KH == 3 ? launch_bigx3<3, false, true>(&d, 1, st) : launch_bigx3<2, false, true>(&d, 1, st);
+    } else if (d.dtype == SSR_F32H) *rc = d.KH == 3 ? launch_bigx3<3, true>(&d, 1, st) : launch_bigx3<2, true>(&d, 1, st);
     else *rc = d.KH == 3 ? launch_bigx3<3>(&d, 1, st) : launch_bigx3<2>(&d, 1, st);
     return true;
 }
 
-bool ssr_conv_bigx3_batch_try(const ssr_conv_desc* ds, int n, hipStream_t st, int* rc) {
+bool ssr_conv_bigx3_batch_qualifies(const ssr_conv_desc* ds, int n) {
     const char* e = getenv("SSR_X3_BIGTILE2");
     const bool off = e && e[0] == '0', always = e && e[0] == '2';
     if (off || n < 1 || n > 4) return false;
@@ -450,10 +502,14 @@
     const ssr_conv_desc& d = ds[0];
     for (int k = 1; k < n; ++k)
         if (ds[k].N != d.N || ds[k].Gh != d.Gh || ds[k].Gw != d.Gw || ds[k].CoutPad != d.CoutPad || ds[k].Cin != d.Cin || ds[k].Hi != d.Hi || ds[k].Wi != d.Wi ||
-            ds[k].up != d.up)
+            ds[k].up != d.up || (ds[k].ybits != nullptr || ds[k].mbits != nullptr) != (d.ybits != nullptr || d.mbits != nullptr))
             return false;
     const long per_img = (long)((d.Gh + XB_TH - 1) / XB_TH) * ((d.Gw + XB_TW - 1) / XB_TW) * (d.CoutPad / 64) * n;
-    if (!always && (per_img < 8 || d.Gh < 24)) return false;
-    *rc = launch_bigx3<2>(ds, n, st);
+    return always || (per_img >= 8 && d.Gh >= 24);
+}
+
+bool ssr_conv_bigx3_batch_try(const ssr_conv_desc* ds, int n, hipStream_t st, int* rc) {
+    if (!ssr_conv_bigx3_batch_qualifies(ds, n)) return false;
+    *rc = (ds[0].ybits || ds[0].mbits) ? launch_bigx3<2, false, true>(ds, n, st) : launch_bigx3<2>(ds, n, st);
     return true;
 }
diff --git a/satlas_super_resolution_amd/csrc/conv_x3c.hip b/satlas_super_resolution_amd/csrc/conv_x3c.hip
--- a/satlas_super_resolution_amd/csrc/conv_x3c.hip
+++ b/satlas_super_resolution_amd/csrc/conv_x3c.hip
@@ -393,6 +393,7 @@
     for (int k = 0; k < n; ++k) {
         const ssr_conv_desc& d = ds[k];
         if (d.dtype != SSR_F32X3 || !ssr_conv_x3r_shape_ok(d) || d.CoutPad != 32 || d.Cout > 32) return 0;
+        if (d.ybits || d.mbits) return 0;
         if (d.N != ds[0].N || d.Hi != ds[0].Hi || d.Wi != ds[0].Wi || d.Gh != ds[0].Gh || d.Gw != ds[0].Gw) return 0;
         if ((d.Cin % 16) != 0 || (d.x2.p && (d.Cin2 % 16) != 0) || (d.Cin + d.Cin2) / 16 > XC_MAXCH || d.Cin + d.Cin2 < 16) return 0;
         int nt = 0, nu = 0, ep = 3;
diff --git a/satlas_super_resolution_amd/engine.py b/satlas_super_resolution_amd/engine.py
--- a/satlas_super_resolution_amd/engine.py
+++ b/satlas_super_resolution_amd/engine.py
@@ -304,7 +304,7 @@
 
     def conv(self, L: Launcher, name: str, x: View, hi: int, wi: int, y: View, *, up=1, act=hip.ACT_NONE, alpha=1.0,
              y0: View = hip.NULL_VIEW, r1: View = hip.NULL_VIEW, r1_nc=0, beta1=0.0, r2: View = hip.NULL_VIEW,
-             r2_nc=0, beta2=0.0, cin: Optional[int] = None):
+             r2_nc=0, beta2=0.0, cin: Optional[int] = None, ybits: Optional[torch.Tensor] = None, ybits_s0=False):
         s = self.store.specs[name]
         cout_pad, _, _, _ = self.store.pad[name]
         d = ConvDesc()
@@ -328,6 +328,10 @@
         d.accumulate = 0
         d.m, d.m_c0, d.m_c1 = hip.NULL_VIEW, 0, 0
         d.s2d = 1 if self.store.s2d.get(name) else 0
+        if ybits is not None:
+            d.ybits, d.ybits_words, d.ybits_s0 = ybits.data_ptr(), ybits.shape[-1], 1 if ybits_s0 else 0
+        if L is None:
+            return d
         self.keep.append(d)
         fix = (self.store.fwd_dtype == hip.F32X3 and act == hip.ACT_LRELU and s.stride == 1 and s.k == 3 and alpha == 1.0 and not y0.p
                and not r1.p and not r2.p and X3_FIXUP[0])
@@ -355,7 +359,9 @@
     def dgrad(self, L: Launcher, name: str, dy: View, gh: int, gw: int, y: View, *, cout: Optional[int] = None,
               alpha=1.0, y1: View = hip.NULL_VIEW, r1: View = hip.NULL_VIEW, r1_nc=0, beta1=0.0,
               r2: View = hip.NULL_VIEW, r2_nc=0, beta2=0.0, accumulate=0, m: View = hip.NULL_VIEW, m_c0=0, m_c1=0,
-              cin_dy: Optional[int] = None, m_relu=0):
+              cin_dy: Optional[int] = None, m_relu=0, mbits: Optional[torch.Tensor] = None):
+        if mbits is not None:
+            m = hip.NULL_VIEW
         s = self.store.specs[name]
         _, _, cin_pad_o, cout_pad_i = self.store.pad[name]
         wbase = self.packed_dgrad[name].data_ptr()
@@ -390,11 +396,29 @@
             d.accumulate = accumulate
             d.m, d.m_c0, d.m_c1 = m, m_c0, m_c1
             d.m_relu = m_relu
+            if mbits is not None:
+                d.mbits, d.mbits_words = mbits.data_ptr(), mbits.shape[-1]
+        if L is None:
+            return arr
         self.keep.append(arr)
         if len(classes) == 1:
             L.add(hip.lib().ssr_conv2d, C.byref(arr[0]), what=f"conv dgrad {name}")
         else:
             L.add(hip.lib().ssr_conv2d_batch, arr, len(classes), what=f"conv dgrad {name}")
+        return arr
+
+
+    def mask_plane(self, ho: int, wo: int, c: int, producer, consumer) -> Optional[torch.Tensor]:
+        if os.environ.get("SSR_MASK_BITS", "0") != "1":
+            return None
+        plane = torch.zeros(self.N, ho, wo, hip.mask_bits_words(c), dtype=torch.int32, device=self.store.device)
+        if not hip.conv_bits_ok(producer(plane)) or not hip.conv_bits_ok(consumer(plane)[0]):
+            return None
+        return plane
+
+    def n_bits_descs(self) -> Tuple[int, int]:
+        ds = [d for k in self.keep for d in (k if isinstance(k, C.Array) else [k]) if isinstance(d, ConvDesc)]
+        return sum(1 for d in ds if d.ybits), sum(1 for d in ds if d.mbits)
 
 
 def gather_dgrad(cb: "_ConvBuilder", L: Launcher, prefix: str, k: int, x1: View, c1: int, x2: View, c2: int, gh: int,
@@ -807,11 +831,23 @@
                         r2=view(buf(r - 2), 0), r2_nc=nf, beta2=1.0, cin=cd)
         self._link_rdb_prefetch(self._rdb_descs)
         cb.conv(F, "conv_body", view(self.body_out), H, W, view(self.trunk), r1=view(self.feat, 0), r1_nc=nf, beta1=1.0)
+        self.hr_bits = self.up_bits = None
+        if training:
+            Ho_, Wo_, nu = self.Ho, self.Wo, self.n_up
+            up_src = self.ups[nu - 2] if nu > 1 else self.trunk
+            d_out_probe = d_out_buf if d_out_buf is not None else self.out
+            g_probe = self.hr
+            self.hr_bits = cb.mask_plane(Ho_, Wo_, nf,
+                                         lambda pl: cb.conv(None, "conv_hr", view(self.ups[-1]), Ho_, Wo_, view(self.hr), act=hip.ACT_LRELU, ybits=pl),
+                                         lambda pl: cb.dgrad(None, "conv_last", view(d_out_probe), Ho_, Wo_, view(g_probe), m_c0=0, m_c1=nf, mbits=pl))
+            self.up_bits = cb.mask_plane(Ho_, Wo_, nf,
+                                         lambda pl: cb.conv(None, self.up_names[-1], view(up_src), Ho_ // 2, Wo_ // 2, view(self.ups[-1]), up=2, act=hip.ACT_LRELU, ybits=pl),
+                                         lambda pl: cb.dgrad(None, "conv_hr", view(g_probe), Ho_, Wo_, view(g_probe), m_c0=0, m_c1=nf, mbits=pl))
         src, sh, sw = self.trunk, H, W
         for i, nm in enumerate(self.up_names):
-            cb.conv(F, nm, view(src), sh, sw, view(self.ups[i]), up=2, act=hip.ACT_LRELU)
+            cb.conv(F, nm, view(src), sh, sw, view(self.ups[i]), up=2, act=hip.ACT_LRELU, ybits=self.up_bits if i == self.n_up - 1 else None)
             src, sh, sw = self.ups[i], sh * 2, sw * 2
-        cb.conv(F, "conv_hr", view(src), sh, sw, view(self.hr), act=hip.ACT_LRELU)
+        cb.conv(F, "conv_hr", view(src), sh, sw, view(self.hr), act=hip.ACT_LRELU, ybits=self.hr_bits)
         cb.conv(F, "conv_last", view(self.hr), sh, sw, view(self.out))
         self.fwd = F
         if not training:
@@ -871,9 +907,9 @@
         Ho, Wo = self.Ho, self.Wo
         last_up = self.ups[-1]
         add_wg("conv_last", view(self.hr), view(self.d_out), Ho, Wo, 1, Ho, Wo)
-        cb.dgrad(Bk, "conv_last", view(self.d_out), Ho, Wo, view(self.g_hr), m=view(self.hr), m_c0=0, m_c1=nf)
+        cb.dgrad(Bk, "conv_last", view(self.d_out), Ho, Wo, view(self.g_hr), m=view(self.hr), m_c0=0, m_c1=nf, mbits=self.hr_bits)
         add_wg("conv_hr", view(last_up), view(self.g_hr), Ho, Wo, 1, Ho, Wo)
-        cb.dgrad(Bk, "conv_hr", view(self.g_hr), Ho, Wo, view(self.g_ups[-1]), m=view(last_up), m_c0=0, m_c1=nf)
+        cb.dgrad(Bk, "conv_hr", view(self.g_hr), Ho, Wo, view(self.g_ups[-1]), m=view(last_up), m_c0=0, m_c1=nf, mbits=self.up_bits)
         for i in reversed(range(self.n_up)):
             nm = self.up_names[i]
             hh, ww = H << (i + 1), W << (i + 1)
@@ -1063,11 +1099,15 @@
         self.x0, self.x1, self.x2, self.x3 = z(B, H, W, nf), z(B, H2, W2, 2 * nf), z(B, H4, W4, 4 * nf), z(B, H8, W8, 8 * nf)
         self.u3, self.a4 = z(B, H4, W4, 8 * nf), z(B, H4, W4, 4 * nf)
         self.u4, self.a5 = z(B, H2, W2, 4 * nf), z(B, H2, W2, 2 * nf)
-        self.u5, self.a6 = z(B, H, W, 2 * nf), z(B, H, W, nf)
-        self.x6 = z(B, H, W, nf) if skip_connection else self.a6
+        self.u5 = z(B, H, W, 2 * nf)
+        self.x6 = z(B, H, W, nf)
         self.o7, self.o8 = z(B, H, W, nf), z(B, H, W, nf)
         self.logits = z(B, H, W, 8)
         self._cb = _ConvBuilder(store, B)
+        self.mask_bits: Dict[str, Optional[torch.Tensor]] = {k: None for k in ("o8", "o7", "a6", "x0", "x1", "x2")}
+        if training:
+            self._plan_mask_bits()
+        self.a6_buf = (z(B, H, W, nf) if self.mask_bits["a6"] is None else None) if skip_connection else self.x6
         self._fwd_cache: Dict[Tuple[int, int], Launcher] = {}
         self._bwd_cache: Dict[Tuple, Launcher] = {}
         self.training = training
@@ -1083,6 +1123,48 @@
             self.g3, self.g2, self.g1, self.g0 = z(B, H8, W8, 8 * nf), z(B, H4, W4, 4 * nf), z(B, H2, W2, 2 * nf), z(B, H, W, nf)
             self.g_in = z(B, H, W, self.cdp)
 
+    def _plan_mask_bits(self):
+        cb, nf, H, W = self._cb, self.nf, self.H, self.W
+        H2, W2, H4, W4, H8, W8 = H // 2, W // 2, H // 4, W // 4, H // 8, W // 8
+        LR, NV = hip.ACT_LRELU, hip.NULL_VIEW
+        tdt, dev = hip.torch_dtype(self.dt), self.store.device
+        xin = torch.zeros(self.B, H, W, self.cdp, dtype=tdt, device=dev)
+        g64, g128h, g256q, g512 = self.o7, self.x1, self.x2, self.x3
+        sk = lambda t: (view(t) if self.skip else NV)
+        mb = self.mask_bits
+        mb["o8"] = cb.mask_plane(H, W, nf, lambda pl: cb.conv(None, "conv8", view(self.o7), H, W, view(self.o8), act=LR, ybits=pl),
+                                 lambda pl: cb.dgrad(None, "conv9", view(self.logits), H, W, view(g64), m_c0=0, m_c1=nf, mbits=pl))
+        mb["o7"] = cb.mask_plane(H, W, nf, lambda pl: cb.conv(None, "conv7", view(self.x6), H, W, view(self.o7), act=LR, ybits=pl),
+                                 lambda pl: cb.dgrad(None, "conv8", view(g64), H, W, view(g64), m_c0=0, m_c1=nf, mbits=pl))
+        mb["a6"] = cb.mask_plane(H, W, nf, lambda pl: self._conv6(None, pl),
+                                 lambda pl: cb.dgrad(None, "conv7", view(g64), H, W, view(g64), y1=sk(self.x6), m_c0=0, m_c1=nf, mbits=pl))
+        mb["x0"] = cb.mask_plane(H, W, nf, lambda pl: cb.conv(None, "conv0", view(xin), H, W, view(self.x0), act=LR, cin=self.cdp, ybits=pl),
+                                 lambda pl: cb.dgrad(None, "conv1", view(g128h), H2, W2, view(g64), r1=sk(self.x6), r1_nc=nf, beta1=1.0,
+                                                     m_c0=0, m_c1=nf, mbits=pl))
+        mb["x1"] = cb.mask_plane(H2, W2, 2 * nf, lambda pl: cb.conv(None, "conv1", view(self.x0), H, W, view(self.x1), act=LR, ybits=pl),
+                                 lambda pl: cb.dgrad(None, "conv2", view(g256q), H4, W4, view(g128h), r1=sk(self.x1), r1_nc=2 * nf, beta1=1.0,
+                                                     m_c0=0, m_c1=2 * nf, mbits=pl))
+        mb["x2"] = cb.mask_plane(H4, W4, 4 * nf, lambda pl: cb.conv(None, "conv2", view(self.x1), H2, W2, view(self.x2), act=LR, ybits=pl),
+                                 lambda pl: cb.dgrad(None, "conv3", view(g512), H8, W8, view(g256q), r1=sk(self.x2), r1_nc=4 * nf, beta1=1.0,
+                                                     m_c0=0, m_c1=4 * nf, mbits=pl))
+
+    def _conv6(self, L: Optional[Launcher], a6_bits: Optional[torch.Tensor]):
+        cb, nf, H, W, LR = self._cb, self.nf, self.H, self.W, hip.ACT_LRELU
+        if not self.skip:
+            return cb.conv(L, "conv6", view(self.u5), H, W, view(self.x6), act=LR, ybits=a6_bits)
+        if a6_bits is not None:
+            return cb.conv(L, "conv6", view(self.u5), H, W, view(self.x6), act=LR, r1=view(self.x0), r1_nc=nf, beta1=1.0,
+                           ybits=a6_bits, ybits_s0=True)
+        return cb.conv(L, "conv6", view(self.u5), H, W, view(self.x6), act=LR, y0=view(self.a6_buf), r1=view(self.x0), r1_nc=nf, beta1=1.0)
+
+    @property
+    def a6(self) -> torch.Tensor:
+        if self.a6_buf is not None:
+            return self.a6_buf
+        pl = self.mask_bits["a6"]
+        bit = (pl.unsqueeze(-1) >> torch.arange(32, dtype=torch.int32, device=pl.device)) & 1
+        return (bit.reshape(*pl.shape[:-1], -1)[..., :self.nf].to(torch.float32) * 2 - 1).contiguous()
+
     def forward_plan(self, x_buf: torch.Tensor) -> Launcher:
         key = x_buf.data_ptr()
         if key in self._fwd_cache:
@@ -1093,9 +1175,10 @@
         L = Launcher()
         lib = hip.lib()
         LR = hip.ACT_LRELU
-        cb.conv(L, "conv0", view(x_buf), H, W, view(self.x0), act=LR, cin=self.cdp)
-        cb.conv(L, "conv1", view(self.x0), H, W, view(self.x1), act=LR)
-        cb.conv(L, "conv2", view(self.x1), H2, W2, view(self.x2), act=LR)
+        mb = self.mask_bits
+        cb.conv(L, "conv0", view(x_buf), H, W, view(self.x0), act=LR, cin=self.cdp, ybits=mb["x0"])
+        cb.conv(L, "conv1", view(self.x0), H, W, view(self.x1), act=LR, ybits=mb["x1"])
+        cb.conv(L, "conv2", view(self.x1), H2, W2, view(self.x2), act=LR, ybits=mb["x2"])
         cb.conv(L, "conv3", view(self.x2), H4, W4, view(self.x3), act=LR)
         L.add(lib.ssr_bilinear2x_fwd, view(self.x3), hip.NULL_VIEW, view(self.u3), dt, B, H8, W8, 8 * nf,
               what="bilinear u3")
@@ -1105,13 +1188,9 @@
         cb.conv(L, "conv5", view(self.u4), H2, W2, view(self.a5), act=LR)
         L.add(lib.ssr_bilinear2x_fwd, view(self.a5), view(self.x1) if self.skip else hip.NULL_VIEW, view(self.u5), dt,
               B, H2, W2, 2 * nf, what="bilinear u5")
-        if self.skip:
-            cb.conv(L, "conv6", view(self.u5), H, W, view(self.x6), act=LR, y0=view(self.a6), r1=view(self.x0),
-                    r1_nc=nf, beta1=1.0)
-        else:
-            cb.conv(L, "conv6", view(self.u5), H, W, view(self.a6), act=LR)
-        cb.conv(L, "conv7", view(self.x6), H, W, view(self.o7), act=LR)
-        cb.conv(L, "conv8", view(self.o7), H, W, view(self.o8), act=LR)
+        self._conv6(L, mb["a6"])
+        cb.conv(L, "conv7", view(self.x6), H, W, view(self.o7), act=LR, ybits=mb["o7"])
+        cb.conv(L, "conv8", view(self.o7), H, W, view(self.o8), act=LR, ybits=mb["o8"])
         cb.conv(L, "conv9", view(self.o8), H, W, view(self.logits))
         self._fwd_cache[key] = L
         return L
@@ -1136,14 +1215,14 @@
                                            1.0, st.ptr(st.wkey(name), arena), s.cin,
                                            st.ptr(name + ".bias", st.grad) if s.bias else None)
 
-        NV = hip.NULL_VIEW
+        NV, mb = hip.NULL_VIEW, self.mask_bits
         add_wg("conv9", view(self.o8), view(self.d_logits), H, W, H, W)
-        cb.dgrad(L, "conv9", view(self.d_logits), H, W, view(self.g_o8), m=view(self.o8), m_c0=0, m_c1=nf)
+        cb.dgrad(L, "conv9", view(self.d_logits), H, W, view(self.g_o8), m=view(self.o8), m_c0=0, m_c1=nf, mbits=mb["o8"])
         add_wg("conv8", view(self.o7), view(self.g_o8), H, W, H, W)
-        cb.dgrad(L, "conv8", view(self.g_o8), H, W, view(self.g_o7), m=view(self.o7), m_c0=0, m_c1=nf)
+        cb.dgrad(L, "conv8", view(self.g_o8), H, W, view(self.g_o7), m=view(self.o7), m_c0=0, m_c1=nf, mbits=mb["o7"])
         add_wg("conv7", view(self.x6), view(self.g_o7), H, W, H, W)
         cb.dgrad(L, "conv7", view(self.g_o7), H, W, view(self.g_a6), y1=view(self.g_x6) if self.skip else NV,
-                 m=view(self.a6), m_c0=0, m_c1=nf)
+                 m=view(self.a6_buf), m_c0=0, m_c1=nf, mbits=mb["a6"])
         add_wg("conv6", view(self.u5), view(self.g_a6), H, W, H, W)
         cb.dgrad(L, "conv6", view(self.g_a6), H, W, view(self.g_u5))
         L.add(lib.ssr_bilinear2x_bwd, view(self.g_u5), NV, view(self.g_x5) if self.skip else NV, view(self.g_a5),
@@ -1159,13 +1238,13 @@
         sk = lambda t: (view(t) if self.skip else NV)
         add_wg("conv3", view(self.x2), view(self.g3), H4, W4, H8, W8)
         cb.dgrad(L, "conv3", view(self.g3), H8, W8, view(self.g2), r1=sk(self.g_x4), r1_nc=4 * nf, beta1=1.0,
-                 m=view(self.x2), m_c0=0, m_c1=4 * nf)
+                 m=view(self.x2), m_c0=0, m_c1=4 * nf, mbits=mb["x2"])
         add_wg("conv2", view(self.x1), view(self.g2), H2, W2, H4, W4)
         cb.dgrad(L, "conv2", view(self.g2), H4, W4, view(self.g1), r1=sk(self.g_x5), r1_nc=2 * nf, beta1=1.0,
-                 m=view(self.x1), m_c0=0, m_c1=2 * nf)
+                 m=view(self.x1), m_c0=0, m_c1=2 * nf, mbits=mb["x1"])
         add_wg("conv1", view(self.x0), view(self.g1), H, W, H2, W2)
         cb.dgrad(L, "conv1", view(self.g1), H2, W2, view(self.g0), r1=sk(self.g_x6), r1_nc=nf, beta1=1.0,
-                 m=view(self.x0), m_c0=0, m_c1=nf)
+                 m=view(self.x0), m_c0=0, m_c1=nf, mbits=mb["x0"])
         add_wg("conv0", view(x_buf), view(self.g0), H, W, H, W, cin=self.cdp)
         if input_grad:
             kw = {}
diff --git a/satlas_super_resolution_amd/hip.py b/satlas_super_resolution_amd/hip.py
--- a/satlas_super_resolution_amd/hip.py
+++ b/satlas_super_resolution_amd/hip.py
@@ -48,6 +48,8 @@
         ("s2d", C.c_int32), ("m_relu", C.c_int32),
         ("fix_list", C.c_void_p), ("fix_cap", C.c_int32), ("fix_thr", C.c_float), ("w_ref", C.c_void_p), ("w_ref_sigma", C.c_void_p),
         ("w_ref_cin", C.c_int32),
+        ("ybits", C.c_void_p), ("ybits_words", C.c_int32), ("ybits_s0", C.c_int32),
+        ("mbits", C.c_void_p), ("mbits_words", C.c_int32),
     ]
 
 
@@ -113,7 +115,7 @@
 
 
 ABI_SYMBOLS = [
-    "ssr_conv2d", "ssr_conv2d_fixup", "ssr_conv2d_batch", "ssr_conv2d_impl", "ssr_conv2d_variant", "ssr_conv2d_symbol", "ssr_conv2d_chain", "ssr_conv2d_chain_ok", "ssr_conv2d_chain_state_bytes", "ssr_conv2d_ck", "ssr_conv2d_s2d_ok", "ssr_rdb_forward", "ssr_rdb_backward", "ssr_rdb_tile_of", "ssr_conv2d_wgrad", "ssr_wgrad_reduce", "ssr_wgrad_tiles", "ssr_wgrad_ci_tile", "ssr_wgrad_co_tile", "ssr_pack_weights", "ssr_pack_dgrad_gather", "ssr_add_views", "ssr_nchw_to_nhwc", "ssr_nhwc_to_nchw",
+    "ssr_conv2d", "ssr_conv2d_fixup", "ssr_conv2d_batch", "ssr_conv2d_impl", "ssr_conv2d_variant", "ssr_conv2d_symbol", "ssr_conv2d_chain", "ssr_conv2d_chain_ok", "ssr_conv2d_chain_state_bytes", "ssr_conv2d_ck", "ssr_conv2d_s2d_ok", "ssr_conv2d_bits_ok", "ssr_rdb_forward", "ssr_rdb_backward", "ssr_rdb_tile_of", "ssr_conv2d_wgrad", "ssr_wgrad_reduce", "ssr_wgrad_tiles", "ssr_wgrad_ci_tile", "ssr_wgrad_co_tile", "ssr_pack_weights", "ssr_pack_dgrad_gather", "ssr_add_views", "ssr_nchw_to_nhwc", "ssr_nhwc_to_nchw",
     "ssr_fill", "ssr_bilinear2x_fwd", "ssr_bilinear2x_bwd", "ssr_nearest2x_bwd", "ssr_spectral_norm",
     "ssr_spectral_norm_bwd", "ssr_usm_sharp", "ssr_l1_loss", "ssr_bce_logits_loss", "ssr_adam_step", "ssr_axpby_f32",
     "ssr_quantize_u8", "ssr_metric_shift_sums", "ssr_metric_ssim_sums", "ssr_split_bf16", "ssr_split_bf16_multi", "ssr_channel_affine", "ssr_relu_maxpool2_fwd", "ssr_relu_maxpool2_bwd",
@@ -153,6 +155,7 @@
     l.ssr_conv2d_chain_state_bytes.argtypes = [i32, i32, i32]
     l.ssr_conv2d_ck.argtypes = [i32, i32]
     l.ssr_conv2d_s2d_ok.argtypes = [i32, i32, i32, i32]
+    l.ssr_conv2d_bits_ok.argtypes = [C.POINTER(ConvDesc)]
     l.ssr_rdb_forward.argtypes = [C.POINTER(RdbDesc), vp]
     l.ssr_rdb_backward.argtypes = [C.POINTER(RdbDesc), vp]
     l.ssr_rdb_tile_of.argtypes = [C.POINTER(RdbDesc)]
@@ -282,6 +285,28 @@
     return buf.value.decode()
 
 
+def pack_mask_bits(out: torch.Tensor, words: Optional[int] = None) -> torch.Tensor:
+    C_ = out.shape[-1]
+    nw = (C_ + 31) // 32
+    words = nw if words is None else words
+    assert words >= nw
+    pos = (out.to(torch.float64) > 0).to(torch.int64)
+    pad = words * 32 - C_
+    if pad:
+        pos = torch.cat([pos, pos.new_zeros(*pos.shape[:-1], pad)], dim=-1)
+    pos = pos.reshape(*pos.shape[:-1], words, 32)
+    w = (pos << torch.arange(32, dtype=torch.int64, device=pos.device)).sum(dim=-1)
+    return torch.where(w >= 2 ** 31, w - 2 ** 32, w).to(torch.int32)
+
+
+def mask_bits_words(c: int) -> int:
+    return 2 * ((c + 63) // 64)
+
+
+def conv_bits_ok(desc) -> bool:
+    return lib().ssr_conv2d_bits_ok(C.byref(desc)) == 1
+
+
 def conv_symbol(desc) -> str:
     buf = C.create_string_buffer(96)
     check(lib().ssr_conv2d_symbol(C.byref(desc), buf, 96), "ssr_conv2d_symbol")
```

Measured after the change: 1183. About the same (-0.0%).
